# Hanbo-Cheng/DAWN-pytorch

Measured on NVIDIA H100. Metric: denoising-steps/sec (200-frame 256^2 clip), higher is better.
Workload: dtype f32

## Files before the change

### dawn_pytorch_b200/_lib.py

```python
import ctypes
import os

import torch
from torch import nn

_HERE = os.path.dirname(os.path.abspath(__file__))
LIB_PATH = os.path.join(_HERE, "libdawn_unet.so")


class DawnUnetCfg(ctypes.Structure):
    _fields_ = [("dim", ctypes.c_int), ("n_levels", ctypes.c_int), ("dim_mults", ctypes.c_int * 8),
                ("channels", ctypes.c_int), ("cond_aud", ctypes.c_int), ("cond_pose", ctypes.c_int),
                ("cond_eye", ctypes.c_int), ("out_grid_dim", ctypes.c_int), ("out_conf_dim", ctypes.c_int),
                ("attn_heads", ctypes.c_int), ("attn_dim_head", ctypes.c_int), ("resnet_groups", ctypes.c_int),
                ("init_kernel_size", ctypes.c_int), ("win_width", ctypes.c_int),
                ("upconv", ctypes.c_int), ("pad_mode", ctypes.c_int), ("no_sla", ctypes.c_int)]


class DawnLfgCfg(ctypes.Structure):
    _fields_ = [("num_channels", ctypes.c_int), ("block_expansion", ctypes.c_int), ("max_features", ctypes.c_int),
                ("num_down_blocks", ctypes.c_int), ("num_bottleneck_blocks", ctypes.c_int), ("skips", ctypes.c_int)]


PATH_MMA_SYNC, PATH_TC_GEMM, PATH_TC_GEMM_PRESPLIT, PATH_TC_CONV3, PATH_TC_CONV3_TMA = range(5)
EPI_PLAIN, EPI_QKV_TEMPORAL, EPI_QKV_SLA, EPI_QKV_MID, EPI_CA_GATE, EPI_GN_APPLY, EPI_GELU, EPI_LN_BIAS, EPI_LN_BIAS_GELU = range(9)


class DawnContractionCase(ctypes.Structure):
    _i, _p = ctypes.c_int, ctypes.c_void_p
    _fields_ = [("path", _i), ("epi", _i),
                ("F", _i), ("IH", _i), ("IW", _i), ("Cin", _i), ("lda", _i),
                ("ntaps", _i), ("dy", _i * 52), ("dx", _i * 52), ("in_stride", _i),
                ("OHs", _i), ("OWs", _i), ("OH", _i), ("OW", _i), ("out_stride", _i), ("oy0", _i), ("ox0", _i),
                ("up2", _i),
                ("perm_pb", _i), ("perm_F", _i), ("perm_in", _i), ("perm_out", _i), ("perm_f_lo", _i), ("perm_f_hi", _i),
                ("P", _i),
                ("N", _i), ("ldb", _i), ("ldo", _i), ("ldr", _i), ("drain", _i), ("ln_inline", _i),
                ("rows_per_batch", _i), ("b_batch_stride", ctypes.c_longlong), ("cpg", _i),
                ("q_post_scale", ctypes.c_float),
                ("A", _p), ("B", _p), ("bias", _p), ("Res", _p), ("Out", _p),
                ("stats", _p), ("rowstats", _p), ("wsum", _p), ("rot", _p),
                ("kq", _p), ("nkq", _p), ("gates", _p),
                ("Y", _p), ("ldy", _i), ("gn_stats", _p), ("gn_w", _p), ("gn_b", _p), ("film", _p), ("gn_count", ctypes.c_double)]


FUSED_TEMPORAL, FUSED_ATTN_TC, FUSED_ATTN_SIMT, FUSED_SLA_CTX, FUSED_SLA_OUT, FUSED_SLA_CTX_UNFUSED, FUSED_CA_WT, \
    FUSED_CA_RSTD, FUSED_GN_HCOND, FUSED_TEMPORAL_MMA_SYNC = range(10)


class DawnFusedCase(ctypes.Structure):
    _i, _p = ctypes.c_int, ctypes.c_void_p
    _fields_ = [("kernel", _i), ("F", _i), ("P", _i), ("C", _i), ("band", _i), ("q_lo", _i), ("q_hi", _i),
                ("nseq", _i), ("L", _i), ("pb", _i), ("seq_base_stride", ctypes.c_longlong), ("elem_stride", ctypes.c_longlong),
                ("ldx", _i), ("ldr", _i), ("ldo", _i), ("ld", _i), ("ldb", _i), ("ldy", _i), ("ldbT", _i),
                ("x", _p), ("res", _p), ("out", _p), ("gamma", _p), ("w_qkv", _p), ("w_out", _p), ("rot", _p), ("bias", _p),
                ("qkv", _p), ("Bf", _p), ("out_bias", _p), ("kq", _p), ("nkq", _p), ("G", _p), ("gates", _p), ("Wt", _p),
                ("T", _p), ("Y", _p), ("out16h", _p), ("out16l", _p),
                ("gn_stats", _p), ("gn_count", ctypes.c_double), ("cpg", _i), ("gn_w", _p), ("gn_b", _p), ("film", _p)]


KERNEL_ROWSTATS, KERNEL_GN_APPLY, KERNEL_COND_TABLES, KERNEL_TIME_MLP, KERNEL_FILM, KERNEL_ROTARY, KERNEL_SPLIT_ROWS, \
    KERNEL_NCF_TO_NHWC, KERNEL_FRAME_INVARIANCE, KERNEL_FEA_SHIFT, KERNEL_MAP_REDUCE, KERNEL_INIT_CONV_X3, KERNEL_HEADS_OUT, \
    KERNEL_DDIM_STEP, KERNEL_DDPM_STEP = range(15)
KERNEL_MAX_DESC = 16


class DawnKernelDesc(ctypes.Structure):
    _i, _p = ctypes.c_int, ctypes.c_void_p
    _fields_ = [("off", _i), ("K", _i), ("co", _i), ("ldbT", _i), ("ca", _i),
                ("mW", _p), ("mB", _p), ("Wkv", _p), ("nkv", _p), ("qs", _p), ("ks", _p), ("Wout", _p), ("gout", _p),
                ("ctx", _p), ("kv", _p), ("kq", _p), ("nkq", _p), ("T", _p), ("G", _p),
                ("W", _p), ("b", _p), ("out", _p), ("n", _i)]


class DawnKernelCase(ctypes.Structure):
    _i, _p, _ll = ctypes.c_int, ctypes.c_void_p, ctypes.c_longlong
    _fields_ = [("kernel", _i), ("M", _i), ("C", _i), ("ld", _i), ("ldy", _i), ("ldr", _i), ("ldo", _i),
                ("F", _i), ("H", _i), ("W", _i), ("P", _i), ("clips", _i),
                ("Cpad", _i), ("c0", _i), ("k", _i), ("skip_if", _i), ("cpg", _i), ("t_stride", _i), ("pos0", _i), ("dim", _i),
                ("ng", _i), ("nc", _i), ("cond_ld", _i), ("ndesc", _i),
                ("n", _ll), ("cstride", _ll), ("clip_stride", _ll), ("count", ctypes.c_double), ("eps", ctypes.c_float),
                ("x", _p), ("y", _p), ("res", _p), ("w", _p), ("b", _p), ("w2", _p), ("b2", _p),
                ("map", _p), ("freqs", _p), ("stats", _p), ("t", _p), ("skip_flag", _p),
                ("out", _p), ("out_hi", _p), ("out_lo", _p), ("flag", _p),
                ("desc", DawnKernelDesc * KERNEL_MAX_DESC),
                ("xs", _p), ("e", _p), ("noise", _p), ("scratch", _p), ("tab", _p), ("t_slot", _p), ("num_t", _i),
                ("replicas", _i), ("coef", ctypes.c_float * 5), ("q", ctypes.c_float)]


LFG_MOTION_PACK, LFG_WARP_BLEND, LFG_AFFINE_RELU, LFG_RESIDUAL_BN_RELU, LFG_RELU_AVGPOOL2, LFG_CHW_TO_HWC, LFG_HWC_TO_CHW, \
    LFG_FINAL_CONV = range(8)


class DawnLfgKernelCase(ctypes.Structure):
    _i, _p = ctypes.c_int, ctypes.c_void_p
    _fields_ = [("kernel", _i), ("F", _i), ("H", _i), ("W", _i), ("h", _i), ("w", _i), ("C", _i), ("Cpad", _i),
                ("layout", _i), ("blend", _i), ("ldx", _i), ("ldp", _i), ("ldo", _i), ("M", ctypes.c_longlong),
                ("x", _p), ("y", _p), ("flow", _p), ("occ", _p), ("motion", _p), ("prev", _p), ("scale", _p), ("shift", _p),
                ("weight", _p), ("bias", _p), ("source", _p), ("out", _p), ("out2", _p)]


class DawnLfgMotionCfg(ctypes.Structure):
    _i, _f = ctypes.c_int, ctypes.c_float
    _fields_ = [("num_regions", _i), ("num_channels", _i), ("estimate_affine", _i), ("pca_based", _i), ("fast_svd", _i),
                ("rp_block_expansion", _i), ("rp_max_features", _i), ("rp_num_blocks", _i), ("rp_temperature", _f),
                ("rp_scale_factor", _f), ("bg_block_expansion", _i), ("bg_max_features", _i), ("bg_num_blocks", _i),
                ("bg_type", _i), ("pw_block_expansion", _i), ("pw_max_features", _i), ("pw_num_blocks", _i),
                ("pw_scale_factor", _f), ("use_covar_heatmap", _i), ("use_deformed_source", _i),
                ("estimate_occlusion_map", _i), ("revert_axis_swap", _i)]


LFG_BG_ZERO, LFG_BG_AFFINE = 0, 1
LFGM_AA_DOWN, LFGM_REGION_MOMENTS, LFGM_FLOW_INPUT, LFGM_FLOW_COMBINE, LFGM_BG_HEAD = range(5)


class DawnLfgMotionKernelCase(ctypes.Structure):
    _i, _p = ctypes.c_int, ctypes.c_void_p
    _fields_ = [("kernel", _i), ("N", _i), ("H", _i), ("W", _i), ("h", _i), ("w", _i), ("R", _i), ("ld", _i), ("off", _i),
                ("cw", _i), ("ldl", _i), ("revert", _i), ("temperature", ctypes.c_float),
                ("x", _p), ("weight", _p), ("logits", _p), ("motion", _p), ("source", _p), ("bg", _p), ("fc_w", _p), ("fc_b", _p),
                ("src_shift", _p), ("src_covar", _p), ("src_affine", _p), ("drv_shift", _p), ("drv_covar", _p), ("drv_affine", _p),
                ("out", _p), ("out2", _p), ("out3", _p)]


class DawnPbnetCfg(ctypes.Structure):
    _fields_ = [(n, ctypes.c_int) for n in ("band", "pose_dim", "audio_dim", "latent_dim", "audio_latent_dim", "pose_latent_dim",
                                            "ff_size", "num_layers", "num_heads")]


class DawnPbnetAttentionCase(ctypes.Structure):
    _i, _p = ctypes.c_int, ctypes.c_void_p
    _fields_ = [("bs", _i), ("F", _i), ("D", _i), ("H", _i), ("band", _i), ("npairs", _i), ("qscale", ctypes.c_float),
                ("x_q", _p), ("x_kv", _p), ("wq", _p), ("wk", _p), ("wv", _p), ("freqs", _p), ("bias", _p), ("out", _p)]


class DawnHubertCfg(ctypes.Structure):
    _i = ctypes.c_int
    _fields_ = [("hidden_size", _i), ("num_layers", _i), ("num_heads", _i), ("intermediate_size", _i), ("num_conv", _i),
                ("conv_dim", _i * 8), ("conv_kernel", _i * 8), ("conv_stride", _i * 8), ("conv_bias", _i), ("pos_kernel", _i),
                ("pos_groups", _i), ("layer_norm_eps", ctypes.c_float)]


HUBERT_ATTENTION, HUBERT_CONV0, HUBERT_POS_CONV, HUBERT_ROW_LN, HUBERT_FE_CONV, HUBERT_LN_LINEAR = range(6)


class DawnHubertKernelCase(ctypes.Structure):
    _i, _p = ctypes.c_int, ctypes.c_void_p
    _fields_ = [("kernel", _i), ("B", _i), ("T", _i), ("L", _i), ("H", _i), ("ld", _i), ("C", _i), ("k", _i), ("s", _i), ("G", _i),
                ("eps", ctypes.c_float), ("q", _p), ("kk", _p), ("v", _p), ("x", _p), ("w", _p), ("bias", _p), ("gamma", _p),
                ("beta", _p), ("g", _p), ("out", _p),
                ("M", _i), ("N", _i), ("ldo", _i), ("gelu", _i), ("parts", _i), ("qscale", ctypes.c_float)]


class DawnError(RuntimeError):
    pass


def _load():
    if not os.path.exists(LIB_PATH):
        raise ImportError(
            f"{LIB_PATH} is missing: build it with `python dawn_pytorch_b200/build.py` "
            "(nvcc, sm_90a). There is no CPU or PyTorch fallback for the DAWN denoising UNet.")
    lib = ctypes.CDLL(LIB_PATH)
    vp, i64p, fp, cp = ctypes.c_void_p, ctypes.POINTER(ctypes.c_int64), ctypes.c_void_p, ctypes.c_char_p
    lib.dawn_unet_create.argtypes = [ctypes.POINTER(DawnUnetCfg), ctypes.POINTER(vp)]
    lib.dawn_unet_destroy.argtypes = [vp]
    lib.dawn_unet_destroy.restype = None
    lib.dawn_unet_set_param.argtypes = [vp, cp, fp, i64p, ctypes.c_int]
    lib.dawn_unet_commit_params.argtypes = [vp]
    lib.dawn_unet_set_num_frames.argtypes = [vp, ctypes.c_int, ctypes.c_int, ctypes.c_int]
    lib.dawn_unet_set_geometry.argtypes = [vp, ctypes.c_int, ctypes.c_int, ctypes.c_int, ctypes.c_int]
    lib.dawn_unet_set_clip_invariants.argtypes = [vp, fp, fp, vp]
    lib.dawn_unet_forward.argtypes = [vp, fp, vp, fp, fp, vp]
    lib.dawn_unet_forward_x3.argtypes = [vp, fp, vp, fp, vp]
    lib.dawn_unet_forward_host.argtypes = [vp, fp, fp, fp, ctypes.c_int64, fp]
    lib.dawn_unet_set_tap.argtypes = [vp, cp, fp]
    lib.dawn_unet_tap_shape.argtypes = [vp, cp, ctypes.POINTER(ctypes.c_int), ctypes.POINTER(ctypes.c_int),
                                        ctypes.POINTER(ctypes.c_int)]
    dp = ctypes.POINTER(ctypes.c_double)
    lib.dawn_unet_profile_enable.argtypes = [vp, ctypes.c_int]
    lib.dawn_unet_profile_read.argtypes = [vp, dp, dp, dp, i64p]
    lib.dawn_unet_last_launch_count.argtypes = [vp]
    lib.dawn_unet_last_launch_count.restype = ctypes.c_int64
    lib.dawn_unet_workspace_bytes.argtypes = [vp]
    lib.dawn_unet_workspace_bytes.restype = ctypes.c_int64
    lib.dawn_test_contraction.argtypes = [ctypes.POINTER(DawnContractionCase), vp]
    lib.dawn_test_fused.argtypes = [ctypes.POINTER(DawnFusedCase), vp]
    lib.dawn_test_kernel.argtypes = [ctypes.POINTER(DawnKernelCase), vp]
    lib.dawn_nccl_unique_id.argtypes = [ctypes.c_char_p]
    lib.dawn_unet_init_shard.argtypes = [vp, ctypes.c_char_p, ctypes.c_int, ctypes.c_int, ctypes.c_int]
    lib.dawn_unet_shard_ipc_export.argtypes = [vp, ctypes.c_char_p]
    lib.dawn_unet_shard_ipc_import.argtypes = [vp, ctypes.c_char_p]
    lib.dawn_ddim_step.argtypes = [fp, fp, fp, ctypes.c_int64] + [ctypes.c_float] * 6 + [vp, vp]
    lib.dawn_unet_ddim_step.argtypes = [vp, fp, fp, fp, ctypes.c_int64] + [ctypes.c_float] * 6 + [vp, vp]
    lib.dawn_unet_sampler_capture.argtypes = [vp, fp, fp, fp, vp, ctypes.POINTER(ctypes.c_float), ctypes.c_int, ctypes.c_float, vp]
    lib.dawn_unet_sampler_launch.argtypes = [vp, vp]
    lib.dawn_unet_ddim_step_guided.argtypes = [vp, fp, fp, fp, ctypes.c_int64, fp] + [ctypes.c_float] * 6 + [vp, vp]
    lib.dawn_unet_sampler_capture_guided.argtypes = [vp, fp, fp, fp, vp, fp, ctypes.POINTER(ctypes.c_float), ctypes.c_int,
                                                     ctypes.c_float, vp]
    lib.dawn_unet_sampler_launch_guided.argtypes = [vp, vp]
    lib.dawn_ddpm_step.argtypes = [fp, fp, fp, ctypes.c_int64] + [ctypes.c_float] * 6 + [vp, vp]
    lib.dawn_unet_ddpm_step.argtypes = [vp, fp, fp, fp, ctypes.c_int64] + [ctypes.c_float] * 6 + [vp, vp]
    lib.dawn_unet_ddpm_capture.argtypes = [vp, fp, fp, fp, vp, fp, ctypes.c_int, ctypes.c_float, vp]
    lib.dawn_unet_ddpm_launch.argtypes = [vp, vp]
    ip = ctypes.POINTER(ctypes.c_int)
    lib.dawn_lfg_create.argtypes = [ctypes.POINTER(DawnLfgCfg), ctypes.POINTER(vp)]
    lib.dawn_lfg_destroy.argtypes = [vp]
    lib.dawn_lfg_destroy.restype = None
    lib.dawn_lfg_set_param.argtypes = [vp, cp, fp, i64p, ctypes.c_int]
    lib.dawn_lfg_commit_params.argtypes = [vp]
    lib.dawn_lfg_set_geometry.argtypes = [vp] + [ctypes.c_int] * 5
    lib.dawn_lfg_set_source.argtypes = [vp, fp, vp]
    lib.dawn_lfg_get_fea.argtypes = [vp, fp, vp]
    lib.dawn_lfg_decode.argtypes = [vp, fp, fp, fp, fp, vp]
    lib.dawn_lfg_decode_sample.argtypes = [vp, fp, fp, fp, vp]
    lib.dawn_lfg_read_tap.argtypes = [vp, cp, fp, ip, ip, ip, vp]
    lib.dawn_conv3x3_s2_relu.argtypes = [fp, ctypes.c_int, ctypes.c_int, ctypes.c_int, fp, fp, ctypes.c_int, fp, vp]
    lib.dawn_lfg_last_launch_count.argtypes = [vp]
    lib.dawn_lfg_last_launch_count.restype = ctypes.c_int64
    lib.dawn_lfg_workspace_bytes.argtypes = [vp]
    lib.dawn_lfg_workspace_bytes.restype = ctypes.c_int64
    lib.dawn_lfg_test_kernel.argtypes = [ctypes.POINTER(DawnLfgKernelCase), vp]
    lib.dawn_lfg_motion_create.argtypes = [ctypes.POINTER(DawnLfgMotionCfg), ctypes.POINTER(vp)]
    lib.dawn_lfg_motion_destroy.argtypes = [vp]
    lib.dawn_lfg_motion_destroy.restype = None
    lib.dawn_lfg_motion_set_param.argtypes = [vp, cp, fp, i64p, ctypes.c_int]
    lib.dawn_lfg_motion_commit_params.argtypes = [vp]
    lib.dawn_lfg_motion_set_geometry.argtypes = [vp] + [ctypes.c_int] * 3
    lib.dawn_lfg_motion_regions.argtypes = [vp, fp, ctypes.c_int, fp, fp, fp, vp]
    lib.dawn_lfg_motion_bg.argtypes = [vp, fp, ctypes.c_int, fp, ctypes.c_int, fp, vp]
    lib.dawn_lfg_motion_flow.argtypes = [vp, fp, ctypes.c_int] + [fp] * 9 + [vp]
    lib.dawn_lfg_motion_read_tap.argtypes = [vp, cp, fp, ip, ip, ip, ip, vp]
    lib.dawn_lfg_motion_last_launch_count.argtypes = [vp]
    lib.dawn_lfg_motion_last_launch_count.restype = ctypes.c_int64
    lib.dawn_lfg_motion_workspace_bytes.argtypes = [vp]
    lib.dawn_lfg_motion_workspace_bytes.restype = ctypes.c_int64
    lib.dawn_lfg_motion_test_kernel.argtypes = [ctypes.POINTER(DawnLfgMotionKernelCase), vp]
    lib.dawn_pbnet_create.argtypes = [ctypes.POINTER(DawnPbnetCfg), ctypes.POINTER(vp)]
    lib.dawn_pbnet_destroy.argtypes = [vp]
    lib.dawn_pbnet_destroy.restype = None
    lib.dawn_pbnet_set_param.argtypes = [vp, cp, fp, i64p, ctypes.c_int]
    lib.dawn_pbnet_commit_params.argtypes = [vp]
    lib.dawn_pbnet_generate.argtypes = [vp, fp, fp, fp, fp, ctypes.c_int, ctypes.c_int, fp, vp]
    lib.dawn_pbnet_last_launch_count.argtypes = [vp]
    lib.dawn_pbnet_last_launch_count.restype = ctypes.c_int64
    lib.dawn_pbnet_workspace_bytes.argtypes = [vp]
    lib.dawn_pbnet_workspace_bytes.restype = ctypes.c_int64
    lib.dawn_pbnet_test_attention.argtypes = [ctypes.POINTER(DawnPbnetAttentionCase), vp]
    lib.dawn_hubert_create.argtypes = [ctypes.POINTER(DawnHubertCfg), ctypes.POINTER(vp)]
    lib.dawn_hubert_destroy.argtypes = [vp]
    lib.dawn_hubert_destroy.restype = None
    lib.dawn_hubert_set_param.argtypes = [vp, cp, fp, i64p, ctypes.c_int]
    lib.dawn_hubert_commit_params.argtypes = [vp]
    lib.dawn_hubert_forward.argtypes = [vp, fp, ctypes.c_int, ctypes.c_int, fp, vp]
    lib.dawn_hubert_output_length.argtypes = [vp, ctypes.c_int]
    lib.dawn_hubert_hidden.argtypes = [vp, fp, ctypes.c_int, ctypes.c_int, ctypes.c_int, fp, vp]
    lib.dawn_hubert_last_launch_count.argtypes = [vp]
    lib.dawn_hubert_last_launch_count.restype = ctypes.c_int64
    lib.dawn_hubert_workspace_bytes.argtypes = [vp]
    lib.dawn_hubert_workspace_bytes.restype = ctypes.c_int64
    lib.dawn_hubert_test_kernel.argtypes = [ctypes.POINTER(DawnHubertKernelCase), vp]
    lib.dawn_last_error.restype = cp
    lib.dawn_live_bytes.argtypes = []
    lib.dawn_live_bytes.restype = ctypes.c_int64
    lib.dawn_build_info.restype = cp
    return lib


lib = _load()

EXPORTS = ["dawn_unet_create", "dawn_unet_destroy", "dawn_unet_set_param", "dawn_unet_commit_params",
           "dawn_unet_set_num_frames", "dawn_unet_set_geometry", "dawn_nccl_unique_id", "dawn_unet_init_shard", "dawn_unet_shard_ipc_export", "dawn_unet_shard_ipc_import", "dawn_unet_set_clip_invariants", "dawn_unet_forward",
           "dawn_unet_forward_x3", "dawn_unet_forward_host", "dawn_unet_set_tap", "dawn_unet_tap_shape",
           "dawn_unet_profile_enable", "dawn_unet_profile_read", "dawn_unet_last_launch_count", "dawn_unet_workspace_bytes", "dawn_ddim_step", "dawn_unet_ddim_step", "dawn_unet_sampler_capture", "dawn_unet_sampler_launch",
           "dawn_unet_ddim_step_guided", "dawn_unet_sampler_capture_guided", "dawn_unet_sampler_launch_guided",
           "dawn_ddpm_step", "dawn_unet_ddpm_step", "dawn_unet_ddpm_capture", "dawn_unet_ddpm_launch",
           "dawn_test_contraction", "dawn_test_fused", "dawn_test_kernel", "dawn_last_error", "dawn_live_bytes", "dawn_build_info"]


LFG_EXPORTS = ["dawn_lfg_create", "dawn_lfg_destroy", "dawn_lfg_set_param", "dawn_lfg_commit_params", "dawn_lfg_set_geometry",
               "dawn_lfg_set_source", "dawn_lfg_get_fea", "dawn_lfg_decode", "dawn_lfg_decode_sample", "dawn_lfg_read_tap",
               "dawn_lfg_last_launch_count", "dawn_lfg_workspace_bytes", "dawn_lfg_test_kernel"]
LFG_MOTION_EXPORTS = ["dawn_lfg_motion_create", "dawn_lfg_motion_destroy", "dawn_lfg_motion_set_param",
                      "dawn_lfg_motion_commit_params", "dawn_lfg_motion_set_geometry", "dawn_lfg_motion_regions", "dawn_lfg_motion_bg",
                      "dawn_lfg_motion_flow", "dawn_lfg_motion_read_tap", "dawn_lfg_motion_last_launch_count",
                      "dawn_lfg_motion_workspace_bytes", "dawn_lfg_motion_test_kernel"]
LFG_EXPORTS += LFG_MOTION_EXPORTS
MISC_EXPORTS = ["dawn_conv3x3_s2_relu"]
PBNET_EXPORTS = ["dawn_pbnet_create", "dawn_pbnet_destroy", "dawn_pbnet_set_param", "dawn_pbnet_commit_params",
                 "dawn_pbnet_generate", "dawn_pbnet_last_launch_count", "dawn_pbnet_workspace_bytes", "dawn_pbnet_test_attention"]
HUBERT_EXPORTS = ["dawn_hubert_create", "dawn_hubert_destroy", "dawn_hubert_set_param", "dawn_hubert_commit_params",
                  "dawn_hubert_forward", "dawn_hubert_output_length", "dawn_hubert_hidden", "dawn_hubert_last_launch_count", "dawn_hubert_workspace_bytes",
                  "dawn_hubert_test_kernel"]

PROF_CATS = ["conv3x3", "conv_other", "qkv_proj", "out_proj", "ca_gate", "gn_hcond", "attn_core", "sla_context",
             "gn_apply", "rowstats", "ca_rstd", "misc", "prep", "temporal_fused_l0", "conv3x3_l0", "comm_allreduce", "comm_halo"]
PROF_NCAT = 20


def check(rc, what):
    if rc != 0:
        raise DawnError(f"{what} failed (rc={rc}): {lib.dawn_last_error().decode()}")


def stream():
    return ctypes.c_void_p(torch.cuda.current_stream().cuda_stream)


def ptr(t):
    return ctypes.c_void_p(t.data_ptr()) if t is not None else None


def put_param(set_param, handle, name, t):
    t = t.detach().to(device="cpu", dtype=torch.float32).contiguous()
    shape = (ctypes.c_int64 * max(t.dim(), 1))(*t.shape)
    check(set_param(handle, name.encode(), ctypes.c_void_p(t.data_ptr()), shape, t.dim()), f"{set_param.__name__}({name})")


class _Holder(nn.Module):

    def forward(self, *a, **k):
        raise RuntimeError("parameter holder: the computation runs in the CUDA library")


class _Handle:

    def __init__(self, api, cfg, what, param_name=lambda key: key, extra=lambda module: {}, keeps_geom=False):
        self.api, self.cfg, self.what, self.param_name, self.extra, self.keeps_geom = api, cfg, what, param_name, extra, keeps_geom
        self.handle, self.device_index, self.dirty, self.geom, self.commits = None, None, True, None, 0

    def _entry(self, name):
        return getattr(lib, f"{self.api}_{name}")

    def _create(self):
        hd = ctypes.c_void_p()
        check(self._entry("create")(ctypes.byref(self.cfg), ctypes.byref(hd)), f"{self.api}_create")
        return hd

    def validate(self):
        self._entry("destroy")(self._create())

    def destroy(self):
        if self.handle is not None:
            self._entry("destroy")(self.handle)
        self.handle, self.geom = None, None

    def ensure(self, module, device):
        if device.type != "cuda":
            raise DawnError(f"{self.what} runs on CUDA (sm_90a) only; there is no CPU path")
        idx = device.index if device.index is not None else torch.cuda.current_device()
        if self.handle is not None and self.device_index != idx:
            self.destroy()
            self.dirty = True
        with torch.cuda.device(idx):
            if self.handle is None:
                self.handle, self.device_index = self._create(), idx
            if self.dirty:
                for key, t in module.state_dict().items():
                    name = None if key.endswith("num_batches_tracked") else self.param_name(key)
                    if name is not None:
                        put_param(self._entry("set_param"), self.handle, name, t)
                for name, t in self.extra(module).items():
                    put_param(self._entry("set_param"), self.handle, name, t)
                check(self._entry("commit_params")(self.handle), f"{self.api}_commit_params")
                self.dirty, self.commits = False, self.commits + 1
                if not self.keeps_geom:
                    self.geom = None
        return idx

    def last_launch_count(self):
        return int(self._entry("last_launch_count")(self.handle)) if self.handle is not None else 0

    def workspace_bytes(self):
        return int(self._entry("workspace_bytes")(self.handle)) if self.handle is not None else 0


class _NativeModule(nn.Module):
    TRAIN_REFUSAL = None

    def _hold(self, *handles):
        self._handles = list(handles)
        self.register_load_state_dict_post_hook(lambda module, incompatible: module.mark_dirty())
        if self.TRAIN_REFUSAL:
            self.eval()

    def mark_dirty(self):
        for h in self._handles:
            h.dirty = True

    def _apply(self, fn, *a, **k):
        for h in self.__dict__.get("_handles", ()):
            h.dirty = True
        return super()._apply(fn, *a, **k)

    def train(self, mode=True):
        if mode and self.TRAIN_REFUSAL:
            raise NotImplementedError(self.TRAIN_REFUSAL)
        return super().train(mode)

    def __del__(self):
        for h in self.__dict__.get("_handles", ()):
            try:
                h.destroy()
            except Exception:
                pass

    def last_launch_count(self):
        return self._handles[0].last_launch_count()

    def workspace_bytes(self):
        return self._handles[0].workspace_bytes()
```

### dawn_pytorch_b200/csrc/contraction.cu

```cuda
#include <algorithm>
#include <atomic>
#include <cmath>
#include <cstring>

#include "common.cuh"
#include "contraction.cuh"
#include "kernels.cuh"
#include "tc_gemm.cuh"

namespace dawn {

void HostParams::set(const std::string& name, const float* data, const int64_t* shape, int ndim) {
  HostParam p;
  p.shape.assign(shape, shape + ndim);
  int64_t numel = 1;
  for (int64_t s : p.shape) numel *= s;
  p.data.assign(data, data + numel);
  map[name] = std::move(p);
}

int HostParams::need(const std::string& name, const std::vector<int64_t>& shape, const HostParam** out) const {
  auto it = map.find(name);
  if (it == map.end()) { set_last_error(prefix + "missing parameter: " + name); return -1; }
  const HostParam& p = it->second;
  if (p.shape != shape) {
    std::string s = prefix + "parameter " + name + " has shape (";
    for (auto d : p.shape) s += std::to_string(d) + ",";
    s += ") expected (";
    for (auto d : shape) s += std::to_string(d) + ",";
    set_last_error(s + ")");
    return -1;
  }
  *out = &p;
  return 0;
}

namespace {
std::atomic<int64_t> g_arena_bytes{0};
}

int DeviceArena::alloc_bytes(size_t bytes, void** out) {
  *out = nullptr;
  bytes = std::max<size_t>(bytes, 16);
  DAWN_CUDA_OK(cudaMalloc(out, bytes));
  blocks_.emplace_back(*out);
  bytes_ += (int64_t)bytes;
  g_arena_bytes += (int64_t)bytes;
  return 0;
}
int DeviceArena::copy_in(void* dst, const void* src, size_t bytes) {
  DAWN_CUDA_OK(cudaMemcpy(dst, src, bytes, cudaMemcpyHostToDevice));
  return 0;
}
void DeviceArena::release() {
  blocks_.clear();
  g_arena_bytes -= bytes_;
  bytes_ = 0;
}
int64_t DeviceArena::live_bytes() { return g_arena_bytes.load(); }

int upload_weight(DeviceArena& arena, const std::vector<float>& m, int K, int N, int ldb, const std::vector<float>& bias,
                  PackedWeight* out) {
  *out = PackedWeight{};
  DAWN_TRY(arena.upload(m, &out->w));
  if (N % 64 == 0 && K % 64 == 0) {
    std::vector<float> img;
    tc_pack_weights(m.data(), K, N, ldb, img, &out->img_scale);
    DAWN_TRY(arena.upload(img, &out->img));
  }
  if (!bias.empty()) {
    std::vector<float> b(ldb, 0.f);
    std::copy(bias.begin(), bias.end(), b.begin());
    DAWN_TRY(arena.upload(b, &out->b));
  }
  out->K = K; out->N = N; out->ldb = ldb;
  return 0;
}

std::vector<float> fold_linear(const float* w, int N, int K, const float* gain, float qscale, int nscale) {
  std::vector<float> m((size_t)N * K);
  for (int n = 0; n < N; ++n) {
    const float sc = (n < nscale) ? qscale : 1.0f;
    for (int k = 0; k < K; ++k) {
      float v = w[(size_t)n * K + k];
      if (gain) v *= gain[k];
      m[(size_t)n * K + k] = v * sc;
    }
  }
  return m;
}

std::vector<float> row_sums(const std::vector<float>& w, int N, int K) {
  std::vector<float> s(N);
  for (int n = 0; n < N; ++n) {
    double acc = 0.0;
    for (int k = 0; k < K; ++k) acc += w[(size_t)n * K + k];
    s[n] = (float)acc;
  }
  return s;
}

void fold_ca_q(const float* const to_q[3], const float* const gain[3], int ci, std::vector<float>& wq, std::vector<float>& wsum) {
  wq.assign((size_t)ci * 192, 0.f);
  wsum.assign(192, 0.f);
  for (int a = 0; a < 3; ++a) {
    const std::vector<float> m = fold_linear(to_q[a], 64, ci, gain[a], 1.f, 0);
    const std::vector<float> s = row_sums(m, 64, ci);
    for (int j = 0; j < 64; ++j) {
      for (int k = 0; k < ci; ++k) wq[(size_t)k * 192 + a * 64 + j] = m[(size_t)j * ci + k];
      wsum[a * 64 + j] = s[j];
    }
  }
}

int bn_affine(const HostParams& raw, const std::string& prefix, int c, std::vector<double>& s, std::vector<double>& t) {
  const HostParam *g, *b, *rm, *rv;
  DAWN_TRY(raw.need(prefix + ".weight", {c}, &g));
  DAWN_TRY(raw.need(prefix + ".bias", {c}, &b));
  DAWN_TRY(raw.need(prefix + ".running_mean", {c}, &rm));
  DAWN_TRY(raw.need(prefix + ".running_var", {c}, &rv));
  s.resize(c); t.resize(c);
  for (int i = 0; i < c; ++i) {
    s[i] = (double)g->data[i] / std::sqrt((double)rv->data[i] + 1e-5);
    t[i] = (double)b->data[i] - (double)rm->data[i] * s[i];
  }
  return 0;
}

void pack_conv_taps(const float* w, int co, int ci, int taps, int ci_pad, int ldb, int n0, const double* scale, std::vector<float>& m) {
  for (int n = 0; n < co; ++n) {
    const double sn = scale ? scale[n] : 1.0;
    for (int c = 0; c < ci; ++c)
      for (int tp = 0; tp < taps; ++tp)
        m[((size_t)tp * ci_pad + c) * ldb + n0 + n] = (float)((double)w[((size_t)n * ci + c) * taps + tp] * sn);
  }
}

int pack_lfg_conv(const HostParams& raw, DeviceArena& arena, const std::vector<std::pair<std::string, int>>& convs,
                  const std::string& bn_after, int ci, int k, int ci_pad, PackedWeight* out) {
  int N = 0;
  for (auto& c : convs) N += c.second;
  const int ldb = round_up(N, 64), K = k * k * ci_pad;
  std::vector<float> m((size_t)K * ldb, 0.f), bias(N);
  int n0 = 0;
  for (auto& cv : convs) {
    const int co = cv.second;
    const HostParam *w, *b;
    DAWN_TRY(raw.need(cv.first + ".weight", {co, ci, k, k}, &w));
    DAWN_TRY(raw.need(cv.first + ".bias", {co}, &b));
    std::vector<double> s(co, 1.0), t(co, 0.0);
    if (!bn_after.empty()) DAWN_TRY(bn_affine(raw, bn_after, co, s, t));
    for (int n = 0; n < co; ++n) bias[n0 + n] = (float)((double)b->data[n] * s[n] + t[n]);
    pack_conv_taps(w->data.data(), co, ci, k * k, ci_pad, ldb, n0, s.data(), m);
    n0 += co;
  }
  return upload_weight(arena, m, K, N, ldb, bias, out);
}

void base_params(GemmParams& p, const float* A, int lda, int Cin, int frames, int H, int W) {
  memset(&p, 0, sizeof(p));
  p.A = A; p.lda = lda; p.Cin = Cin;
  p.IH = H; p.IW = W; p.OHs = H; p.OWs = W; p.in_stride = 1;
  p.ntaps = 1;
  p.M = frames * H * W; p.rows_per_batch = p.M;
  p.OH = H; p.OW = W; p.out_stride = 1;
  p.P = H * W;
  p.q_post_scale = 1.f;
  p.clips = 1;
}
void set_weights(GemmParams& p, const PackedWeight& w) {
  p.B = w.w; p.Bimg = w.img; p.tc_scale = 1.0f / w.img_scale; p.ldb = w.ldb; p.N = w.N; p.K = w.K; p.bias = w.b;
}
void set_square_taps(GemmParams& p, int k, int pad) {
  p.ntaps = k * k;
  for (int ky = 0; ky < k; ++ky)
    for (int kx = 0; kx < k; ++kx) { p.dy[ky * k + kx] = (signed char)(ky - pad); p.dx[ky * k + kx] = (signed char)(kx - pad); }
}

namespace {
long long split_rows(const GemmParams& p) { return (long long)(p.M / (p.OHs * p.OWs)) * p.IH * p.IW; }
}

bool path_ok(const GemmParams& p, int epi, int path, size_t scratch_bytes) {
  const bool planes = p.A16h != nullptr || (p.Cin % 64 == 0 && (size_t)split_rows(p) * p.Cin * 4 <= scratch_bytes);
  switch (path) {
    case DAWN_PATH_MMA_SYNC: return true;
    case DAWN_PATH_TC_GEMM: return p.Bimg && tc_gemm_supported(p, epi);
    case DAWN_PATH_TC_GEMM_PRESPLIT: return p.Bimg && tc_gemm_supported(p, epi) && planes;
    case DAWN_PATH_TC_CONV3: return p.Bimg && tc_conv3_supported(p, epi);
    case DAWN_PATH_TC_CONV3_TMA: return p.Bimg && tc_conv3_supported(p, epi) && p.lda == p.Cin && planes;
  }
  return false;
}

int choose_path(const GemmParams& p, int epi, size_t scratch_bytes) {
  if (path_ok(p, epi, DAWN_PATH_TC_CONV3, 0)) return p.A16h ? DAWN_PATH_TC_CONV3_TMA : DAWN_PATH_TC_CONV3;
  if (!path_ok(p, epi, DAWN_PATH_TC_GEMM, 0)) return DAWN_PATH_MMA_SYNC;
  const bool split = (p.ntaps == 9 && p.N >= 256 && !p.perm_in) || p.want_split;
  return split && path_ok(p, epi, DAWN_PATH_TC_GEMM_PRESPLIT, scratch_bytes) ? DAWN_PATH_TC_GEMM_PRESPLIT : DAWN_PATH_TC_GEMM;
}

int launch_path(const GemmParams& p, int epi, int path, void* scratch, cudaStream_t st, int* kernels) {
  if (kernels) *kernels = 1;
  if (path == DAWN_PATH_MMA_SYNC) return launch_gemm(p, epi, st);
  GemmParams q = p;
  if ((path == DAWN_PATH_TC_GEMM_PRESPLIT || path == DAWN_PATH_TC_CONV3_TMA) && p.A16h == nullptr) {
    const long long rows = split_rows(p);
    unsigned short* hi = static_cast<unsigned short*>(scratch);
    q.A16h = hi; q.A16l = hi + (size_t)rows * p.Cin;
    DAWN_TRY(launch_split_rows(p.A, p.lda, p.Cin, rows, (void*)q.A16h, (void*)q.A16l, st));
    if (kernels) *kernels = 2;
  }
  if (path == DAWN_PATH_TC_CONV3 || path == DAWN_PATH_TC_CONV3_TMA) return launch_tc_conv3(q, q.Bimg, st);
  return launch_tc_gemm(q, q.Bimg, epi, st);
}

int pack_up(DeviceArena& arena, int ci, int co, const int (&off)[2][2], const std::vector<float>& bias, const UpWeight& weight,
            UpConv* u) {
  memcpy(u->off, off, sizeof(u->off));
  const int ldb = round_up(co, 64);
  for (int py = 0; py < 2; ++py)
    for (int px = 0; px < 2; ++px) {
      std::vector<float> m((size_t)4 * ci * ldb, 0.f);
      for (int ty = 0; ty < 2; ++ty)
        for (int tx = 0; tx < 2; ++tx)
          for (int c = 0; c < ci; ++c)
            for (int n = 0; n < co; ++n) m[((size_t)(ty * 2 + tx) * ci + c) * ldb + n] = weight(py, px, ty, tx, c, n);
      DAWN_TRY(upload_weight(arena, m, 4 * ci, co, ldb, bias, &u->cls[py * 2 + px]));
    }
  if (co == 64 && ci % 64 == 0) {
    const int N4 = 4 * co;
    std::vector<float> m((size_t)9 * ci * N4, 0.f), b4(N4, 0.f);
    for (int py = 0; py < 2; ++py)
      for (int px = 0; px < 2; ++px) {
        const int cls = py * 2 + px;
        for (int n = 0; n < co; ++n) b4[cls * co + n] = bias[n];
        for (int ty = 0; ty < 2; ++ty)
          for (int tx = 0; tx < 2; ++tx) {
            const int tap = (off[py][ty] + 1) * 3 + (off[px][tx] + 1);
            for (int c = 0; c < ci; ++c)
              for (int n = 0; n < co; ++n) m[((size_t)tap * ci + c) * N4 + cls * co + n] = weight(py, px, ty, tx, c, n);
          }
      }
    DAWN_TRY(upload_weight(arena, m, 9 * ci, N4, N4, b4, &u->all));
  }
  return 0;
}

int pack_up_nearest(DeviceArena& arena, const float* w, int ci, int co, const double* scale, const std::vector<float>& bias,
                    UpConv* u) {
  return pack_up(arena, ci, co, kUpOff, bias, [&](int py, int px, int ty, int tx, int c, int n) {
    double acc = 0.0;
    for (int ky = 0; ky < 3; ++ky)
      for (int kx = 0; kx < 3; ++kx)
        if (up_in_set(py, ty, ky) && up_in_set(px, tx, kx)) acc += (double)w[(((size_t)n * ci + c) * 3 + ky) * 3 + kx];
    return (float)(scale ? acc * scale[n] : acc);
  }, u);
}

int pack_lfg_up(const HostParams& raw, DeviceArena& arena, const std::string& name, int co, int ci, UpConv* u) {
  const HostParam *w, *b;
  DAWN_TRY(raw.need(name + ".conv.weight", {co, ci, 3, 3}, &w));
  DAWN_TRY(raw.need(name + ".conv.bias", {co}, &b));
  std::vector<double> s, t;
  DAWN_TRY(bn_affine(raw, name + ".norm", co, s, t));
  std::vector<float> bias(co);
  for (int n = 0; n < co; ++n) bias[n] = (float)((double)b->data[n] * s[n] + t[n]);
  return pack_up_nearest(arena, w->data.data(), ci, co, s.data(), bias, u);
}

int run_up(const GemmParams& in, const UpConv& u, float* out, int ldo, const std::function<int(const GemmParams&)>& run, int border) {
  if (!border) {
    GemmParams p = in;
    set_weights(p, u.all); set_square_taps(p, 3, 1);
    p.up2 = 1; p.Out = out; p.ldo = ldo;
    if (path_ok(p, EPI_PLAIN, DAWN_PATH_TC_CONV3, 0)) return run(p);
  }
  for (int py = 0; py < 2; ++py)
    for (int px = 0; px < 2; ++px) {
      GemmParams q = in;
      set_weights(q, u.cls[py * 2 + px]);
      q.ntaps = 4;
      for (int ty = 0; ty < 2; ++ty)
        for (int tx = 0; tx < 2; ++tx) {
          q.dy[ty * 2 + tx] = (signed char)(u.off[py][ty] + border); q.dx[ty * 2 + tx] = (signed char)(u.off[px][tx] + border);
        }
      q.OH = 2 * in.OHs; q.OW = 2 * in.OWs; q.out_stride = 2; q.oy0 = py; q.ox0 = px;
      q.Out = out; q.ldo = ldo;
      DAWN_TRY(run(q));
    }
  return 0;
}

namespace {

int refuse(const char* why) {
  set_last_error(std::string("dawn_test_contraction: ") + why);
  return -1;
}

int test_contraction(const dawn_contraction_case& c, cudaStream_t st) {
  if (c.path < DAWN_PATH_MMA_SYNC || c.path > DAWN_PATH_TC_CONV3_TMA) return refuse("unknown path");
  if (c.epi < EPI_PLAIN || c.epi > EPI_LN_BIAS_GELU) return refuse("unknown epilogue");
  if (c.ntaps < 1 || c.ntaps > 52 || c.F < 1 || c.N < 1 || c.ldb < c.N || c.lda < 1 || (c.ntaps > 1 && c.lda < c.Cin))
    return refuse("bad geometry");
  if (!c.A || !c.B) return refuse("A and B are required");
  if (c.epi == EPI_CA_GATE ? !c.gates : !c.Out) return refuse("no output buffer");

  GemmParams p;
  memset(&p, 0, sizeof(p));
  p.A = c.A; p.lda = c.lda; p.Cin = c.Cin;
  p.up2 = c.up2;
  p.IH = c.IH; p.IW = c.IW; p.OHs = c.OHs; p.OWs = c.OWs; p.in_stride = c.in_stride;
  p.ntaps = c.ntaps;
  for (int t = 0; t < c.ntaps; ++t) { p.dy[t] = (signed char)c.dy[t]; p.dx[t] = (signed char)c.dx[t]; }
  p.M = c.F * c.OHs * c.OWs; p.N = c.N; p.K = c.ntaps * c.Cin;
  p.rows_per_batch = c.rows_per_batch > 0 ? c.rows_per_batch : p.M;
  p.perm_pb = c.perm_pb; p.perm_F = c.perm_F; p.perm_in = c.perm_in; p.perm_out = c.perm_out;
  p.perm_f_lo = c.perm_f_lo; p.perm_f_hi = c.perm_f_hi;
  p.B = c.B; p.ldb = c.ldb; p.b_batch_stride = c.b_batch_stride;
  p.Out = c.Out; p.ldo = c.ldo; p.OH = c.OH; p.OW = c.OW; p.out_stride = c.out_stride; p.oy0 = c.oy0; p.ox0 = c.ox0;
  p.bias = c.bias; p.Res = c.Res; p.ldr = c.ldr;
  p.stats = c.stats; p.cpg = c.cpg; p.clips = 1;
  p.rowstats = c.rowstats; p.ln_inline = c.ln_inline; p.wsum = c.wsum; p.rot = c.rot; p.P = c.P;
  p.q_post_scale = c.q_post_scale;
  p.kq = c.kq; p.nkq = c.nkq; p.gates = c.gates;
  p.Y = c.Y; p.ldy = c.ldy; p.gn_stats = c.gn_stats; p.gn_w = c.gn_w; p.gn_b = c.gn_b; p.film = c.film; p.gn_count = c.gn_count;
  p.drain = c.drain;

  const bool ln_bias = c.epi == EPI_LN_BIAS || c.epi == EPI_LN_BIAS_GELU;
  const bool ln = (c.epi >= EPI_QKV_TEMPORAL && c.epi <= EPI_CA_GATE) || ln_bias;
  if (p.ln_inline && (c.path != DAWN_PATH_TC_GEMM || p.ntaps != 1)) return refuse("inline LayerNorm statistics need the gather-producer wgmma GEMM and one tap");
  if (ln && !p.ln_inline && !p.rowstats) return refuse("LayerNorm epilogue without row statistics");
  if (ln && !p.wsum) return refuse("LayerNorm epilogue without wsum");
  if (ln_bias && !p.bias) return refuse("LayerNorm + bias epilogue without a bias");
  if (p.stats && c.epi != EPI_PLAIN) return refuse("GroupNorm statistics with an epilogue other than the plain one");
  if (c.epi == EPI_PLAIN && p.stats && (p.cpg <= 0 || p.N / p.cpg > 8)) return refuse("GroupNorm statistics need 8 groups");

  DeviceArena arena;
  if (c.path != DAWN_PATH_MMA_SYNC) {
    std::vector<float> hB((size_t)p.K * p.ldb);
    DAWN_CUDA_OK(cudaMemcpy(hB.data(), p.B, hB.size() * sizeof(float), cudaMemcpyDeviceToHost));
    PackedWeight w;
    DAWN_TRY(upload_weight(arena, hB, p.K, p.N, p.ldb, {}, &w));
    set_weights(p, w);
    p.bias = c.bias;
  }
  const bool split = c.path == DAWN_PATH_TC_GEMM_PRESPLIT || c.path == DAWN_PATH_TC_CONV3_TMA;
  const size_t scratch_bytes = split ? (size_t)split_rows(p) * p.Cin * 4 : 0;
  if (!path_ok(p, c.epi, c.path, scratch_bytes)) return refuse("the path does not accept this geometry");
  unsigned short* scratch = nullptr;
  if (split) DAWN_TRY(arena.alloc(scratch_bytes / sizeof(unsigned short), &scratch));
  DAWN_TRY(launch_path(p, c.epi, c.path, scratch, st));
  DAWN_CUDA_OK(cudaStreamSynchronize(st));
  return 0;
}

}
}

extern "C" int dawn_test_contraction(const dawn_contraction_case* c, void* stream) {
  if (!c) return dawn::refuse("null case");
  return dawn::test_contraction(*c, static_cast<cudaStream_t>(stream));
}
```

### dawn_pytorch_b200/csrc/gemm.cuh

```cuda
#pragma once
#include <cuda_runtime.h>

namespace dawn {

enum Epi : int {
  EPI_PLAIN = 0,
  EPI_QKV_TEMPORAL = 1,
  EPI_QKV_SLA = 2,
  EPI_QKV_MID = 3,
  EPI_CA_GATE = 4,
  EPI_GN_APPLY = 5,
  EPI_GELU = 6,
  EPI_LN_BIAS = 7,
  EPI_LN_BIAS_GELU = 8,
};

__device__ __forceinline__ float gelu_erf(float x) { return 0.5f * x * (1.0f + erff(x * 0.70710678118654752440f)); }

struct GemmParams {
  const float* A; int lda; int Cin;
  const unsigned short* A16h = nullptr; const unsigned short* A16l = nullptr;
  int want_split = 0;
  int up2 = 0;
  int IH, IW;
  int OHs, OWs;
  int in_stride;
  int ntaps; signed char dy[52]; signed char dx[52];
  int M, N, K;
  int rows_per_batch;
  int perm_pb, perm_F, perm_in, perm_out;
  int perm_f_lo, perm_f_hi;
  const float* B; int ldb; long long b_batch_stride;
  const float* Bimg;
  float tc_scale;
  float* Out; int ldo; int OH, OW, out_stride, oy0, ox0;
  const float* bias;
  const float* Res; int ldr;
  double* stats; int cpg;
  int clips;
  const float* rowstats;
  int ln_inline;
  const float* wsum;
  const float* rot;
  int P;
  float q_post_scale;
  const float* kq;
  const float* nkq;
  float* gates;
  const float* Y; int ldy; const double* gn_stats; const float* gn_w; const float* gn_b;
  const float* film;
  double gn_count;
  const int* skip_flag; int skip_if;
  int drain;
};

__host__ __device__ inline int seq_blocked_pixel(int m, int pb, int F, int P) {
  const int blk = m / (F * pb), rem = m - blk * F * pb;
  const int f = rem / pb, pi = rem - f * pb;
  return f * P + blk * pb + pi;
}
__host__ __device__ inline int seq_blocked_out_pixel(int m, int pb, int F, int P, int f_lo, int f_hi) {
  const int blk = m / (F * pb), rem = m - blk * F * pb;
  const int f = rem / pb, pi = rem - f * pb;
  if (f < f_lo || f >= f_hi) return -1;
  return (f - f_lo) * P + blk * pb + pi;
}

int launch_gemm(const GemmParams& p, int epi, cudaStream_t st);

}
```

### dawn_pytorch_b200/csrc/tc_conv3.cu

```cuda
#include <cuda.h>
#include <cuda_fp16.h>
#include <cstdlib>
#include <cstring>
#include <string>
#include <map>
#include <tuple>
#include "common.cuh"
#include "f16x3.cuh"
#include "gemm.cuh"
#include "tc_common.cuh"
#include "tc_gemm.cuh"

namespace dawn {
namespace {

using namespace tc;

constexpr int TH = 16, TW = 8;
constexpr int HH = TH + 2, HW = TW + 2;
constexpr int NPROD = 256;
constexpr int PAIR_HH = 8 + 2;
constexpr int PAIR_ROW_B = 104;

template <int BN, bool PAIR = false>
struct CCfg {
  static_assert(!PAIR || BN == 64, "the pair-mode halos fit next to 64-column weight stages only");
  static constexpr int NWG = BN / 64;
  static constexpr bool SPLIT_EPI = (BN == 64);
  static constexpr int B_PANEL = BN * 128;
  static constexpr int FRAME_ROWS = PAIR ? PAIR_HH * HW : HH * HW;
  static constexpr int HALO_ROWS = PAIR ? PAIR_ROW_B + FRAME_ROWS : FRAME_ROWS;
  static constexpr int A_HALO = (HALO_ROWS * 128 + 1023) / 1024 * 1024;
  static constexpr int A_STAGES = 2;
  static constexpr int B_STAGES = PAIR ? 3 : (BN == 64) ? 4 : 2;
  static constexpr int A_BYTES = A_STAGES * 2 * A_HALO;
  static constexpr int B_BYTES = B_STAGES * 2 * B_PANEL;
  static constexpr int ACC_STAGE = 2 * 128 * kStageLd * 4;
  static constexpr int SMEM_DYN = A_BYTES + B_BYTES + ACC_STAGE + 1024;
  static_assert(SMEM_DYN + 1024 <= 232448, "shared memory");
  static constexpr int EPI_WARP = NPROD / 32 + 4 * NWG;
  static constexpr int LOAD_WARP = EPI_WARP + (SPLIT_EPI ? 4 : 0);
  static constexpr int NTHREADS = 32 * LOAD_WARP + 128;
  static constexpr uint32_t REG_LAUNCH = (65536 / NTHREADS) & ~7u;
  static constexpr uint32_t REG_LOAD = 24, REG_MMA = SPLIT_EPI ? 136 : 128, REG_EPI = 128;
  static_assert(REG_LOAD < REG_LAUNCH && REG_MMA > REG_LAUNCH && REG_EPI > REG_LAUNCH, "register budgets");
  static_assert(2 * REG_LAUNCH + REG_LOAD + NWG * REG_MMA + (SPLIT_EPI ? REG_EPI : 0) <= NTHREADS / 128 * REG_LAUNCH, "CTA register pool");
};

template <int BN, bool TMA, bool PAIR>
__device__ __forceinline__ void tc_conv3_body(const GemmParams& p, const float* __restrict__ Bimg, int tiles_y, int tiles_x, int tiles_n,
                                              int img_bn, const CUtensorMap& tm_hi, const CUtensorMap& tm_lo) {
  using C = CCfg<BN, PAIR>;
  constexpr int B_PANEL = C::B_PANEL, A_STAGES = C::A_STAGES, B_STAGES = C::B_STAGES, NWG = C::NWG;
  constexpr int A_HALO = C::A_HALO, FRAME_ROWS = C::FRAME_ROWS;
  constexpr bool SPLIT = C::SPLIT_EPI;
  extern __shared__ uint8_t smem_raw[];
  __shared__ uint64_t a_full[A_STAGES], a_free[A_STAGES], b_full[B_STAGES], b_free[B_STAGES];
  __shared__ uint64_t st_full[2], st_free[2];
  __shared__ float s_stat[NWG][16];
  __shared__ __align__(16) float s_bias[NWG][64];

  const int tid = threadIdx.x, lane = tid & 31;
  const int warp = __shfl_sync(0xffffffffu, tid >> 5, 0);
  uint8_t* smem = smem_align1024(smem_raw);
  uint8_t* smemA = smem;
  uint8_t* smemB = smem + C::A_BYTES;
  float* stage_base = reinterpret_cast<float*>(smemB + C::B_BYTES);

  if (tid == 0) {
    for (int s = 0; s < A_STAGES; ++s) { mbar_init(&a_full[s], TMA ? 1 : NPROD); mbar_init(&a_free[s], 4 * NWG); }
    for (int s = 0; s < B_STAGES; ++s) { mbar_init(&b_full[s], 1); mbar_init(&b_free[s], 4 * NWG); }
    for (int s = 0; s < 2; ++s) { mbar_init(&st_full[s], 128); mbar_init(&st_free[s], 128); }
    asm volatile("fence.mbarrier_init.release.cluster;" ::: "memory");
  }
  __syncthreads();

  const int H = p.IH, W = p.IW;
  const int F = p.M / (H * W);
  const int NCH = p.Cin / 64;
  const int tiles_sp = tiles_y * tiles_x;
  const int fpc = F / p.clips;
  const int ppc = (fpc + 1) / 2;
  const int total_tiles = (PAIR ? p.clips * ppc : F * tiles_sp) * tiles_n;
  auto decode = [&](int tile, int& f, int& y0, int& x0, int& nt, int& nf) {
    nt = tile % tiles_n;
    const int sp = tile / tiles_n;
    if constexpr (PAIR) {
      const int clip = sp / ppc, fa = 2 * (sp - clip * ppc);
      f = fa * p.clips + clip;
      nf = fa + 1 < fpc ? 2 : 1;
      y0 = 0; x0 = 0;
    } else {
      const int seq = sp / tiles_sp;
      const int r = sp - seq * tiles_sp;
      f = p.clips == 1 ? seq : (seq % fpc) * p.clips + seq / fpc;
      nf = 1;
      y0 = (r / tiles_x) * TH; x0 = (r % tiles_x) * TW;
    }
  };

  if (warp < 8) {
    if (TMA) {
      if (tid == 0) {
        const uint64_t mh = reinterpret_cast<uint64_t>(&tm_hi), ml = reinterpret_cast<uint64_t>(&tm_lo);
        uint32_t ait = 0;
        for (int tile = blockIdx.x; tile < total_tiles; tile += gridDim.x) {
          int f, y0, x0, nt, nf;
          decode(tile, f, y0, x0, nt, nf);
          for (int cc = 0; cc < NCH; ++cc, ++ait) {
            const int s = ait % A_STAGES;
            mbar_wait(&a_free[s], ((ait / A_STAGES) & 1) ^ 1);
            mbar_arrive_expect_tx(&a_full[s], nf * 2 * FRAME_ROWS * 128);
            const uint32_t bar = smem_u32(&a_full[s]);
            const int c0 = cc * 64, c1 = x0 - 1, c2 = y0 - 1;
            for (int fr = 0; fr < nf; ++fr) {
              const uint32_t dst = smem_u32(smemA + s * 2 * A_HALO) + fr * PAIR_ROW_B * 128;
              const int c3 = f + fr * p.clips;
              asm volatile("cp.async.bulk.tensor.4d.shared::cluster.global.tile.mbarrier::complete_tx::bytes [%0], [%1, {%3, %4, %5, %6}], [%2];"
                           ::"r"(dst), "l"(mh), "r"(bar), "r"(c0), "r"(c1), "r"(c2), "r"(c3) : "memory");
              asm volatile("cp.async.bulk.tensor.4d.shared::cluster.global.tile.mbarrier::complete_tx::bytes [%0], [%1, {%3, %4, %5, %6}], [%2];"
                           ::"r"(dst + A_HALO), "l"(ml), "r"(bar), "r"(c0), "r"(c1), "r"(c2), "r"(c3) : "memory");
            }
          }
        }
      }
    } else {
      constexpr int NQ = (C::FRAME_ROWS * (PAIR ? 2 : 1) + 31) / 32;
      const int c16 = tid & 7;
      const int r0 = (tid >> 3) & 31;
      uint32_t ait = 0;
      for (int tile = blockIdx.x; tile < total_tiles; tile += gridDim.x) {
        int f, y0, x0, nt, nf;
        decode(tile, f, y0, x0, nt, nf);
        const float* img = p.A + (size_t)f * H * W * p.lda;
        const float* img_b = PAIR ? img + (size_t)p.clips * H * W * p.lda : img;
        for (int cc = 0; cc < NCH; ++cc, ++ait) {
          const int s = ait % A_STAGES;
          const uint32_t round = ait / A_STAGES;
          auto load = [&](int q, float4& a, float4& b) {
            const int l = r0 + 32 * q;
            const int fr = (!PAIR || 32 * q + 31 < FRAME_ROWS) ? 0 : (32 * q >= FRAME_ROWS) ? 1 : (l >= FRAME_ROWS ? 1 : 0);
            const int r = l - fr * FRAME_ROWS;
            const int hy = r / HW, hx = r - hy * HW;
            const int iy = y0 + hy - 1, ix = x0 + hx - 1;
            const bool ok = (r < FRAME_ROWS) && fr < nf && (iy >= 0) && (iy < H) && (ix >= 0) && (ix < W);
            if (ok) {
              const float* fimg = fr ? img_b : img;
              const float4* src = reinterpret_cast<const float4*>(fimg + (size_t)(iy * W + ix) * p.lda + cc * 64) + 2 * c16;
              a = __ldg(src);
              b = __ldg(src + 1);
            } else {
              a = make_float4(0.f, 0.f, 0.f, 0.f);
              b = make_float4(0.f, 0.f, 0.f, 0.f);
            }
          };
          uint8_t* a_hi = smemA + s * 2 * A_HALO;
          uint8_t* a_lo = a_hi + A_HALO;
          auto store = [&](int q, const float4& a, const float4& b) {
            const int lr = r0 + 32 * q;
            const int fr = (!PAIR || 32 * q + 31 < FRAME_ROWS) ? 0 : (32 * q >= FRAME_ROWS) ? 1 : (lr >= FRAME_ROWS ? 1 : 0);
            const int r = lr + fr * (PAIR_ROW_B - FRAME_ROWS);
            if (lr < FRAME_ROWS * (PAIR ? 2 : 1)) {
              uint32_t h[4], l[4];
              split_f16x2_rn(a.x, a.y, h[0], l[0]);
              split_f16x2_rn(a.z, a.w, h[1], l[1]);
              split_f16x2_rn(b.x, b.y, h[2], l[2]);
              split_f16x2_rn(b.z, b.w, h[3], l[3]);
              const uint32_t off = swz(r, c16);
              *reinterpret_cast<uint4*>(a_hi + off) = make_uint4(h[0], h[1], h[2], h[3]);
              *reinterpret_cast<uint4*>(a_lo + off) = make_uint4(l[0], l[1], l[2], l[3]);
            }
          };
          constexpr int NPRE = NQ < 6 ? NQ : 6;
          float4 v[2 * NPRE];
#pragma unroll
          for (int q = 0; q < NPRE; ++q) load(q, v[2 * q], v[2 * q + 1]);
          mbar_wait(&a_free[s], (round & 1) ^ 1);
#pragma unroll
          for (int q = 0; q < NPRE; ++q) store(q, v[2 * q], v[2 * q + 1]);
#pragma unroll
          for (int q = NPRE; q < NQ; ++q) {
            float4 a, b;
            load(q, a, b);
            store(q, a, b);
          }
          mbar_arrive_relaxed(&a_full[s]);
        }
      }
    }
    return;
  }
  if (warp >= C::LOAD_WARP) {
    setmaxnreg_dec<C::REG_LOAD>();
    if (warp == C::LOAD_WARP && lane == 0) {
      uint32_t bit = 0;
      const int KC = 9 * NCH;
      const int sub = PAIR ? img_bn / BN : 1;
      const size_t ipanel = (size_t)sub * B_PANEL;
      for (int tile = blockIdx.x; tile < total_tiles; tile += gridDim.x) {
        int f, y0, x0, nt, nf;
        decode(tile, f, y0, x0, nt, nf);
        const uint8_t* src = reinterpret_cast<const uint8_t*>(Bimg) + (size_t)(nt / sub) * KC * (2 * ipanel) + (size_t)(nt % sub) * B_PANEL;
        for (int cc = 0; cc < NCH; ++cc)
          for (int tap = 0; tap < 9; ++tap, ++bit) {
            const int s = bit % B_STAGES;
            const uint32_t round = bit / B_STAGES;
            mbar_wait(&b_free[s], (round & 1) ^ 1);
            mbar_arrive_expect_tx(&b_full[s], 2 * B_PANEL);
            const uint8_t* panel = src + (size_t)(tap * NCH + cc) * (2 * ipanel);
            if (PAIR) {
              bulk_copy_g2s(smemB + s * 2 * B_PANEL, panel, B_PANEL, &b_full[s]);
              bulk_copy_g2s(smemB + s * 2 * B_PANEL + B_PANEL, panel + ipanel, B_PANEL, &b_full[s]);
            } else {
              bulk_copy_g2s(smemB + s * 2 * B_PANEL, panel, 2 * B_PANEL, &b_full[s]);
            }
          }
      }
    }
    return;
  }

  const int wg = SPLIT ? 0 : (warp - 8) >> 2;
  const int ew = (warp - 8) & 3;
  const int etid = ew * 32 + lane;
  const int bar_id = 2 + wg;
  constexpr uint32_t SBO_HALO = HW * 128;
  constexpr uint32_t H2 = PAIR ? PAIR_ROW_B * 128 : 8 * HW * 128;
  const int dt = (p.drain == 1 || p.drain == 3) ? p.drain : 9;

  auto mma_tile = [&](auto DTc, float* stage, uint32_t& ait, uint32_t& bit, auto&& claim) {
    constexpr int DT = decltype(DTc)::value;
    float d0[32], d1[32];
    bool first_drain = true;
    for (int cc = 0; cc < NCH; ++cc, ++ait) {
      const int sa = ait % A_STAGES;
      mbar_wait(&a_full[sa], (ait / A_STAGES) & 1);
      fence_proxy_async();
      const uint32_t a_hi = smem_u32(smemA + sa * 2 * A_HALO), a_lo = a_hi + A_HALO;
      static_for<0, 9>([&](auto TAPc) {
        constexpr int tap = decltype(TAPc)::value;
        constexpr bool group_first = tap % DT == 0, group_last = tap % DT == DT - 1;
        constexpr uint32_t woff = (uint32_t)(((tap / 3) * HW + tap % 3) * 128);
        const int sb = bit % B_STAGES;
        const int sprev = (bit + B_STAGES - 1) % B_STAGES;
        mbar_wait(&b_full[sb], (bit / B_STAGES) & 1);
        const uint64_t ahi = make_desc(a_hi + woff, SBO_HALO), alo = make_desc(a_lo + woff, SBO_HALO);
        const uint64_t ahi2 = make_desc(a_hi + woff + H2, SBO_HALO), alo2 = make_desc(a_lo + woff + H2, SBO_HALO);
        const uint32_t sbaddr = smem_u32(smemB + sb * 2 * B_PANEL) + wg * 64 * 128;
        const uint64_t bhi = make_desc(sbaddr), blo = make_desc(sbaddr + B_PANEL);
        wgmma_fence();
#pragma unroll
        for (int j = 0; j < 4; ++j) {
          const uint64_t o = (uint64_t)(j * 2);
          const uint32_t acc = (group_first && j == 0) ? 0u : 1u;
          wgmma_m64n64k16(d0, alo + o, bhi + o, acc);
          wgmma_m64n64k16(d1, alo2 + o, bhi + o, acc);
          wgmma_m64n64k16(d0, ahi + o, blo + o, 1u);
          wgmma_m64n64k16(d1, ahi2 + o, blo + o, 1u);
          wgmma_m64n64k16(d0, ahi + o, bhi + o, 1u);
          wgmma_m64n64k16(d1, ahi2 + o, bhi + o, 1u);
        }
        wgmma_commit();
        if constexpr (group_last) {
          wgmma_wait<0>();
          wgmma_fence_acc(d0); wgmma_fence_acc(d1);
          if (lane == 0) { if (!group_first) mbar_arrive(&b_free[sprev]); mbar_arrive(&b_free[sb]); }
          if (first_drain) claim();
          stage_fragment(stage, 0, d0, first_drain, etid);
          stage_fragment(stage, 64, d1, first_drain, etid);
          first_drain = false;
        } else {
          wgmma_wait<1>();
          wgmma_fence_acc(d0); wgmma_fence_acc(d1);
          if (lane == 0 && !group_first) mbar_arrive(&b_free[sprev]);
        }
        ++bit;
      });
      if (lane == 0) mbar_arrive(&a_free[sa]);
    }
  };

  const bool defer_stats = (p.stats != nullptr) && tiles_n == 1;
  const bool bias_smem = (p.bias != nullptr) && tiles_n == 1;
  auto load_bias = [&]() {
    if (bias_smem) {
      if (etid < 64) s_bias[wg][etid] = __ldg(p.bias + wg * 64 + etid);
      asm volatile("bar.sync %0, 128;" ::"r"(bar_id) : "memory");
    }
  };
  auto flush_stats = [&](float (&gs)[8], float (&gss)[8], int clip) {
    const int n0f = wg * 64;
    double* cs = p.stats + 16 * clip;
#pragma unroll
    for (int b8 = 0; b8 < 8; ++b8) {
      double s = (double)gs[b8], ss = (double)gss[b8];
#pragma unroll
      for (int o = 16; o > 0; o >>= 1) { s += __shfl_xor_sync(0xffffffffu, s, o); ss += __shfl_xor_sync(0xffffffffu, ss, o); }
      if (lane == 0) {
        const int grp = (n0f + b8 * 8) / p.cpg;
        atomicAdd(&cs[2 * grp], s);
        atomicAdd(&cs[2 * grp + 1], ss);
      }
      gs[b8] = 0.f; gss[b8] = 0.f;
    }
  };
  auto epilogue_tile = [&](int tile, float* stage, float (&gs)[8], float (&gss)[8], int& pending, int& pclip) {
    int f, y0, x0, nt, nf;
    decode(tile, f, y0, x0, nt, nf);
    const int clip = p.clips > 1 ? f % p.clips : 0;
    const int n0 = nt * BN + wg * 64;
    const int row_in_tile = etid;
    float* s_st = s_stat[wg];
    float* wbuf = stage + ew * 32 * kStageLd;
    float acc[64];
    {
      const float4* src = reinterpret_cast<const float4*>(stage + row_in_tile * kStageLd);
#pragma unroll
      for (int i = 0; i < 16; ++i) {
        const float4 v = src[i];
        acc[4 * i] = v.x; acc[4 * i + 1] = v.y; acc[4 * i + 2] = v.z; acc[4 * i + 3] = v.w;
      }
    }
    __syncwarp();
#pragma unroll
    for (int i = 0; i < 64; ++i) acc[i] *= p.tc_scale;
    const int fr = PAIR ? row_in_tile >> 6 : 0;
    const int img = f + fr * p.clips;
    const int oy = y0 + ((row_in_tile >> 3) & (PAIR ? 7 : 15)), ox = x0 + (row_in_tile & 7);
    const bool rv = (oy < H) && (ox < W) && fr < nf;
    size_t opix = (size_t)img * H * W + (size_t)(rv ? oy * W + ox : 0);
    int ocol = n0;
    if (p.up2) {
      const int cls = n0 >> 6, py = cls >> 1, px = cls & 1;
      opix = (size_t)img * 4 * H * W + (size_t)(rv ? (2 * oy + py) * 2 * W + 2 * ox + px : 0);
      ocol = n0 & 63;
    }
    if (bias_smem) {
      const float4* bp = reinterpret_cast<const float4*>(s_bias[wg]);
#pragma unroll
      for (int i = 0; i < 16; ++i) {
        const float4 b = bp[i];
        acc[4 * i] += b.x; acc[4 * i + 1] += b.y; acc[4 * i + 2] += b.z; acc[4 * i + 3] += b.w;
      }
    } else if (p.bias) {
      const float4* bp = reinterpret_cast<const float4*>(p.bias + n0);
#pragma unroll
      for (int i = 0; i < 16; ++i) {
        const float4 b = __ldg(bp + i);
        acc[4 * i] += b.x; acc[4 * i + 1] += b.y; acc[4 * i + 2] += b.z; acc[4 * i + 3] += b.w;
      }
    }
    store_rows_coalesced(wbuf, acc, p.Out, opix, p.ldo, ocol, rv, lane);
    if (defer_stats) {
      if (pending > 0 && clip != pclip) { flush_stats(gs, gss, pclip); pending = 0; }
      pclip = clip;
      if (rv) {
#pragma unroll
        for (int b8 = 0; b8 < 8; ++b8) {
          float s = 0.f, ss = 0.f;
#pragma unroll
          for (int i = 0; i < 8; ++i) { const float x = acc[b8 * 8 + i]; s += x; ss += x * x; }
          gs[b8] += s; gss[b8] += ss;
        }
      }
      if (++pending == 8) { flush_stats(gs, gss, clip); pending = 0; }
    } else if (p.stats != nullptr) {
      if (etid < 16) s_st[etid] = 0.f;
      asm volatile("bar.sync %0, 128;" ::"r"(bar_id) : "memory");
#pragma unroll
      for (int b8 = 0; b8 < 8; ++b8) {
        float s = 0.f, ss = 0.f;
        if (rv) {
#pragma unroll
          for (int i = 0; i < 8; ++i) { const float x = acc[b8 * 8 + i]; s += x; ss += x * x; }
        }
        s = warp_sum(s); ss = warp_sum(ss);
        if (lane == 0) {
          const int grp = (n0 + b8 * 8) / p.cpg;
          atomicAdd(&s_st[2 * grp], s);
          atomicAdd(&s_st[2 * grp + 1], ss);
        }
      }
      asm volatile("bar.sync %0, 128;" ::"r"(bar_id) : "memory");
      if (etid < 16) {
        const int grp = etid >> 1;
        const int glo = n0 / p.cpg, ghi = (n0 + 63) / p.cpg;
        if (grp >= glo && grp <= ghi) atomicAdd(&p.stats[16 * clip + etid], (double)s_st[etid]);
      }
    }
  };
  auto with_drain = [&](auto&& run) {
    if (dt == 1) run(std::integral_constant<int, 1>{});
    else if (dt == 3) run(std::integral_constant<int, 3>{});
    else run(std::integral_constant<int, 9>{});
  };

  if (SPLIT && warp >= C::EPI_WARP) {
    setmaxnreg_inc<C::REG_EPI>();
    float gs[8], gss[8];
    int pending = 0, pclip = 0;
#pragma unroll
    for (int i = 0; i < 8; ++i) { gs[i] = 0.f; gss[i] = 0.f; }
    load_bias();
    uint32_t lt = 0;
    for (int tile = blockIdx.x; tile < total_tiles; tile += gridDim.x, ++lt) {
      const int b = lt & 1;
      mbar_wait(&st_full[b], (lt >> 1) & 1);
      epilogue_tile(tile, stage_base + b * 128 * kStageLd, gs, gss, pending, pclip);
      mbar_arrive(&st_free[b]);
    }
    if (defer_stats && pending > 0) flush_stats(gs, gss, pclip);
  } else if (SPLIT) {
    setmaxnreg_inc<C::REG_MMA>();
    with_drain([&](auto DTc) {
      uint32_t ait = 0, bit = 0, lt = 0;
      for (int tile = blockIdx.x; tile < total_tiles; tile += gridDim.x, ++lt) {
        const int b = lt & 1;
        mma_tile(DTc, stage_base + b * 128 * kStageLd, ait, bit, [&]() { mbar_wait(&st_free[b], ((lt >> 1) & 1) ^ 1); });
        mbar_arrive(&st_full[b]);
      }
    });
  } else {
    setmaxnreg_inc<C::REG_MMA>();
    float gs[8], gss[8];
    int pending = 0, pclip = 0;
#pragma unroll
    for (int i = 0; i < 8; ++i) { gs[i] = 0.f; gss[i] = 0.f; }
    load_bias();
    float* stage = stage_base + wg * 128 * kStageLd;
    uint32_t ait = 0, bit = 0;
    for (int tile = blockIdx.x; tile < total_tiles; tile += gridDim.x) {
      with_drain([&](auto DTc) { mma_tile(DTc, stage, ait, bit, []() {}); });
      asm volatile("bar.sync %0, 128;" ::"r"(bar_id) : "memory");
      epilogue_tile(tile, stage, gs, gss, pending, pclip);
      asm volatile("bar.sync %0, 128;" ::"r"(bar_id) : "memory");
    }
    if (defer_stats && pending > 0) flush_stats(gs, gss, pclip);
  }
}

template <int BN, bool TMA>
__global__ void __launch_bounds__(CCfg<BN>::NTHREADS, 1) tc_conv3_kernel(const GemmParams p, const float* __restrict__ Bimg,
                                                                          int tiles_y, int tiles_x, int tiles_n, int img_bn,
                                                                          const __grid_constant__ CUtensorMap tm_hi,
                                                                          const __grid_constant__ CUtensorMap tm_lo) {
  tc_conv3_body<BN, TMA, false>(p, Bimg, tiles_y, tiles_x, tiles_n, img_bn, tm_hi, tm_lo);
}

template <bool TMA>
__global__ void __launch_bounds__(CCfg<64, true>::NTHREADS, 1) tc_conv3_pair_kernel(const GemmParams p, const float* __restrict__ Bimg,
                                                                                     int tiles_y, int tiles_x, int tiles_n, int img_bn,
                                                                                     const __grid_constant__ CUtensorMap tm_hi,
                                                                                     const __grid_constant__ CUtensorMap tm_lo) {
  tc_conv3_body<64, TMA, true>(p, Bimg, tiles_y, tiles_x, tiles_n, img_bn, tm_hi, tm_lo);
}

template <int BN, bool TMA, bool PAIR>
constexpr auto c3_kernel() {
  if constexpr (PAIR) return tc_conv3_pair_kernel<TMA>;
  else return tc_conv3_kernel<BN, TMA>;
}

typedef CUresult (*EncodeTiledFn)(CUtensorMap*, CUtensorMapDataType, cuuint32_t, void*, const cuuint64_t*, const cuuint64_t*, const cuuint32_t*,
                                  const cuuint32_t*, CUtensorMapInterleave, CUtensorMapSwizzle, CUtensorMapL2promotion, CUtensorMapFloatOOBfill);
int halo_tensor_map(const void* plane, int Cin, int W, int H, int F, int box_h, CUtensorMap* out) {
  static EncodeTiledFn fn = nullptr;
  if (!fn) {
    void* ptr = nullptr;
    cudaDriverEntryPointQueryResult q;
    DAWN_CUDA_OK(cudaGetDriverEntryPoint("cuTensorMapEncodeTiled", &ptr, cudaEnableDefault, &q));
    if (q != cudaDriverEntryPointSuccess || !ptr) { set_last_error("cuTensorMapEncodeTiled is not available in this driver"); return -2; }
    fn = reinterpret_cast<EncodeTiledFn>(ptr);
  }
  static std::map<std::tuple<const void*, int, int, int, int, int>, CUtensorMap> cache;
  const auto key = std::make_tuple(plane, Cin, W, H, F, box_h);
  auto it = cache.find(key);
  if (it != cache.end()) { *out = it->second; return 0; }
  const cuuint64_t dims[4] = {(cuuint64_t)Cin, (cuuint64_t)W, (cuuint64_t)H, (cuuint64_t)F};
  const cuuint64_t strides[3] = {(cuuint64_t)Cin * 2, (cuuint64_t)W * Cin * 2, (cuuint64_t)H * W * Cin * 2};
  const cuuint32_t box[4] = {64, (cuuint32_t)HW, (cuuint32_t)box_h, 1};
  const cuuint32_t estr[4] = {1, 1, 1, 1};
  CUtensorMap m;
  const CUresult r = fn(&m, CU_TENSOR_MAP_DATA_TYPE_UINT16, 4, const_cast<void*>(plane), dims, strides, box, estr, CU_TENSOR_MAP_INTERLEAVE_NONE,
                        CU_TENSOR_MAP_SWIZZLE_128B, CU_TENSOR_MAP_L2_PROMOTION_L2_128B, CU_TENSOR_MAP_FLOAT_OOB_FILL_NONE);
  if (r != CUDA_SUCCESS) { set_last_error("cuTensorMapEncodeTiled failed with CUresult " + std::to_string((int)r)); return -2; }
  if (cache.size() > 4096) cache.clear();
  cache[key] = m;
  *out = m;
  return 0;
}

template <int BN, bool PAIR>
int launch_c3(const GemmParams& p, const float* Bimg, cudaStream_t st) {
  using C = CCfg<BN, PAIR>;
  static bool attr_set = false;
  static int num_sms = 0;
  if (!attr_set) {
    DAWN_CUDA_OK(cudaFuncSetAttribute(c3_kernel<BN, false, PAIR>(), cudaFuncAttributeMaxDynamicSharedMemorySize, C::SMEM_DYN));
    DAWN_CUDA_OK(cudaFuncSetAttribute(c3_kernel<BN, true, PAIR>(), cudaFuncAttributeMaxDynamicSharedMemorySize, C::SMEM_DYN));
    int dev = 0;
    DAWN_CUDA_OK(cudaGetDevice(&dev));
    DAWN_CUDA_OK(cudaDeviceGetAttribute(&num_sms, cudaDevAttrMultiProcessorCount, dev));
    attr_set = true;
  }
  const int tiles_y = PAIR ? 1 : p.IH / TH, tiles_x = PAIR ? 1 : p.IW / TW, tiles_n = p.N / BN;
  const int F = p.M / (p.IH * p.IW);
  const int seqs = PAIR ? p.clips * ((F / p.clips + 1) / 2) : F;
  const int grid = std::min(seqs * tiles_y * tiles_x * tiles_n, num_sms);
  const int img_bn = tc_tile_n(p.N);
  if (p.A16h != nullptr && p.A16l != nullptr) {
    CUtensorMap mh, ml;
    const int box_h = PAIR ? PAIR_HH : HH;
    if (halo_tensor_map(p.A16h, p.Cin, p.IW, p.IH, F, box_h, &mh) != 0 || halo_tensor_map(p.A16l, p.Cin, p.IW, p.IH, F, box_h, &ml) != 0)
      return -2;
    c3_kernel<BN, true, PAIR>()<<<grid, C::NTHREADS, C::SMEM_DYN, st>>>(p, Bimg, tiles_y, tiles_x, tiles_n, img_bn, mh, ml);
  } else {
    CUtensorMap dummy;
    memset(&dummy, 0, sizeof(dummy));
    c3_kernel<BN, false, PAIR>()<<<grid, C::NTHREADS, C::SMEM_DYN, st>>>(p, Bimg, tiles_y, tiles_x, tiles_n, img_bn, dummy, dummy);
  }
  DAWN_LAUNCH_OK();
  return 0;
}

bool pair_mode(const GemmParams& p) { return p.IH == 8 && p.IW == 8; }

}

bool tc_conv3_supported(const GemmParams& p, int epi) {
  if (epi != EPI_PLAIN || p.Res != nullptr || p.perm_in || p.perm_out) return false;
  if (p.ntaps != 9 || p.in_stride != 1 || p.out_stride != 1 || p.oy0 != 0 || p.ox0 != 0) return false;
  for (int t = 0; t < 9; ++t)
    if (p.dy[t] != t / 3 - 1 || p.dx[t] != t % 3 - 1) return false;
  if (p.IH != p.OH || p.IW != p.OW || p.OHs != p.OH || p.OWs != p.OW) return false;
  if ((p.IH % TH != 0 || p.IW % TW != 0) && !pair_mode(p)) return false;
  if (p.Cin % 64 != 0 || p.N % 64 != 0 || p.K != 9 * p.Cin) return false;
  if (p.b_batch_stride != 0 || p.rows_per_batch != p.M) return false;
  if ((p.lda & 3) || (p.ldo & 3)) return false;
  if (p.stats && (p.cpg % 8 != 0)) return false;
  if (p.up2 && (p.stats != nullptr || p.N != 256)) return false;
  return true;
}

int launch_tc_conv3(const GemmParams& p, const float* Bimg, cudaStream_t st) {
  if (!tc_conv3_supported(p, EPI_PLAIN)) { set_last_error("launch_tc_conv3: unsupported geometry"); return -1; }
  if (pair_mode(p)) return launch_c3<64, true>(p, Bimg, st);
  if (tc_tile_n(p.N) == 128) return launch_c3<128, false>(p, Bimg, st);
  return launch_c3<64, false>(p, Bimg, st);
}

}
```

### dawn_pytorch_b200/csrc/tc_gemm.cuh

```cuda
#pragma once
#include <cuda_runtime.h>
#include <vector>
#include "gemm.cuh"

namespace dawn {

int tc_tile_n(int N);
bool tc_gemm_supported(const GemmParams& p, int epi);
size_t tc_pack_weights(const float* Bkn, int K, int N, int ldb, std::vector<float>& out, float* scale);
int launch_tc_gemm(const GemmParams& p, const float* Bimg, int epi, cudaStream_t st);
bool tc_conv3_supported(const GemmParams& p, int epi);
int launch_tc_conv3(const GemmParams& p, const float* Bimg, cudaStream_t st);

}
```

### dawn_pytorch_b200/csrc/unet.cu

```cuda
#include <dlfcn.h>
#include <algorithm>
#include <cmath>
#include <cstring>
#include <map>
#include <string>
#include <vector>

#include "../../include/dawn_unet.h"
#include "common.cuh"
#include "contraction.cuh"
#include "gemm.cuh"
#include "kernels.cuh"
#include "temporal_fused.cuh"
#include "sla_fused.cuh"
#include "ca_fused.cuh"
#include "sampler.cuh"

namespace dawn {

static thread_local std::string g_last_error;
void set_last_error(const std::string& s) { g_last_error = s; }

typedef struct ncclComm* ncclComm_t;
struct NcclUniqueId { char internal[128]; };
struct NcclApi {
  int (*GetUniqueId)(NcclUniqueId*) = nullptr;
  int (*CommInitRank)(ncclComm_t*, int, NcclUniqueId, int) = nullptr;
  int (*CommDestroy)(ncclComm_t) = nullptr;
  int (*AllReduce)(const void*, void*, size_t, int, int, ncclComm_t, cudaStream_t) = nullptr;
  int (*Send)(const void*, size_t, int, int, ncclComm_t, cudaStream_t) = nullptr;
  int (*Recv)(void*, size_t, int, int, ncclComm_t, cudaStream_t) = nullptr;
  int (*GroupStart)() = nullptr;
  int (*GroupEnd)() = nullptr;
  const char* (*GetErrorString)(int) = nullptr;
  bool ok = false;
};
constexpr int kNcclUint32 = 3, kNcclUint64 = 5, kNcclFloat32 = 7, kNcclFloat64 = 8, kNcclSum = 0, kNcclMin = 3;
static NcclApi g_nccl;
static int load_nccl() {
  if (g_nccl.ok) return 0;
  void* lib = dlopen("libnccl.so.2", RTLD_NOW | RTLD_GLOBAL);
  if (!lib) lib = dlopen("libnccl.so", RTLD_NOW | RTLD_GLOBAL);
  if (!lib) { set_last_error(std::string("cannot load libnccl.so.2: ") + dlerror()); return -1; }
#define DAWN_NCCL_SYM(field, name)                                                        \
  g_nccl.field = reinterpret_cast<decltype(g_nccl.field)>(dlsym(lib, name));              \
  if (!g_nccl.field) { set_last_error(std::string("libnccl lacks ") + name); return -1; }
  DAWN_NCCL_SYM(GetUniqueId, "ncclGetUniqueId")
  DAWN_NCCL_SYM(CommInitRank, "ncclCommInitRank")
  DAWN_NCCL_SYM(CommDestroy, "ncclCommDestroy")
  DAWN_NCCL_SYM(AllReduce, "ncclAllReduce")
  DAWN_NCCL_SYM(Send, "ncclSend")
  DAWN_NCCL_SYM(Recv, "ncclRecv")
  DAWN_NCCL_SYM(GroupStart, "ncclGroupStart")
  DAWN_NCCL_SYM(GroupEnd, "ncclGroupEnd")
  DAWN_NCCL_SYM(GetErrorString, "ncclGetErrorString")
#undef DAWN_NCCL_SYM
  g_nccl.ok = true;
  return 0;
}
#define DAWN_NCCL_OK(expr)                                                                                   \
  do {                                                                                                       \
    int _r = (expr);                                                                                         \
    if (_r != 0) { ::dawn::set_last_error(std::string(#expr) + ": " + g_nccl.GetErrorString(_r)); return -2; } \
  } while (0)

struct Act {
  float* p = nullptr; int ld = 0; int C = 0; int H = 0; int W = 0;
};

struct CrossAttnW { float *Wkv, *nkv, *qs, *ks, *Wout, *gout; };

struct ResBlockW {
  std::string name;
  int ci = 0, co = 0;
  bool cond = false, res = false;
  PackedWeight c1, c2, cres;
  float *gn1w = nullptr, *gn1b = nullptr, *gn2w = nullptr, *gn2b = nullptr;
  float *tW = nullptr, *tB = nullptr;
  float *mW[3] = {nullptr, nullptr, nullptr}, *mB[3] = {nullptr, nullptr, nullptr};
  PackedWeight wq; float* wsumq = nullptr;
  uint16_t* fWq = nullptr; float f_inv_wscale = 1.f;
  CrossAttnW ca[3];
  float *film = nullptr, *kq = nullptr, *nkq = nullptr, *T = nullptr, *G = nullptr;
  int ldbT = 0;
  int st1 = 0, st2 = 0;
};

struct AttnW {
  int C = 0; PackedWeight qkv, out; float* wsum = nullptr;
  uint16_t *fq = nullptr, *fo = nullptr; float f_inv_wscale = 1.f, f_inv_oscale = 1.f;
};
struct SlaW {
  int C = 0; PackedWeight qkv; float *wsum = nullptr, *WoutT = nullptr, *bout = nullptr;
  uint16_t* fkv = nullptr; float f_inv_wscale = 1.f;
  uint16_t* fq = nullptr; float fq_inv_wscale = 1.f;
};

}

using namespace dawn;

constexpr int kP2pMaxRanks = 8, kP2pSlots = 4;
struct P2pMail {
  double val[kP2pSlots][kP2pMaxRanks][16];
  unsigned int flag[kP2pSlots][kP2pMaxRanks];
};
struct P2pPeers { P2pMail* m[kP2pMaxRanks]; };

__global__ void gn_p2p_allreduce_kernel(double* __restrict__ stats, P2pPeers peers, int rank, int nranks, unsigned int* ctr) {
  const int lane = threadIdx.x;
  unsigned int seq = 0;
  if (lane == 0) seq = ++(*ctr);
  seq = __shfl_sync(0xffffffffu, seq, 0);
  const int slot = seq % kP2pSlots;
  if (lane < 16) {
    const double v = stats[lane];
    for (int r = 0; r < nranks; ++r) peers.m[r]->val[slot][rank][lane] = v;
  }
  __threadfence_system();
  __syncwarp();
  if (lane < nranks) {
    volatile unsigned int* f = &peers.m[lane]->flag[slot][rank];
    *f = seq;
  }
  P2pMail* mine = peers.m[rank];
  if (lane < nranks) {
    volatile unsigned int* f = &mine->flag[slot][lane];
    const long long t0 = clock64();
    while (*f != seq) {
      if (clock64() - t0 > 8000000000LL) break;
    }
  }
  __syncwarp();
  __threadfence_system();
  if (lane < 16) {
    double acc = 0.0;
    for (int r = 0; r < nranks; ++r) acc += *(volatile double*)&mine->val[slot][r][lane];
    stats[lane] = acc;
  }
}

struct SamplerGraph {
  cudaGraphExec_t exec = nullptr;
  int64_t launches = 0;
};

struct dawn_unet {
  dawn_unet_cfg cfg{};
  int nlev = 0;
  std::vector<int> dims;
  std::vector<std::pair<int, int>> in_out;
  int cond_dim = 0, tdim = 0;
  HostParams raw;
  bool committed = false;

  DeviceArena weights;
  DeviceArena workspace;
  PackedWeight init_full;
  float* init_w3 = nullptr;
  int cin_pad = 0;
  float *time_freqs = nullptr, *tW1 = nullptr, *tb1 = nullptr, *tW2 = nullptr, *tb2 = nullptr;
  float *rel_bias = nullptr, *rot_freqs = nullptr;
  std::vector<ResBlockW> rb;
  std::map<std::string, int> rb_index;
  AttnW init_ta, mid_sa, mid_ta;
  std::vector<AttnW> down_ta, up_ta;
  std::vector<SlaW> down_sla, up_sla;
  std::vector<PackedWeight> down_conv;
  std::vector<UpConv> up_conv;
  float *headW[2] = {nullptr, nullptr}, *headB[2] = {nullptr, nullptr};
  FilmDesc* film_descs = nullptr; int n_film = 0, film_max_n = 0;
  CondDesc* cond_descs = nullptr; int n_cond = 0, cond_max_n1 = 0, cond_max_k = 0, cond_max_co = 0;

  int B = 1, F = 0, H = 0, W = 0;
  std::vector<int> lH, lW;
  float* MAPPART = nullptr;
  int* VARY = nullptr;
  float *X288 = nullptr, *FEA288 = nullptr, *MAP = nullptr, *XR = nullptr, *S0 = nullptr;
  std::vector<float*> bufA, bufB, CAT, DS;
  float *Y = nullptr, *A1 = nullptr, *QKV = nullptr, *O = nullptr, *ROWSTATS = nullptr, *GATES = nullptr, *WT = nullptr;
  float *BF = nullptr, *HF = nullptr, *HO = nullptr, *ROT = nullptr, *TSILU = nullptr;
  float* UPPAD = nullptr;
  double* STATS = nullptr; int n_stats = 0;
  int64_t* T_HOSTSIDE = nullptr;
  float *H_XT = nullptr, *H_FEA = nullptr, *H_COND = nullptr, *H_OUT = nullptr;
  bool have_invariants = false;

  int sh_nranks = 1, sh_rank = 0, sh_Fglobal = 0, sh_halo_l = 0, sh_halo_r = 0;
  ncclComm_t sh_comm = nullptr;
  float* XE = nullptr;
  DeviceArena mailbox;
  P2pMail* p2p_own = nullptr;
  P2pMail* p2p_peer[kP2pMaxRanks] = {nullptr};
  unsigned int* p2p_ctr = nullptr;
  bool p2p_ready = false;

  std::map<std::string, float*> taps;
  int64_t launches = 0;

  SamplerGraph ddim_graph;
  SamplerGraph guided_graph;
  SamplerGraph ddpm_graph;
  cudaStream_t samp_stream = nullptr;

  bool prof_on = false;
  std::vector<cudaEvent_t> prof_ev;
  size_t prof_used = 0;
  struct ProfRec { int cat; double flops; double bytes; };
  std::vector<ProfRec> prof_recs;
  double prof_ms[DAWN_PROF_NCAT] = {0};
  double prof_flops[DAWN_PROF_NCAT] = {0};
  double prof_bytes[DAWN_PROF_NCAT] = {0};
  int64_t prof_cnt[DAWN_PROF_NCAT] = {0};
};

namespace {

int pack_conv(dawn_unet* h, const std::string& prefix, int co, int ci, int kh, int kw, int ci_pad, bool bias, PackedWeight* out) {
  const HostParam* w; const HostParam* b = nullptr;
  DAWN_TRY(h->raw.need(prefix + ".weight", {co, ci, 1, kh, kw}, &w));
  if (bias) DAWN_TRY(h->raw.need(prefix + ".bias", {co}, &b));
  const int ldb = round_up(co, 64);
  const int K = kh * kw * ci_pad;
  std::vector<float> m((size_t)K * ldb, 0.f);
  pack_conv_taps(w->data.data(), co, ci, kh * kw, ci_pad, ldb, 0, nullptr, m);
  return upload_weight(h->weights, m, K, co, ldb, b ? b->data : std::vector<float>{}, out);
}

int pack_linear(dawn_unet* h, const HostParam* w, int N, int K, const float* gain, float qscale, int nscale, PackedWeight* out,
                float** wsum) {
  const int ldb = round_up(N, 64);
  const std::vector<float> f = fold_linear(w->data.data(), N, K, gain, qscale, nscale);
  std::vector<float> m((size_t)K * ldb, 0.f), s = row_sums(f, N, K);
  for (int n = 0; n < N; ++n)
    for (int k = 0; k < K; ++k) m[(size_t)k * ldb + n] = f[(size_t)n * K + k];
  s.resize(ldb, 0.f);
  DAWN_TRY(upload_weight(h->weights, m, K, N, ldb, {}, out));
  if (wsum) DAWN_TRY(h->weights.upload(s, wsum));
  return 0;
}

int upload_raw(dawn_unet* h, const std::string& name, std::vector<int64_t> shape, float** out) {
  const HostParam* p;
  DAWN_TRY(h->raw.need(name, shape, &p));
  return h->weights.upload(p->data, out);
}

int pack_resblock(dawn_unet* h, const std::string& name, int ci, int co, bool cond, int* stat_counter) {
  ResBlockW r;
  r.name = name; r.ci = ci; r.co = co; r.cond = cond; r.res = (ci != co);
  DAWN_CHECK(ci % 32 == 0 && co % 64 == 0, "channel counts must be multiples of 64 (dim=64 family)");
  DAWN_TRY(pack_conv(h, name + ".block1.proj", co, ci, 3, 3, ci, true, &r.c1));
  DAWN_TRY(pack_conv(h, name + ".block2.proj", co, co, 3, 3, co, true, &r.c2));
  DAWN_TRY(upload_raw(h, name + ".block1.norm.weight", {co}, &r.gn1w));
  DAWN_TRY(upload_raw(h, name + ".block1.norm.bias", {co}, &r.gn1b));
  DAWN_TRY(upload_raw(h, name + ".block2.norm.weight", {co}, &r.gn2w));
  DAWN_TRY(upload_raw(h, name + ".block2.norm.bias", {co}, &r.gn2b));
  if (r.res) DAWN_TRY(pack_conv(h, name + ".res_conv", co, ci, 1, 1, ci, true, &r.cres));
  r.st1 = (*stat_counter)++;
  r.st2 = (*stat_counter)++;
  if (cond) {
    const int tdim = h->tdim;
    DAWN_TRY(upload_raw(h, name + ".time_mlp.1.weight", {2 * co, tdim}, &r.tW));
    DAWN_TRY(upload_raw(h, name + ".time_mlp.1.bias", {2 * co}, &r.tB));
    const char* mlp[3] = {"pose_mlp", "audio_mlp", "eye_mlp"};
    const int kdim[3] = {h->cfg.cond_pose, h->cfg.cond_aud, h->cfg.cond_eye};
    const char* can[3] = {"cross_attn_pose", "cross_attn_aud", "cross_attn_eye"};
    const float* to_q[3];
    const float* gain[3];
    for (int a = 0; a < 3; ++a) {
      DAWN_TRY(upload_raw(h, name + "." + mlp[a] + ".1.weight", {2 * co, kdim[a]}, &r.mW[a]));
      DAWN_TRY(upload_raw(h, name + "." + mlp[a] + ".1.bias", {2 * co}, &r.mB[a]));
      const std::string p = name + "." + can[a];
      const HostParam *g, *q;
      DAWN_TRY(h->raw.need(p + ".norm.g", {ci}, &g));
      DAWN_TRY(h->raw.need(p + ".to_q.weight", {64, ci}, &q));
      to_q[a] = q->data.data(); gain[a] = g->data.data();
      DAWN_TRY(upload_raw(h, p + ".to_kv.weight", {128, 2 * co}, &r.ca[a].Wkv));
      DAWN_TRY(upload_raw(h, p + ".null_kv", {2, 8}, &r.ca[a].nkv));
      DAWN_TRY(upload_raw(h, p + ".q_scale", {8}, &r.ca[a].qs));
      DAWN_TRY(upload_raw(h, p + ".k_scale", {8}, &r.ca[a].ks));
      DAWN_TRY(upload_raw(h, p + ".to_out.0.weight", {co, 64}, &r.ca[a].Wout));
      DAWN_TRY(upload_raw(h, p + ".to_out.1.g", {co}, &r.ca[a].gout));
    }
    std::vector<float> wq, wsum;
    fold_ca_q(to_q, gain, ci, wq, wsum);
    DAWN_TRY(upload_weight(h->weights, wq, ci, 192, 192, {}, &r.wq));
    DAWN_TRY(h->weights.upload(wsum, &r.wsumq));
    if (ci == 64 || ci == 128) {
      std::vector<uint16_t> W;
      ca_fused_pack(wq.data(), ci, W, &r.f_inv_wscale);
      DAWN_TRY(h->weights.upload(W, &r.fWq));
    }
  }
  h->rb_index[name] = (int)h->rb.size();
  h->rb.push_back(r);
  return 0;
}

int pack_attn(dawn_unet* h, const std::string& norm_name, const std::string& fn, int C, AttnW* a) {
  const HostParam *g, *qkv, *o;
  DAWN_TRY(h->raw.need(norm_name + ".gamma", {1, C, 1, 1, 1}, &g));
  DAWN_TRY(h->raw.need(fn + ".to_qkv.weight", {768, C}, &qkv));
  DAWN_TRY(h->raw.need(fn + ".to_out.weight", {C, 256}, &o));
  a->C = C;
  const float scale = 1.0f / sqrtf(32.0f);
  DAWN_TRY(pack_linear(h, qkv, 768, C, g->data.data(), scale, 256, &a->qkv, &a->wsum));
  DAWN_TRY(pack_linear(h, o, C, 256, nullptr, 1.f, 0, &a->out, nullptr));
  if (C == 64) {
    const std::vector<float> wq = fold_linear(qkv->data.data(), 768, C, g->data.data(), scale, 256);
    std::vector<uint16_t> Wq, Wo;
    temporal_fused_pack(wq.data(), o->data.data(), Wq, Wo, &a->f_inv_wscale, &a->f_inv_oscale);
    DAWN_TRY(h->weights.upload(Wq, &a->fq));
    DAWN_TRY(h->weights.upload(Wo, &a->fo));
  }
  return 0;
}

int pack_sla(dawn_unet* h, const std::string& p, int C, SlaW* s) {
  const HostParam *g, *qkv, *o, *b;
  DAWN_TRY(h->raw.need(p + ".norm.gamma", {1, C, 1, 1, 1}, &g));
  DAWN_TRY(h->raw.need(p + ".fn.to_qkv.weight", {768, C, 1, 1}, &qkv));
  DAWN_TRY(h->raw.need(p + ".fn.to_out.weight", {C, 256, 1, 1}, &o));
  DAWN_TRY(h->raw.need(p + ".fn.to_out.bias", {C}, &b));
  s->C = C;
  DAWN_TRY(pack_linear(h, qkv, 768, C, g->data.data(), 1.f, 0, &s->qkv, &s->wsum));
  if (C == 64) {
    const std::vector<float> wf = fold_linear(qkv->data.data(), 768, C, g->data.data(), 1.f, 0);
    std::vector<uint16_t> W;
    sla_fused_pack(wf.data(), W, &s->f_inv_wscale);
    DAWN_TRY(h->weights.upload(W, &s->fkv));
    sla_out_pack(wf.data(), W, &s->fq_inv_wscale);
    DAWN_TRY(h->weights.upload(W, &s->fq));
  }
  std::vector<float> wt((size_t)256 * C);
  for (int c = 0; c < C; ++c)
    for (int k = 0; k < 256; ++k) wt[(size_t)k * C + c] = o->data[(size_t)c * 256 + k];
  DAWN_TRY(h->weights.upload(wt, &s->WoutT));
  std::vector<float> bb(round_up(C, 64), 0.f);
  std::copy(b->data.begin(), b->data.end(), bb.begin());
  DAWN_TRY(h->weights.upload(bb, &s->bout));
  return 0;
}

static const int kUpK[2][2] = {{1, 3}, {0, 2}};
static const int kUpD[2][2] = {{0, -1}, {1, 0}};
int pack_up(dawn_unet* h, const std::string& name, int C, UpConv* u) {
  const HostParam *w, *b;
  DAWN_TRY(h->raw.need(name + ".weight", {C, C, 1, 4, 4}, &w));
  DAWN_TRY(h->raw.need(name + ".bias", {C}, &b));
  return dawn::pack_up(h->weights, C, C, kUpD, b->data, [&](int py, int px, int ty, int tx, int c, int n) {
    return w->data[(((size_t)c * C + n) * 4 + kUpK[py][ty]) * 4 + kUpK[px][tx]];
  }, u);
}

int pack_upconv(dawn_unet* h, const std::string& name, int C, UpConv* u) {
  const HostParam *w, *b;
  DAWN_TRY(h->raw.need(name + ".1.weight", {C, C, 1, 3, 3}, &w));
  DAWN_TRY(h->raw.need(name + ".1.bias", {C}, &b));
  return pack_up_nearest(h->weights, w->data.data(), C, C, nullptr, b->data, u);
}

void base_params(GemmParams& p, const Act& in, int F) { dawn::base_params(p, in.p, in.ld, in.C, F, in.H, in.W); }


enum ProfCat : int {
  PC_CONV3 = 0,
  PC_CONV_OTHER,
  PC_QKV,
  PC_OUTPROJ,
  PC_CA_GATE,
  PC_GN_HCOND,
  PC_ATTN_CORE,
  PC_SLA_CTX,
  PC_GN_APPLY,
  PC_ROWSTATS,
  PC_CA_RSTD,
  PC_MISC,
  PC_PREP,
  PC_TEMPORAL_L0,
  PC_CONV3_L0,
  PC_COMM_AR,
  PC_COMM_HALO,
  PC_COUNT
};
static_assert(PC_COUNT <= DAWN_PROF_NCAT, "increase DAWN_PROF_NCAT");

struct Ctx {
  dawn_unet* h; cudaStream_t st;
  int gemm(const GemmParams& p, int epi, int cat);
};

struct ProfScope {
  dawn_unet* h; cudaStream_t st; bool on;
  ProfScope(Ctx& c, int cat, double flops, double bytes) : h(c.h), st(c.st), on(c.h->prof_on) {
    h->launches++;
    if (!on) return;
    while (h->prof_ev.size() < h->prof_used + 2) {
      cudaEvent_t e; cudaEventCreate(&e); h->prof_ev.push_back(e);
    }
    h->prof_recs.push_back({cat, flops, bytes});
    cudaEventRecord(h->prof_ev[h->prof_used], st);
  }
  ~ProfScope() {
    if (!on) return;
    cudaEventRecord(h->prof_ev[h->prof_used + 1], st);
    h->prof_used += 2;
  }
};

int Ctx::gemm(const GemmParams& p, int epi, int cat) {
  const double flops = 2.0 * p.M * (double)p.N * (p.up2 ? p.K / 9 * 4 : p.K);
  double bytes = 4.0 * p.M * ((double)p.Cin * (p.in_stride == 1 ? 1 : 4) + p.N);
  if (p.Res) bytes += 4.0 * p.M * p.N;
  if (p.Y) bytes += 4.0 * p.M * p.N;
  if (epi == EPI_CA_GATE) bytes = 4.0 * p.M * (p.Cin + 24.0);
  ProfScope ps(*this, cat, flops, bytes);
  const size_t scratch = (size_t)(h->F * h->B + 2 * h->cfg.win_width) * h->lH[0] * h->lW[0] * 256 * sizeof(float);
  int kernels = 0;
  const int rc = launch_path(p, epi, choose_path(p, epi, scratch), h->O, st, &kernels);
  h->launches += kernels - 1;
  return rc;
}

int tap(Ctx& c, const std::string& name, const Act& a);

int ln_gemm(Ctx& c, GemmParams& p, int epi, int cat, const float* x, int ldx, int C, int rows) {
  dawn_unet* h = c.h;
  p.ln_inline = 0; p.rowstats = h->ROWSTATS;
  const bool tc_ok = path_ok(p, epi, DAWN_PATH_TC_GEMM, 0) && p.ntaps == 1;
  if (tc_ok && (p.N >= 384 || (p.N == 192 && p.Cin >= 256)) && p.Cin % 64 == 0) {
    p.want_split = 1;
    ProfScope ps(c, PC_ROWSTATS, 0, 4.0 * rows * C);
    DAWN_TRY(launch_rowstats(x, ldx, C, rows, 1e-5f, h->ROWSTATS, c.st));
  } else if (tc_ok) {
    p.ln_inline = 1; p.rowstats = nullptr;
  } else {
    ProfScope ps(c, PC_ROWSTATS, 0, 4.0 * rows * C);
    DAWN_TRY(launch_rowstats(x, ldx, C, rows, 1e-5f, h->ROWSTATS, c.st));
  }
  return c.gemm(p, epi, cat);
}

double* stats_slot(dawn_unet* h, int slot) { return h->STATS + (size_t)16 * h->B * slot; }

GemmParams conv_same_params(Ctx& c, const Act& in, const PackedWeight& w, int k, const Act& out, int stat_slot) {
  GemmParams p; base_params(p, in, c.h->F * c.h->B);
  set_weights(p, w); set_square_taps(p, k, k / 2);
  p.Out = out.p; p.ldo = out.ld;
  if (stat_slot >= 0) { p.stats = stats_slot(c.h, stat_slot); p.cpg = w.N / 8; p.clips = c.h->B; }
  return p;
}
int conv_same(Ctx& c, const GemmParams& p) {
  const bool l0 = p.IH == c.h->lH[0] && p.Cin == c.h->cfg.dim && p.N == c.h->cfg.dim;
  return c.gemm(p, EPI_PLAIN, p.ntaps == 9 ? (l0 ? PC_CONV3_L0 : PC_CONV3) : PC_CONV_OTHER);
}

int gn_allreduce(Ctx& c, int slot) {
  dawn_unet* h = c.h;
  if (h->sh_nranks <= 1) return 0;
  double* st = stats_slot(h, slot);
  ProfScope ps(c, PC_COMM_AR, 0, 128.0 * h->sh_nranks);
  if (h->p2p_ready) {
    P2pPeers pp;
    for (int r = 0; r < kP2pMaxRanks; ++r) pp.m[r] = h->p2p_peer[r];
    gn_p2p_allreduce_kernel<<<1, 32, 0, c.st>>>(st, pp, h->sh_rank, h->sh_nranks, h->p2p_ctr);
    DAWN_LAUNCH_OK();
    return 0;
  }
  DAWN_NCCL_OK(g_nccl.AllReduce(st, st, 16, kNcclFloat64, kNcclSum, h->sh_comm, c.st));
  return 0;
}

int resblock(Ctx& c, const ResBlockW& r, const Act& x, const Act& out) {
  dawn_unet* h = c.h;
  const int F = h->F * h->B, M = F * x.H * x.W, P = x.H * x.W;
  DAWN_CHECK(x.C == r.ci && out.C == r.co, "resblock channel mismatch: " + r.name);
  Act y{h->Y, r.co, r.co, x.H, x.W}, a1{h->A1, r.co, r.co, x.H, x.W};
  const double count = (double)h->sh_Fglobal * P * (r.co / 8);
  if (r.cond && r.fWq && ca_fused_supported(r.ci, P)) {
    CaFusedArgs a{};
    a.x = x.p; a.ldx = x.ld; a.F = F; a.P = P; a.Wq = r.fWq; a.inv_wscale = r.f_inv_wscale;
    a.kq = r.kq; a.nkq = r.nkq; a.G = r.G; a.Wt = h->WT;
    ProfScope ps(c, PC_CA_GATE, 2.0 * M * r.ci * 192, 4.0 * M * (r.ci + 32));
    DAWN_TRY(launch_ca_fused(a, r.ci, c.st));
  } else if (r.cond) {
    GemmParams p; base_params(p, x, F);
    set_weights(p, r.wq);
    p.wsum = r.wsumq; p.kq = r.kq; p.nkq = r.nkq; p.gates = h->GATES;
    DAWN_TRY(ln_gemm(c, p, EPI_CA_GATE, PC_CA_GATE, x.p, x.ld, x.C, M));
    ProfScope ps(c, PC_CA_RSTD, 0, 4.0 * M * 56);
    DAWN_TRY(launch_ca_rstd(h->GATES, r.G, M, P, h->WT, c.st));
  }
  DAWN_TRY(conv_same(c, conv_same_params(c, x, r.c1, 3, y, r.st1)));
  DAWN_TRY(gn_allreduce(c, r.st1));
  GemmParams conv2 = conv_same_params(c, a1, r.c2, 3, y, r.st2);
  if (r.cond && gn_hcond_supported(r.co, P) && path_ok(conv2, EPI_PLAIN, DAWN_PATH_TC_CONV3, 0)) {
    conv2.A16h = reinterpret_cast<const unsigned short*>(h->A1);
    conv2.A16l = conv2.A16h + (size_t)M * r.co;
  }
  if (r.cond && gn_hcond_supported(r.co, P)) {
    GnHcondArgs a{};
    a.Wt = h->WT; a.T = r.T; a.ldbT = r.ldbT; a.Y = y.p; a.ldy = y.ld; a.Out = a1.p; a.ldo = a1.ld;
    a.Out16h = const_cast<unsigned short*>(conv2.A16h); a.Out16l = const_cast<unsigned short*>(conv2.A16l);
    a.F = F; a.P = P; a.co = r.co; a.clips = h->B;
    a.gn_stats = stats_slot(h, r.st1); a.gn_count = count; a.cpg = r.co / 8;
    a.gn_w = r.gn1w; a.gn_b = r.gn1b; a.film = r.film;
    ProfScope ps(c, PC_GN_HCOND, 2.0 * M * 32 * r.co, 4.0 * M * (2.0 * r.co + 32));
    DAWN_TRY(launch_gn_hcond(a, c.st));
  } else if (r.cond) {
    Act wt{h->WT, 32, 32, x.H, x.W};
    GemmParams p; base_params(p, wt, F);
    p.B = r.T; p.ldb = r.ldbT; p.b_batch_stride = (long long)32 * r.ldbT; p.N = r.co; p.K = 32;
    p.rows_per_batch = P;
    p.Out = a1.p; p.ldo = a1.ld;
    p.Y = y.p; p.ldy = y.ld; p.gn_stats = stats_slot(h, r.st1); p.gn_w = r.gn1w; p.gn_b = r.gn1b;
    p.film = r.film; p.gn_count = count; p.cpg = r.co / 8; p.clips = h->B;
    DAWN_TRY(c.gemm(p, EPI_GN_APPLY, PC_GN_HCOND));
  } else {
    ProfScope ps(c, PC_GN_APPLY, 0, 8.0 * M * r.co);
    DAWN_TRY(launch_gn_apply(y.p, y.ld, r.co, M, stats_slot(h, r.st1), count, r.co / 8, P, h->B, r.gn1w, r.gn1b, nullptr,
                             nullptr, 0, a1.p, a1.ld, c.st));
  }
  DAWN_TRY(conv_same(c, conv2));
  DAWN_TRY(gn_allreduce(c, r.st2));
  const float* res = x.p; int ldr = x.ld;
  if (r.res) {
    DAWN_TRY(conv_same(c, conv_same_params(c, x, r.cres, 1, out, -1)));
    res = out.p; ldr = out.ld;
  }
  {
  ProfScope ps(c, PC_GN_APPLY, 0, 12.0 * M * r.co);
  DAWN_TRY(launch_gn_apply(y.p, y.ld, r.co, M, stats_slot(h, r.st2), count, r.co / 8, P, h->B, r.gn2w, r.gn2b, nullptr,
                           res, ldr, out.p, out.ld, c.st));
  }
  return tap(c, r.name, out);
}

inline int seq_block(int P) { for (int b = 16; b > 1; --b) if (P % b == 0) return b; return 1; }

int temporal_attn(Ctx& c, const AttnW& w, const Act& x, const Act& dst, const std::string& name) {
  dawn_unet* h = c.h;
  const int F = h->F, P = h->B * x.H * x.W;
  const int pb = seq_block(P);
  const int hl = h->sh_halo_l, hr = h->sh_halo_r, Fe = hl + F + hr;
  const int Me = Fe * P;
  Act xe = x;
  if (h->sh_nranks > 1) {
    const size_t rowb = (size_t)x.C * sizeof(float);
    float* mid = h->XE + (size_t)hl * P * x.C;
    ProfScope ps(c, PC_COMM_HALO, 0, 4.0 * (2.0 * F + 2.0 * (hl + hr)) * P * x.C);
    DAWN_CUDA_OK(cudaMemcpy2DAsync(mid, rowb, x.p, (size_t)x.ld * sizeof(float), rowb, (size_t)F * P, cudaMemcpyDeviceToDevice, c.st));
    const size_t hcount = (size_t)h->cfg.win_width * P * x.C;
    DAWN_NCCL_OK(g_nccl.GroupStart());
    if (h->sh_rank > 0) {
      DAWN_NCCL_OK(g_nccl.Send(mid, hcount, kNcclFloat32, h->sh_rank - 1, h->sh_comm, c.st));
      DAWN_NCCL_OK(g_nccl.Recv(h->XE, hcount, kNcclFloat32, h->sh_rank - 1, h->sh_comm, c.st));
    }
    if (h->sh_rank < h->sh_nranks - 1) {
      DAWN_NCCL_OK(g_nccl.Send(mid + (size_t)(F - h->cfg.win_width) * P * x.C, hcount, kNcclFloat32, h->sh_rank + 1, h->sh_comm, c.st));
      DAWN_NCCL_OK(g_nccl.Recv(mid + (size_t)F * P * x.C, hcount, kNcclFloat32, h->sh_rank + 1, h->sh_comm, c.st));
    }
    DAWN_NCCL_OK(g_nccl.GroupEnd());
    xe = Act{h->XE, x.C, x.C, x.H, x.W};
  }
  const bool fused_ok = w.fq && temporal_fused_supported(x.C, Fe, h->cfg.win_width, hl, hl + F);
  if (fused_ok) {
    TemporalFusedArgs a{};
    a.x = xe.p; a.ldx = xe.ld; a.res = x.p; a.ldr = x.ld; a.out = dst.p; a.ldo = dst.ld;
    a.F = Fe; a.P = P; a.q_lo = hl; a.q_hi = hl + F;
    a.Wqkv = w.fq; a.Wout = w.fo; a.wsum = w.wsum; a.rot = h->ROT; a.bias = h->rel_bias; a.band = h->cfg.win_width;
    a.inv_wscale = w.f_inv_wscale; a.inv_oscale = w.f_inv_oscale;
    double pairs = 0;
    for (int i = hl; i < hl + F; ++i) pairs += std::min(Fe - 1, i + a.band) - std::max(0, i - a.band) + 1;
    ProfScope ps(c, x.H == h->lH[0] ? PC_TEMPORAL_L0 : PC_ATTN_CORE, 2.0 * Me * x.C * 768 + 4.0 * 32 * 8 * P * pairs + 2.0 * F * P * 256 * x.C,
                 4.0 * (Me + 2.0 * F * P) * x.C);
    DAWN_TRY(launch_temporal_fused(a, c.st));
    return tap(c, name, dst);
  }
  {
    GemmParams p; base_params(p, xe, Fe * h->B);
    set_weights(p, w.qkv);
    p.P = P;
    p.wsum = w.wsum; p.rot = h->ROT;
    p.Out = h->QKV; p.ldo = 768;
    p.perm_pb = pb; p.perm_F = Fe; p.perm_in = 1; p.perm_out = 0;
    p.OH = Me; p.OW = 1; p.OHs = Me; p.OWs = 1; p.IH = Me; p.IW = 1;
    DAWN_TRY(ln_gemm(c, p, EPI_QKV_TEMPORAL, PC_QKV, xe.p, xe.ld, xe.C, Me));
  }
  {
    AttnArgs a{};
    a.qkv = h->QKV; a.ld = 768; a.out = h->O; a.ldo = 256;
    a.nseq = P; a.L = Fe; a.seq_base_stride = 1; a.elem_stride = P; a.pb = pb;
    a.band = h->cfg.win_width; a.bias = h->rel_bias; a.q_lo = hl; a.q_hi = hl + F;
    double pairs = 0;
    for (int i = hl; i < hl + F; ++i) pairs += std::min(Fe - 1, i + a.band) - std::max(0, i - a.band) + 1;
    ProfScope ps(c, PC_ATTN_CORE, 4.0 * 32 * 8 * P * pairs, 4.0 * Me * 1024);
    if (attention_tc_supported(a)) DAWN_TRY(launch_attention_tc(a, c.st));
    else DAWN_TRY(launch_attention(a, c.st));
  }
  {
    Act o{h->O, 256, 256, Me, 1};
    GemmParams p; base_params(p, o, 1);
    set_weights(p, w.out);
    p.P = P;
    p.perm_pb = pb; p.perm_F = Fe; p.perm_in = 0; p.perm_out = 1; p.perm_f_lo = hl; p.perm_f_hi = hl + F;
    p.Res = x.p; p.ldr = x.ld; p.Out = dst.p; p.ldo = dst.ld;
    DAWN_TRY(c.gemm(p, EPI_PLAIN, PC_OUTPROJ));
  }
  return tap(c, name, dst);
}

int mid_spatial_attn(Ctx& c, const AttnW& w, const Act& x, const std::string& name) {
  dawn_unet* h = c.h;
  const int F = h->F * h->B, P = x.H * x.W, M = F * P;
  {
    GemmParams p; base_params(p, x, F);
    set_weights(p, w.qkv);
    p.wsum = w.wsum;
    p.Out = h->QKV; p.ldo = 768;
    DAWN_TRY(ln_gemm(c, p, EPI_QKV_MID, PC_QKV, x.p, x.ld, x.C, M));
  }
  {
    AttnArgs a{};
    a.qkv = h->QKV; a.ld = 768; a.out = h->O; a.ldo = 256;
    a.nseq = F; a.L = P; a.seq_base_stride = P; a.elem_stride = 1;
    a.band = 1 << 30; a.bias = nullptr; a.q_lo = 0; a.q_hi = P;
    ProfScope ps(c, PC_ATTN_CORE, 4.0 * 32 * 8 * (double)F * P * P, 4.0 * M * 1024);
    if (attention_tc_supported(a)) DAWN_TRY(launch_attention_tc(a, c.st));
    else DAWN_TRY(launch_attention(a, c.st));
  }
  {
    Act o{h->O, 256, 256, x.H, x.W};
    GemmParams p; base_params(p, o, F);
    set_weights(p, w.out);
    p.Res = x.p; p.ldr = x.ld; p.Out = x.p; p.ldo = x.ld;
    DAWN_TRY(c.gemm(p, EPI_PLAIN, PC_OUTPROJ));
  }
  return tap(c, name, x);
}

int sla(Ctx& c, const SlaW& w, const Act& x, const std::string& name) {
  dawn_unet* h = c.h;
  const int F = h->F * h->B, P = x.H * x.W, M = F * P;
  const int ldb = round_up(x.C, 64);
  const bool fused = w.fkv && sla_fused_supported(x.C, P) &&
                     sla_fused_part_floats(F, P) <= (size_t)(F + 2 * h->cfg.win_width) * h->lH[0] * h->lW[0] * 256;
  const int qld = fused ? 256 : 768;
  if (fused) {
    SlaCtxArgs a{};
    a.x = x.p; a.ldx = x.ld; a.F = F; a.P = P; a.Wkv = w.fkv; a.inv_wscale = w.f_inv_wscale; a.part = h->O;
    {
      ProfScope ps(c, PC_SLA_CTX, 2.0 * M * x.C * 512 + 2.0 * 8 * 32 * 32 * M + 2.0 * F * 256 * 32 * x.C, 4.0 * M * x.C);
      h->launches++;
      DAWN_TRY(launch_sla_ctx_fused(a, w.WoutT, h->BF, ldb, c.st));
    }
    SlaOutArgs o{};
    o.x = x.p; o.ldx = x.ld; o.out = x.p; o.ldo = x.ld; o.F = F; o.P = P; o.Wq = w.fq; o.inv_wscale = w.fq_inv_wscale;
    o.Bf = h->BF; o.ldb = ldb; o.bias = w.bout;
    ProfScope ps2(c, PC_OUTPROJ, 2.0 * M * x.C * 256 + 2.0 * M * 256 * x.C, 8.0 * M * x.C);
    DAWN_TRY(launch_sla_out_fused(o, c.st));
    return tap(c, name, x);
  } else {
    GemmParams p; base_params(p, x, F);
    set_weights(p, w.qkv);
    p.wsum = w.wsum; p.q_post_scale = 1.0f / sqrtf(32.0f);
    p.Out = h->QKV; p.ldo = 768;
    DAWN_TRY(ln_gemm(c, p, EPI_QKV_SLA, PC_QKV, x.p, x.ld, x.C, M));
  }
  if (!fused) {
    ProfScope ps(c, PC_SLA_CTX, 2.0 * 8 * 32 * 32 * M + 2.0 * F * 256 * 32 * x.C, 4.0 * M * 768);
    DAWN_TRY(launch_sla_context(h->QKV, 768, F, P, w.WoutT, x.C, h->BF, ldb, c.st));
  }
  {
    Act q{h->QKV, qld, 256, x.H, x.W};
    GemmParams p; base_params(p, q, F);
    p.B = h->BF; p.ldb = ldb; p.b_batch_stride = (long long)256 * ldb; p.N = x.C; p.K = 256;
    p.rows_per_batch = P; p.bias = w.bout;
    p.Res = x.p; p.ldr = x.ld; p.Out = x.p; p.ldo = x.ld;
    DAWN_TRY(c.gemm(p, EPI_PLAIN, PC_OUTPROJ));
  }
  return tap(c, name, x);
}

int downsample(Ctx& c, const PackedWeight& w, const Act& x, const Act& out, const std::string& name) {
  GemmParams p; base_params(p, x, c.h->F * c.h->B);
  set_weights(p, w);
  p.OHs = out.H; p.OWs = out.W; p.in_stride = 2;
  set_square_taps(p, 4, 1);
  p.M = c.h->F * c.h->B * out.H * out.W; p.rows_per_batch = p.M;
  p.OH = out.H; p.OW = out.W; p.P = out.H * out.W;
  p.Out = out.p; p.ldo = out.ld;
  DAWN_TRY(c.gemm(p, EPI_PLAIN, PC_CONV_OTHER));
  return tap(c, name, out);
}

int upsample(Ctx& c, const UpConv& u, const Act& x, const Act& out, const std::string& name) {
  dawn_unet* h = c.h;
  const int NF = h->F * h->B;
  auto run = [&](const GemmParams& q) { return c.gemm(q, EPI_PLAIN, PC_CONV_OTHER); };
  GemmParams p;
  if (h->cfg.pad_mode == 0) {
    base_params(p, x, NF);
    DAWN_TRY(run_up(p, u, out.p, out.ld, run));
    return tap(c, name, out);
  }
  {
    const double px = (double)NF * x.C;
    ProfScope ps(c, PC_CONV_OTHER, 0, 4.0 * px * ((double)x.H * x.W + (x.H + 2.0) * (x.W + 2)));
    DAWN_TRY(launch_pad_border(x.p, x.ld, x.C, NF, x.H, x.W, h->cfg.pad_mode == 3, h->UPPAD, c.st));
  }
  base_params(p, h->UPPAD, x.C, x.C, NF, x.H + 2, x.W + 2);
  p.OHs = x.H; p.OWs = x.W; p.OH = x.H; p.OW = x.W; p.P = x.H * x.W;
  p.M = NF * x.H * x.W; p.rows_per_batch = p.M;
  DAWN_TRY(run_up(p, u, out.p, out.ld, run, 1));
  return tap(c, name, out);
}

__global__ void nhwc_to_ncf_kernel(const float* __restrict__ x, int ld, int C, long long M, float* __restrict__ out) {
  const long long idx = (long long)blockIdx.x * blockDim.x + threadIdx.x;
  if (idx >= M * C) return;
  const long long m = idx / C; const int ch = (int)(idx - m * C);
  out[(size_t)ch * M + m] = x[(size_t)m * ld + ch];
}
int tap(Ctx& c, const std::string& name, const Act& a) {
  auto it = c.h->taps.find(name);
  if (it == c.h->taps.end() || it->second == nullptr) return 0;
  const long long M = (long long)c.h->F * a.H * a.W;
  nhwc_to_ncf_kernel<<<(int)((M * a.C + 255) / 256), 256, 0, c.st>>>(a.p, a.ld, a.C, M, it->second);
  DAWN_LAUNCH_OK();
  return 0;
}

int prep_cond(dawn_unet* h, const float* cond, cudaStream_t st) {
  if (h->n_cond == 0) return 0;
  Ctx c{h, st};
  ProfScope ps(c, PC_PREP, 0, 0);
  h->launches += 2;
  return launch_cond_batched(cond, h->cond_dim, h->cond_descs, h->n_cond, h->cond_max_n1, h->cond_max_k, h->cond_max_co, h->F * h->B,
                             h->B, st);
}

int init_map(dawn_unet* h, const float* fea, long long cstride, long long clip_stride, cudaStream_t st, const int* skip_flag,
             int skip_if) {
  Ctx c{h, st};
  const int H0 = h->lH[0], W0 = h->lW[0], dim = h->cfg.dim, k = h->cfg.init_kernel_size;
  {
    ProfScope ps(c, PC_PREP, 0, 0);
    DAWN_TRY(launch_fea_shift_nhwc(fea, cstride, clip_stride, h->B, h->cfg.channels - 3, H0, W0, h->cin_pad, 3, k, h->FEA288, st,
                                   skip_flag, skip_if));
  }
  {
    Act in{h->FEA288, h->cin_pad, h->cin_pad, H0, W0};
    GemmParams p; base_params(p, in, k * h->B);
    set_weights(p, h->init_full);
    p.ntaps = k;
    for (int kx = 0; kx < k; ++kx) { p.dy[kx] = 0; p.dx[kx] = (signed char)(kx - k / 2); }
    p.K = k * h->cin_pad; p.rows_per_batch = h->B * H0 * W0; p.b_batch_stride = (long long)k * h->cin_pad * h->init_full.ldb;
    p.bias = nullptr;
    p.Out = h->MAPPART; p.ldo = dim;
    p.skip_flag = skip_flag; p.skip_if = skip_if;
    ProfScope ps(c, PC_PREP, 0, 0);
    DAWN_TRY(launch_path(p, EPI_PLAIN, DAWN_PATH_MMA_SYNC, nullptr, st));
  }
  ProfScope ps(c, PC_PREP, 0, 0);
  return launch_map_reduce(h->MAPPART, k, (long long)h->B * H0 * W0 * dim, h->init_full.b, dim, h->MAP, st, skip_flag, skip_if);
}

int forward_core(dawn_unet* h, const int64_t* t_dev, int t_stride, float* out, cudaStream_t st) {
  Ctx c{h, st};
  const int F = h->F * h->B, nlev = h->nlev, dim = h->cfg.dim;
  DAWN_CUDA_OK(cudaMemsetAsync(h->STATS, 0, sizeof(double) * 16 * h->B * h->n_stats, st));
  {
    ProfScope ps(c, PC_MISC, 0, 0);
    h->launches += 1;
    DAWN_TRY(launch_time_mlp(t_dev, t_stride, h->B, h->time_freqs, dim, h->tW1, h->tb1, h->tW2, h->tb2, h->TSILU, st));
    DAWN_TRY(launch_film(h->film_descs, h->n_film, h->film_max_n, h->B, h->TSILU, h->tdim, st));
  }

  const int H0 = h->lH[0], W0 = h->lW[0];
  Act r{h->XR + dim, 2 * dim, dim, H0, W0};
  DAWN_TRY(tap(c, "init_conv", r));
  Act s0{h->S0, dim, dim, H0, W0};
  DAWN_TRY(temporal_attn(c, h->init_ta, r, s0, "init_temporal_attn"));

  Act x = s0;
  for (int L = 0; L < nlev; ++L) {
    const int co = h->in_out[L].second;
    Act a{h->bufA[L], co, co, h->lH[L], h->lW[L]}, b{h->bufB[L], co, co, h->lH[L], h->lW[L]};
    Act skip{h->CAT[L] + co, 2 * co, co, h->lH[L], h->lW[L]};
    const std::string pre = "downs." + std::to_string(L);
    DAWN_TRY(resblock(c, h->rb[h->rb_index[pre + ".0"]], x, a));
    DAWN_TRY(resblock(c, h->rb[h->rb_index[pre + ".1"]], a, b));
    if (!h->cfg.no_sla) DAWN_TRY(sla(c, h->down_sla[L], b, pre + ".2"));
    DAWN_TRY(temporal_attn(c, h->down_ta[L], b, skip, pre + ".3"));
    if (L < nlev - 1) {
      Act d{h->DS[L + 1], co, co, h->lH[L + 1], h->lW[L + 1]};
      DAWN_TRY(downsample(c, h->down_conv[L], skip, d, pre + ".4"));
      x = d;
    } else {
      x = skip;
    }
  }
  {
    const int L = nlev - 1, cm = h->in_out[L].second;
    Act a{h->bufA[L], cm, cm, h->lH[L], h->lW[L]};
    Act xfirst{h->CAT[L], 2 * cm, cm, h->lH[L], h->lW[L]};
    DAWN_TRY(resblock(c, h->rb[h->rb_index["mid_block1"]], x, a));
    DAWN_TRY(mid_spatial_attn(c, h->mid_sa, a, "mid_spatial_attn"));
    DAWN_TRY(temporal_attn(c, h->mid_ta, a, a, "mid_temporal_attn"));
    DAWN_TRY(resblock(c, h->rb[h->rb_index["mid_block2"]], a, xfirst));
  }
  for (int K = 0; K < nlev; ++K) {
    const int l = nlev - 1 - K;
    const int ci = h->in_out[l].first, co = h->in_out[l].second;
    Act cat{h->CAT[l], 2 * co, 2 * co, h->lH[l], h->lW[l]};
    Act a{h->bufA[l], ci, ci, h->lH[l], h->lW[l]}, b{h->bufB[l], ci, ci, h->lH[l], h->lW[l]};
    const std::string pre = "ups." + std::to_string(K);
    DAWN_TRY(resblock(c, h->rb[h->rb_index[pre + ".0"]], cat, a));
    DAWN_TRY(resblock(c, h->rb[h->rb_index[pre + ".1"]], a, b));
    if (!h->cfg.no_sla) DAWN_TRY(sla(c, h->up_sla[K], b, pre + ".2"));
    if (K < nlev - 1) {
      DAWN_TRY(temporal_attn(c, h->up_ta[K], b, b, pre + ".3"));
      const int cn = h->in_out[l - 1].second;
      Act up{h->CAT[l - 1], 2 * cn, cn, h->lH[l - 1], h->lW[l - 1]};
      DAWN_TRY(upsample(c, h->up_conv[K], b, up, pre + ".4"));
    } else {
      Act xf{h->XR, 2 * dim, dim, H0, W0};
      DAWN_TRY(temporal_attn(c, h->up_ta[K], b, xf, pre + ".3"));
    }
  }
  Act xr{h->XR, 2 * dim, 2 * dim, H0, W0};
  Act hf{h->HF, dim, dim, H0, W0}, ho{h->HO, dim, dim, H0, W0};
  DAWN_TRY(resblock(c, h->rb[h->rb_index["final_conv.0"]], xr, hf));
  DAWN_TRY(resblock(c, h->rb[h->rb_index["occlusion_map.0"]], xr, ho));
  ProfScope ps(c, PC_MISC, 0, 4.0 * F * H0 * W0 * (2 * dim + 3));
  DAWN_TRY(launch_heads_out(h->HF, h->HO, dim, F * H0 * W0, H0 * W0, h->B, h->headW[0], h->headB[0], h->cfg.out_grid_dim,
                            h->headW[1], h->headB[1], h->cfg.out_conf_dim, out, st));
  return 0;
}

}

extern "C" {

const char* dawn_last_error(void) { return g_last_error.c_str(); }
int64_t dawn_live_bytes(void) { return dawn::DeviceArena::live_bytes(); }
const char* dawn_build_info(void) { return "dawn_unet sm_90a; contractions: wgmma m64n64k16 FP16x3 (register accumulators, RN fp32 drains) + mma.sync m16n8k16 FP16x3 fused attention kernels; fallback mma.sync 3xTF32"; }

int dawn_check_single_device(void) {
  static int first_dev = -1;
  int dev = -1;
  if (cudaGetDevice(&dev) != cudaSuccess) { cudaGetLastError(); return 0; }
  if (first_dev < 0) first_dev = dev;
  if (dev != first_dev) {
    set_last_error("this process already uses CUDA device " + std::to_string(first_dev) + "; the library supports one GPU per process "
                   "(launch one rank per GPU), got device " + std::to_string(dev));
    return -1;
  }
  return 0;
}

int dawn_unet_create(const dawn_unet_cfg* cfg, dawn_unet** out) {
  DAWN_CHECK(cfg && out, "null argument");
  DAWN_TRY(dawn_check_single_device());
  DAWN_CHECK(cfg->attn_heads == 8 && cfg->attn_dim_head == 32, "only attn_heads=8, attn_dim_head=32 are supported");
  DAWN_CHECK(cfg->resnet_groups == 8, "only resnet_groups=8 is supported");
  DAWN_CHECK(cfg->dim == 64 || cfg->dim == 128, "dim must be 64 or 128");
  DAWN_CHECK(cfg->n_levels >= 2 && cfg->n_levels <= 6, "n_levels out of range");
  DAWN_CHECK(cfg->init_kernel_size == 7 || cfg->init_kernel_size == 5 || cfg->init_kernel_size == 3, "init kernel must be 3, 5 or 7");
  DAWN_CHECK(cfg->win_width >= 1 && cfg->win_width <= 120, "win_width out of range");
  DAWN_CHECK(cfg->upconv == 0 || cfg->upconv == 1, "upconv must be 0 (ConvTranspose3d) or 1 (nearest x2 + 3x3 conv)");
  DAWN_CHECK(cfg->pad_mode >= 0 && cfg->pad_mode <= 3, "pad_mode must be 0 (zeros), 1 (reflect), 2 (replicate) or 3 (circular)");
  DAWN_CHECK(cfg->pad_mode == 0 || cfg->upconv == 1, "pad_mode applies to the upconv variant only (upconv = 1)");
  DAWN_CHECK(cfg->no_sla == 0 || cfg->no_sla == 1, "no_sla must be 0 or 1");
  dawn_unet* h = new dawn_unet();
  h->cfg = *cfg;
  h->nlev = cfg->n_levels;
  h->dims.push_back(cfg->dim);
  for (int i = 0; i < cfg->n_levels; ++i) h->dims.push_back(cfg->dim * cfg->dim_mults[i]);
  for (int i = 0; i < cfg->n_levels; ++i) h->in_out.push_back({h->dims[i], h->dims[i + 1]});
  for (auto& io : h->in_out)
    if (io.second < 1 || io.second > 1024) { delete h; set_last_error("dim * dim_mults[i] must be in [1, 1024] for every level"); return -1; }
  h->cond_dim = cfg->cond_aud + cfg->cond_pose + cfg->cond_eye;
  h->tdim = 4 * cfg->dim;
  h->cin_pad = round_up(cfg->channels, 32);
  *out = h;
  return 0;
}

static void drop_graph(SamplerGraph& g) {
  if (g.exec) { cudaGraphExecDestroy(g.exec); g.exec = nullptr; }
}
static void drop_graphs(dawn_unet* h) {
  drop_graph(h->ddim_graph);
  drop_graph(h->ddpm_graph);
  drop_graph(h->guided_graph);
}

void dawn_unet_destroy(dawn_unet* h) {
  if (!h) return;
  for (cudaEvent_t e : h->prof_ev) cudaEventDestroy(e);
  drop_graphs(h);
  if (h->samp_stream) cudaStreamDestroy(h->samp_stream);
  if (h->sh_comm && g_nccl.ok) g_nccl.CommDestroy(h->sh_comm);
  for (int r = 0; r < kP2pMaxRanks; ++r)
    if (h->p2p_peer[r] && h->p2p_peer[r] != h->p2p_own) cudaIpcCloseMemHandle(h->p2p_peer[r]);
  delete h;
}

int dawn_unet_set_param(dawn_unet* h, const char* name, const float* host, const int64_t* shape, int ndim) {
  DAWN_CHECK(h && name && host && (shape || ndim == 0), "null argument");
  h->raw.set(name, host, shape, ndim);
  h->committed = false;
  return 0;
}

int dawn_unet_commit_params(dawn_unet* h) {
  DAWN_CHECK(h, "null handle");
  drop_graphs(h);
  h->weights.release();
  h->rb.clear(); h->rb_index.clear();
  h->down_ta.clear(); h->up_ta.clear(); h->down_sla.clear(); h->up_sla.clear(); h->down_conv.clear(); h->up_conv.clear();
  const auto& cfg = h->cfg;
  const int dim = cfg.dim, nlev = h->nlev, k = cfg.init_kernel_size;
  DAWN_TRY(pack_conv(h, "init_conv", dim, cfg.channels, k, k, h->cin_pad, true, &h->init_full));
  {
    const HostParam* w;
    DAWN_TRY(h->raw.need("init_conv.weight", {dim, cfg.channels, 1, k, k}, &w));
    std::vector<float> w3((size_t)k * k * 3 * dim);
    for (int t = 0; t < k * k; ++t)
      for (int c = 0; c < 3; ++c)
        for (int n = 0; n < dim; ++n) w3[((size_t)t * 3 + c) * dim + n] = w->data[((size_t)n * cfg.channels + c) * k * k + t];
    DAWN_TRY(h->weights.upload(w3, &h->init_w3));
  }
  DAWN_TRY(upload_raw(h, "aux.time_freqs", {dim / 2}, &h->time_freqs));
  DAWN_TRY(upload_raw(h, "aux.rel_bias", {8, 2 * cfg.win_width + 1}, &h->rel_bias));
  DAWN_TRY(upload_raw(h, "time_mlp.1.weight", {h->tdim, dim}, &h->tW1));
  DAWN_TRY(upload_raw(h, "time_mlp.1.bias", {h->tdim}, &h->tb1));
  DAWN_TRY(upload_raw(h, "time_mlp.3.weight", {h->tdim, h->tdim}, &h->tW2));
  DAWN_TRY(upload_raw(h, "time_mlp.3.bias", {h->tdim}, &h->tb2));
  DAWN_TRY(upload_raw(h, "init_temporal_attn.fn.fn.fn.rotary_emb.freqs", {16}, &h->rot_freqs));
  DAWN_TRY(pack_attn(h, "init_temporal_attn.fn.norm", "init_temporal_attn.fn.fn.fn", dim, &h->init_ta));
  int stat_counter = 0;
  for (int L = 0; L < nlev; ++L) {
    const int ci = h->in_out[L].first, co = h->in_out[L].second;
    const std::string pre = "downs." + std::to_string(L);
    DAWN_TRY(pack_resblock(h, pre + ".0", ci, co, true, &stat_counter));
    DAWN_TRY(pack_resblock(h, pre + ".1", co, co, true, &stat_counter));
    if (!cfg.no_sla) { SlaW s; DAWN_TRY(pack_sla(h, pre + ".2.fn", co, &s)); h->down_sla.push_back(s); }
    AttnW a; DAWN_TRY(pack_attn(h, pre + ".3.fn.norm", pre + ".3.fn.fn.fn", co, &a)); h->down_ta.push_back(a);
    if (L < nlev - 1) {
      PackedWeight d; DAWN_TRY(pack_conv(h, pre + ".4", co, co, 4, 4, co, true, &d)); h->down_conv.push_back(d);
    }
  }
  const int mid = h->dims.back();
  DAWN_TRY(pack_resblock(h, "mid_block1", mid, mid, true, &stat_counter));
  DAWN_TRY(pack_attn(h, "mid_spatial_attn.fn.norm", "mid_spatial_attn.fn.fn.fn", mid, &h->mid_sa));
  DAWN_TRY(pack_attn(h, "mid_temporal_attn.fn.norm", "mid_temporal_attn.fn.fn.fn", mid, &h->mid_ta));
  DAWN_TRY(pack_resblock(h, "mid_block2", mid, mid, true, &stat_counter));
  for (int K = 0; K < nlev; ++K) {
    const int l = nlev - 1 - K;
    const int ci = h->in_out[l].first, co = h->in_out[l].second;
    const std::string pre = "ups." + std::to_string(K);
    DAWN_TRY(pack_resblock(h, pre + ".0", 2 * co, ci, true, &stat_counter));
    DAWN_TRY(pack_resblock(h, pre + ".1", ci, ci, true, &stat_counter));
    if (!cfg.no_sla) { SlaW s; DAWN_TRY(pack_sla(h, pre + ".2.fn", ci, &s)); h->up_sla.push_back(s); }
    AttnW a; DAWN_TRY(pack_attn(h, pre + ".3.fn.norm", pre + ".3.fn.fn.fn", ci, &a)); h->up_ta.push_back(a);
    if (K < nlev - 1) {
      UpConv u; DAWN_TRY(cfg.upconv ? pack_upconv(h, pre + ".4", ci, &u) : pack_up(h, pre + ".4", ci, &u)); h->up_conv.push_back(u);
    }
  }
  DAWN_TRY(pack_resblock(h, "final_conv.0", 2 * dim, dim, false, &stat_counter));
  DAWN_TRY(pack_resblock(h, "occlusion_map.0", 2 * dim, dim, false, &stat_counter));
  DAWN_TRY(upload_raw(h, "final_conv.1.weight", {cfg.out_grid_dim, dim, 1, 1, 1}, &h->headW[0]));
  DAWN_TRY(upload_raw(h, "final_conv.1.bias", {cfg.out_grid_dim}, &h->headB[0]));
  DAWN_TRY(upload_raw(h, "occlusion_map.1.weight", {cfg.out_conf_dim, dim, 1, 1, 1}, &h->headW[1]));
  DAWN_TRY(upload_raw(h, "occlusion_map.1.bias", {cfg.out_conf_dim}, &h->headB[1]));
  h->n_stats = stat_counter;
  h->committed = true;
  h->have_invariants = false;
  if (h->F > 0) return dawn_unet_set_geometry(h, h->B, h->F, h->H, h->W);
  return 0;
}

int dawn_unet_set_num_frames(dawn_unet* h, int F, int height, int width) { return dawn_unet_set_geometry(h, 1, F, height, width); }

int dawn_unet_set_geometry(dawn_unet* h, int B, int F, int height, int width) {
  DAWN_CHECK(h, "null handle");
  drop_graphs(h);
  DAWN_CHECK(h->committed, "commit_params must precede set_geometry");
  DAWN_CHECK(F >= 1 && F <= 65535, "F out of range");
  DAWN_CHECK(B >= 1 && B <= kMaxClips, "the clip count B must be in [1, " + std::to_string(kMaxClips) + "]");
  DAWN_CHECK((int64_t)B * F <= 65535, "B * F out of range");
  DAWN_CHECK(B == 1 || h->sh_nranks <= 1, "a frame-sharded handle runs one clip at a time (B = 1)");
  DAWN_CHECK(B == 1 || h->taps.empty(), "debugging taps need B = 1: clear them before setting B > 1");
  const int nlev = h->nlev, dim = h->cfg.dim;
  const int div = 1 << (nlev - 1);
  DAWN_CHECK(height % div == 0 && width % div == 0 && height >= div && width >= div,
             "latent height/width must be divisible by 2^(levels-1)");
  h->workspace.release();
  h->have_invariants = false;
  h->B = B; h->F = F; h->H = height; h->W = width;
  h->lH.assign(nlev, 0); h->lW.assign(nlev, 0);
  for (int l = 0; l < nlev; ++l) { h->lH[l] = height >> l; h->lW[l] = width >> l; }
  auto& ws = h->workspace;
  const int NF = B * F;
  const size_t P0 = (size_t)height * width, M0 = (size_t)NF * P0;
  DAWN_TRY(ws.alloc(M0 * h->cin_pad, &h->X288));
  DAWN_TRY(ws.alloc(B * P0 * h->cin_pad * h->cfg.init_kernel_size, &h->FEA288));
  DAWN_TRY(ws.alloc(B * P0 * dim * h->cfg.init_kernel_size, &h->MAPPART));
  DAWN_TRY(ws.alloc(B + 4, &h->VARY));
  DAWN_TRY(ws.alloc(B * P0 * dim, &h->MAP));
  DAWN_TRY(ws.alloc(M0 * 2 * dim, &h->XR));
  DAWN_TRY(ws.alloc(M0 * dim, &h->S0));
  h->bufA.assign(nlev, nullptr); h->bufB.assign(nlev, nullptr); h->CAT.assign(nlev, nullptr); h->DS.assign(nlev, nullptr);
  size_t max_mc = 0, max_bf = 0, max_pc = P0 * dim;
  for (int l = 0; l < nlev; ++l) {
    const size_t Ml = (size_t)NF * h->lH[l] * h->lW[l];
    const int ci = h->in_out[l].first, co = h->in_out[l].second;
    const int cw = std::max(ci, co);
    DAWN_TRY(ws.alloc(Ml * cw, &h->bufA[l]));
    DAWN_TRY(ws.alloc(Ml * cw, &h->bufB[l]));
    DAWN_TRY(ws.alloc(Ml * 2 * co, &h->CAT[l]));
    if (l > 0) DAWN_TRY(ws.alloc(Ml * ci, &h->DS[l]));
    max_mc = std::max(max_mc, Ml * cw);
    max_bf = std::max(max_bf, (size_t)NF * 256 * round_up(cw, 64));
    max_pc = std::max(max_pc, (size_t)h->lH[l] * h->lW[l] * cw);
  }
  if (h->cfg.pad_mode != 0) {
    size_t n = 0;
    for (int l = 1; l < nlev; ++l) n = std::max(n, (size_t)NF * (h->lH[l] + 2) * (h->lW[l] + 2) * h->in_out[l].first);
    DAWN_TRY(ws.alloc(n, &h->UPPAD));
  }
  max_mc = std::max(max_mc, M0 * dim);
  DAWN_TRY(ws.alloc(max_mc, &h->Y));
  DAWN_TRY(ws.alloc(max_mc, &h->A1));
  const size_t Mext = (size_t)(NF + 2 * h->cfg.win_width) * P0;
  DAWN_TRY(ws.alloc(Mext * 768, &h->QKV));
  DAWN_TRY(ws.alloc(Mext * 256, &h->O));
  DAWN_TRY(ws.alloc(Mext * 2, &h->ROWSTATS));
  DAWN_TRY(ws.alloc((size_t)(NF + 2 * h->cfg.win_width) * max_pc, &h->XE));
  DAWN_TRY(ws.alloc(M0 * 24, &h->GATES));
  DAWN_TRY(ws.alloc(M0 * 32, &h->WT));
  DAWN_TRY(ws.alloc(max_bf, &h->BF));
  DAWN_TRY(ws.alloc(M0 * dim, &h->HF));
  DAWN_TRY(ws.alloc(M0 * dim, &h->HO));
  DAWN_TRY(ws.alloc((size_t)(F + 2 * h->cfg.win_width) * 32, &h->ROT));
  DAWN_TRY(ws.alloc((size_t)B * h->tdim, &h->TSILU));
  DAWN_TRY(ws.alloc((size_t)h->n_stats * 16 * B, &h->STATS));
  DAWN_TRY(ws.alloc(2, &h->T_HOSTSIDE));
  DAWN_TRY(ws.alloc(3 * M0, &h->H_XT));
  DAWN_TRY(ws.alloc((size_t)(h->cfg.channels - 3) * P0, &h->H_FEA));
  DAWN_TRY(ws.alloc((size_t)F * h->cond_dim, &h->H_COND));
  DAWN_TRY(ws.alloc((size_t)(h->cfg.out_grid_dim + h->cfg.out_conf_dim) * M0, &h->H_OUT));
  std::vector<FilmDesc> descs;
  for (auto& r : h->rb) {
    if (!r.cond) continue;
    r.ldbT = round_up(r.co, 64);
    DAWN_TRY(ws.alloc((size_t)B * 2 * r.co, &r.film));
    DAWN_TRY(ws.alloc((size_t)NF * 3 * 64, &r.kq));
    DAWN_TRY(ws.alloc(24, &r.nkq));
    DAWN_TRY(ws.alloc((size_t)NF * 32 * r.ldbT, &r.T));
    DAWN_CUDA_OK(cudaMemset(r.T, 0, (size_t)NF * 32 * r.ldbT * sizeof(float)));
    DAWN_TRY(ws.alloc((size_t)NF * 3 * 81, &r.G));
    descs.push_back(FilmDesc{r.tW, r.tB, r.film, 2 * r.co});
  }
  {
    DAWN_TRY(ws.upload(descs, &h->film_descs));
    h->n_film = (int)descs.size();
    h->film_max_n = 0;
    for (const auto& fd : descs) h->film_max_n = std::max(h->film_max_n, fd.n);
  }
  {
    const int off[3] = {h->cfg.cond_aud, 0, h->cfg.cond_aud + h->cfg.cond_pose};
    const int kd[3] = {h->cfg.cond_pose, h->cfg.cond_aud, h->cfg.cond_eye};
    std::vector<CondDesc> cd;
    h->cond_max_n1 = h->cond_max_k = h->cond_max_co = 0;
    for (auto& r : h->rb) {
      if (!r.cond) continue;
      for (int a = 0; a < 3; ++a) {
        CondDesc d{};
        d.mW = r.mW[a]; d.mB = r.mB[a]; d.off = off[a]; d.K = kd[a]; d.n1 = 2 * r.co; d.Wkv = r.ca[a].Wkv;
        DAWN_TRY(ws.alloc((size_t)NF * d.n1, &d.ctx));
        DAWN_TRY(ws.alloc((size_t)NF * 128, &d.kv));
        d.t.kv = d.kv; d.t.nkv = r.ca[a].nkv; d.t.qs = r.ca[a].qs; d.t.ks = r.ca[a].ks; d.t.Wout = r.ca[a].Wout; d.t.gout = r.ca[a].gout;
        d.t.co = r.co; d.t.ldbT = r.ldbT; d.t.ca = a; d.t.kq = r.kq; d.t.nkq = r.nkq; d.t.T = r.T; d.t.G = r.G;
        cd.push_back(d);
        h->cond_max_n1 = std::max(h->cond_max_n1, d.n1); h->cond_max_k = std::max(h->cond_max_k, d.K); h->cond_max_co = std::max(h->cond_max_co, r.co);
      }
    }
    DAWN_TRY(ws.upload(cd, &h->cond_descs));
    h->n_cond = (int)cd.size();
  }
  h->sh_nranks = 1; h->sh_rank = 0; h->sh_Fglobal = F; h->sh_halo_l = 0; h->sh_halo_r = 0;
  h->p2p_ready = false;
  DAWN_TRY(launch_rotary_table(h->rot_freqs, 16, F, 0, h->ROT, 0));
  DAWN_CUDA_OK(cudaDeviceSynchronize());
  return 0;
}

int dawn_unet_set_clip_invariants(dawn_unet* h, const float* fea, const float* cond, void* stream) {
  DAWN_CHECK(h && fea && cond, "null argument");
  DAWN_CHECK(h->F > 0, "set_num_frames must precede set_clip_invariants");
  cudaStream_t st = (cudaStream_t)stream;
  const long long P0 = (long long)h->lH[0] * h->lW[0];
  DAWN_TRY(init_map(h, fea, P0, (h->cfg.channels - 3) * P0, st, nullptr, 0));
  DAWN_TRY(prep_cond(h, cond, st));
  h->have_invariants = true;
  return 0;
}

int dawn_unet_forward(dawn_unet* h, const float* x, const int64_t* t, const float* cond, float* out, void* stream) {
  DAWN_CHECK(h && x && t && cond && out, "null argument");
  DAWN_CHECK(h->F > 0, "set_num_frames must precede forward");
  DAWN_CHECK(h->B == 1 || h->taps.empty(), "debugging taps need B = 1");
  cudaStream_t st = (cudaStream_t)stream;
  h->launches = 0;
  Ctx c{h, st};
  const int H0 = h->lH[0], W0 = h->lW[0], dim = h->cfg.dim, k = h->cfg.init_kernel_size, B = h->B, NF = h->B * h->F;
  DAWN_TRY(prep_cond(h, cond, st));
  h->have_invariants = false;
  const int* vary = h->VARY;
  const int* n_vary = h->VARY + B;
  {
    ProfScope ps(c, PC_MISC, 0, 4.0 * NF * H0 * W0 * h->cfg.channels);
    DAWN_TRY(launch_frame_invariance(x, 3, h->cfg.channels, h->F, H0 * W0, B, h->VARY, st));
  }
  {
    ProfScope ps(c, PC_MISC, 0, 8.0 * NF * H0 * W0 * h->cin_pad);
    DAWN_TRY(launch_ncf_to_nhwc(x, h->cfg.channels, h->F, H0 * W0, h->cin_pad, 0, h->X288, st, n_vary, 0, B));
  }
  {
    Act in{h->X288, h->cin_pad, h->cin_pad, H0, W0};
    GemmParams p; base_params(p, in, NF);
    set_weights(p, h->init_full); set_square_taps(p, k, k / 2);
    p.Out = h->XR + dim; p.ldo = 2 * dim;
    p.skip_flag = n_vary; p.skip_if = 0;
    ProfScope ps(c, PC_CONV_OTHER, 2.0 * p.M * (double)p.N * p.K, 4.0 * p.M * ((double)p.Cin + p.N));
    DAWN_TRY(launch_path(p, EPI_PLAIN, DAWN_PATH_MMA_SYNC, nullptr, st));
  }
  const long long clip_in = (long long)h->cfg.channels * h->F * H0 * W0;
  DAWN_TRY(init_map(h, x + (size_t)3 * h->F * H0 * W0, (long long)h->F * H0 * W0, clip_in, st, n_vary, B));
  {
    const double k2 = (double)k * k;
    ProfScope ps(c, PC_MISC, 2.0 * NF * H0 * W0 * dim * 3 * k2, 4.0 * NF * H0 * W0 * (dim + 3));
    DAWN_TRY(launch_init_conv_x3(x, clip_in, h->F, H0, W0, B, h->init_w3, h->MAP, dim, h->XR + dim, 2 * dim, k, st, vary, 1));
  }
  return forward_core(h, t, 1, out, st);
}

static int forward_x3_impl(dawn_unet* h, const float* x_t, const int64_t* t, int t_stride, float* out, cudaStream_t st) {
  DAWN_CHECK(h && x_t && t && out, "null argument");
  DAWN_CHECK(h->F > 0 && h->have_invariants, "set_clip_invariants must precede forward_x3");
  DAWN_CHECK(h->B == 1 || h->taps.empty(), "debugging taps need B = 1");
  h->launches = 0;
  const int H0 = h->lH[0], W0 = h->lW[0], dim = h->cfg.dim, NF = h->B * h->F;
  {
    Ctx c{h, st};
    const double k2 = (double)h->cfg.init_kernel_size * h->cfg.init_kernel_size;
    ProfScope ps(c, PC_MISC, 2.0 * NF * H0 * W0 * dim * 3 * k2, 4.0 * NF * H0 * W0 * (dim + 3));
    DAWN_TRY(launch_init_conv_x3(x_t, 3LL * h->F * H0 * W0, h->F, H0, W0, h->B, h->init_w3, h->MAP, dim, h->XR + dim, 2 * dim,
                                 h->cfg.init_kernel_size, st));
  }
  return forward_core(h, t, t_stride, out, st);
}

int dawn_unet_forward_x3(dawn_unet* h, const float* x_t, const int64_t* t, float* out, void* stream) {
  return forward_x3_impl(h, x_t, t, 1, out, (cudaStream_t)stream);
}

int dawn_unet_forward_host(dawn_unet* h, const float* x_t, const float* fea, const float* cond, int64_t t, float* out) {
  DAWN_CHECK(h && x_t && fea && cond && out, "null argument");
  DAWN_CHECK(h->F > 0, "set_num_frames must precede forward_host");
  DAWN_CHECK(h->B == 1, "forward_host runs one clip: set_geometry with B = 1 (use the device entries for a batch)");
  cudaStream_t st = 0;
  const size_t M0 = (size_t)h->F * h->H * h->W, P0 = (size_t)h->H * h->W;
  const size_t nout = (size_t)(h->cfg.out_grid_dim + h->cfg.out_conf_dim) * M0;
  DAWN_CUDA_OK(cudaMemcpyAsync(h->H_XT, x_t, 3 * M0 * sizeof(float), cudaMemcpyHostToDevice, st));
  DAWN_CUDA_OK(cudaMemcpyAsync(h->H_FEA, fea, (size_t)(h->cfg.channels - 3) * P0 * sizeof(float), cudaMemcpyHostToDevice, st));
  DAWN_CUDA_OK(cudaMemcpyAsync(h->H_COND, cond, (size_t)h->F * h->cond_dim * sizeof(float), cudaMemcpyHostToDevice, st));
  DAWN_CUDA_OK(cudaMemcpyAsync(h->T_HOSTSIDE, &t, sizeof(int64_t), cudaMemcpyHostToDevice, st));
  DAWN_TRY(dawn_unet_set_clip_invariants(h, h->H_FEA, h->H_COND, st));
  const int64_t prep_launches = h->launches;
  DAWN_TRY(forward_x3_impl(h, h->H_XT, h->T_HOSTSIDE, 1, h->H_OUT, st));
  h->launches += prep_launches;
  DAWN_CUDA_OK(cudaMemcpyAsync(out, h->H_OUT, nout * sizeof(float), cudaMemcpyDeviceToHost, st));
  DAWN_CUDA_OK(cudaStreamSynchronize(st));
  return 0;
}

int dawn_unet_tap_shape(dawn_unet* h, const char* name, int* C, int* hl, int* wl) {
  DAWN_CHECK(h && name && C && hl && wl && h->F > 0, "bad argument");
  const std::string n(name);
  const int nlev = h->nlev, dim = h->cfg.dim;
  auto set = [&](int c, int l) { *C = c; *hl = h->lH[l]; *wl = h->lW[l]; return 0; };
  if (n == "init_conv" || n == "init_temporal_attn" || n == "final_conv.0" || n == "occlusion_map.0") return set(dim, 0);
  if (n.rfind("mid_", 0) == 0) return set(h->dims.back(), nlev - 1);
  int L = -1, j = -1;
  if ((sscanf(name, "downs.%d.%d", &L, &j) == 2 || sscanf(name, "ups.%d.%d", &L, &j) == 2) && j == 2)
    DAWN_CHECK(!h->cfg.no_sla, "no such tap: the network has no spatial linear attention");
  if (sscanf(name, "downs.%d.%d", &L, &j) == 2 && L >= 0 && L < nlev) {
    if (j == 4) { DAWN_CHECK(L < nlev - 1, "no such tap"); return set(h->in_out[L].second, L + 1); }
    return set(h->in_out[L].second, L);
  }
  if (sscanf(name, "ups.%d.%d", &L, &j) == 2 && L >= 0 && L < nlev) {
    const int l = nlev - 1 - L;
    if (j == 4) { DAWN_CHECK(L < nlev - 1, "no such tap"); return set(h->in_out[l].first, l - 1); }
    return set(h->in_out[l].first, l);
  }
  set_last_error("unknown tap: " + n);
  return -1;
}

int dawn_unet_set_tap(dawn_unet* h, const char* name, float* dst) {
  DAWN_CHECK(h && name, "null argument");
  DAWN_CHECK(!dst || h->B == 1, "debugging taps need B = 1 (set_geometry with one clip)");
  if (dst) h->taps[name] = dst; else h->taps.erase(name);
  return 0;
}

int dawn_nccl_unique_id(char* out128) {
  DAWN_CHECK(out128, "null argument");
  DAWN_TRY(load_nccl());
  NcclUniqueId id;
  DAWN_NCCL_OK(g_nccl.GetUniqueId(&id));
  memcpy(out128, id.internal, 128);
  return 0;
}

int dawn_unet_init_shard(dawn_unet* h, const char* id128, int nranks, int rank, int F_global) {
  DAWN_CHECK(h && id128, "null argument");
  DAWN_CHECK(h->F > 0, "set_num_frames (with the LOCAL frame count) must precede init_shard");
  DAWN_CHECK(nranks >= 1 && rank >= 0 && rank < nranks, "bad rank");
  DAWN_CHECK(F_global == h->F * nranks, "F_global must equal nranks * local frames (equal contiguous frame ranges)");
  DAWN_CHECK(nranks == 1 || h->F >= h->cfg.win_width, "each rank must own at least win_width frames (only neighbours exchange halos)");
  DAWN_CHECK(nranks == 1 || h->B == 1, "frame sharding runs one clip at a time: set_geometry with B = 1 before init_shard");
  drop_graphs(h);
  if (nranks > 1) {
    DAWN_TRY(load_nccl());
    if (h->sh_comm) { g_nccl.CommDestroy(h->sh_comm); h->sh_comm = nullptr; }
    NcclUniqueId id;
    memcpy(id.internal, id128, 128);
    DAWN_NCCL_OK(g_nccl.CommInitRank(&h->sh_comm, nranks, id, rank));
  }
  h->sh_nranks = nranks; h->sh_rank = rank; h->sh_Fglobal = F_global;
  h->p2p_ready = false;
  h->sh_halo_l = (rank > 0) ? h->cfg.win_width : 0;
  h->sh_halo_r = (rank < nranks - 1) ? h->cfg.win_width : 0;
  const int pos0 = rank * h->F - h->sh_halo_l;
  DAWN_TRY(launch_rotary_table(h->rot_freqs, 16, h->sh_halo_l + h->F + h->sh_halo_r, pos0, h->ROT, 0));
  DAWN_CUDA_OK(cudaDeviceSynchronize());
  return 0;
}

int dawn_unet_shard_ipc_export(dawn_unet* h, char* out64) {
  DAWN_CHECK(h && out64, "null argument");
  DAWN_CHECK(h->sh_nranks > 1 && h->sh_nranks <= kP2pMaxRanks, "init_shard (2..8 ranks) must precede shard_ipc_export");
  if (!h->p2p_own) {
    DAWN_TRY(h->mailbox.alloc(1, &h->p2p_own));
    DAWN_TRY(h->mailbox.alloc(4, &h->p2p_ctr));
  }
  DAWN_CUDA_OK(cudaMemset(h->p2p_own, 0, sizeof(P2pMail)));
  DAWN_CUDA_OK(cudaMemset(h->p2p_ctr, 0, 16));
  DAWN_CUDA_OK(cudaDeviceSynchronize());
  cudaIpcMemHandle_t hd;
  DAWN_CUDA_OK(cudaIpcGetMemHandle(&hd, h->p2p_own));
  static_assert(sizeof(hd) == 64, "cudaIpcMemHandle_t is 64 bytes");
  memcpy(out64, &hd, 64);
  h->p2p_ready = false;
  return 0;
}
int dawn_unet_shard_ipc_import(dawn_unet* h, const char* handles) {
  DAWN_CHECK(h && handles, "null argument");
  DAWN_CHECK(h->p2p_own && h->sh_nranks > 1 && h->sh_nranks <= kP2pMaxRanks, "shard_ipc_export must precede shard_ipc_import");
  for (int r = 0; r < h->sh_nranks; ++r) {
    if (r == h->sh_rank) { h->p2p_peer[r] = h->p2p_own; continue; }
    if (h->p2p_peer[r]) { cudaIpcCloseMemHandle(h->p2p_peer[r]); h->p2p_peer[r] = nullptr; }
    cudaIpcMemHandle_t hd;
    memcpy(&hd, handles + 64 * r, 64);
    void* ptr = nullptr;
    DAWN_CUDA_OK(cudaIpcOpenMemHandle(&ptr, hd, cudaIpcMemLazyEnablePeerAccess));
    h->p2p_peer[r] = reinterpret_cast<P2pMail*>(ptr);
  }
  h->p2p_ready = true;
  drop_graphs(h);
  return 0;
}

static int red_sum_u32(void* ctx, unsigned int* b, size_t n, cudaStream_t st) {
  DAWN_NCCL_OK(g_nccl.AllReduce(b, b, n, kNcclUint32, kNcclSum, (ncclComm_t)ctx, st)); return 0;
}
static int red_sum_u64(void* ctx, unsigned long long* b, size_t n, cudaStream_t st) {
  DAWN_NCCL_OK(g_nccl.AllReduce(b, b, n, kNcclUint64, kNcclSum, (ncclComm_t)ctx, st)); return 0;
}
static int red_min_u32(void* ctx, unsigned int* b, size_t n, cudaStream_t st) {
  DAWN_NCCL_OK(g_nccl.AllReduce(b, b, n, kNcclUint32, kNcclMin, (ncclComm_t)ctx, st)); return 0;
}

}

template <class Step>
static int update_clips(dawn_unet* h, int64_t n_local, Step step) {
  if (h->sh_nranks <= 1 || !h->sh_comm) {
    DAWN_CHECK(n_local % h->B == 0, "n must be a multiple of the clip count");
    const int64_t nc = n_local / h->B;
    for (int b = 0; b < h->B; ++b) DAWN_TRY(step(b * nc, nc, nc, nullptr));
    return 0;
  }
  DdimReduce red{(void*)h->sh_comm, red_sum_u32, red_sum_u64, red_min_u32};
  return step(0, n_local, n_local * h->sh_nranks, &red);
}

static int64_t clip_values(const dawn_unet* h) {
  return (int64_t)(h->cfg.out_grid_dim + h->cfg.out_conf_dim) * h->F * h->H * h->W;
}

template <class Body>
static int capture_graph(dawn_unet* h, SamplerGraph& g, const char* entry, const char* graph, Body body) {
  DAWN_CHECK(h->F > 0 && h->have_invariants, std::string("set_clip_invariants must precede ") + entry);
  DAWN_CHECK(!h->prof_on, std::string("disable profiling before capturing ") + graph);
  drop_graph(g);
  if (!h->samp_stream) DAWN_CUDA_OK(cudaStreamCreateWithFlags(&h->samp_stream, cudaStreamNonBlocking));
  DAWN_CUDA_OK(cudaStreamBeginCapture(h->samp_stream, cudaStreamCaptureModeThreadLocal));
  const int64_t launches = body(h->samp_stream);
  cudaGraph_t captured = nullptr;
  const cudaError_t e = cudaStreamEndCapture(h->samp_stream, &captured);
  if (launches < 0) { if (captured) cudaGraphDestroy(captured); return (int)launches; }
  DAWN_CUDA_OK(e);
  const cudaError_t ei = cudaGraphInstantiate(&g.exec, captured, 0);
  cudaGraphDestroy(captured);
  DAWN_CUDA_OK(ei);
  g.launches = launches;
  return 0;
}

static int launch_graph(dawn_unet* h, SamplerGraph dawn_unet::*slot, const char* entry, const char* launch, void* stream) {
  DAWN_CHECK(h && (h->*slot).exec, std::string(entry) + " must precede " + launch + " (a geometry change drops the graph)");
  DAWN_CHECK(h->have_invariants, std::string("set_clip_invariants must precede ") + launch);
  const SamplerGraph& g = h->*slot;
  DAWN_CUDA_OK(cudaGraphLaunch(g.exec, (cudaStream_t)stream));
  h->launches = g.launches;
  return 0;
}

extern "C" {

int dawn_unet_ddim_step(dawn_unet* h, float* x, const float* eps, const float* noise, int64_t n_local, float ca, float cb,
                        float sqrt_an, float c, float sigma, float q, void* scratch, void* stream) {
  DAWN_CHECK(h, "null handle");
  return update_clips(h, n_local, [&](int64_t o, int64_t n, int64_t n_global, const DdimReduce* red) {
    return ddim_step_impl(x + o, eps + o, noise ? noise + o : nullptr, n, n_global, ca, cb, sqrt_an, c, sigma, q, scratch,
                          (cudaStream_t)stream, red);
  });
}

int dawn_unet_sampler_capture(dawn_unet* h, float* x, float* eps, const float* noise_all, const int64_t* t_all,
                              const float* coef, int nsteps, float q, void* scratch) {
  DAWN_CHECK(h && x && eps && t_all && coef && scratch && nsteps >= 1, "bad argument");
  DAWN_CHECK(noise_all || nsteps == 1, "noise_all is required for more than one step");
  return capture_graph(h, h->ddim_graph, "sampler_capture", "the sampler graph", [&](cudaStream_t st) -> int64_t {
    const int64_t n = clip_values(h) * h->B;
    int64_t launches = 0;
    for (int k = 0; k < nsteps; ++k) {
      DAWN_TRY(forward_x3_impl(h, x, t_all + k, 0, eps, st));
      launches += h->launches;
      const float* cf = coef + 5 * k;
      DAWN_TRY(dawn_unet_ddim_step(h, x, eps, (k < nsteps - 1) ? noise_all + (size_t)k * n : nullptr, n, cf[0], cf[1], cf[2], cf[3],
                                   cf[4], q, scratch, st));
    }
    return launches;
  });
}

int dawn_unet_sampler_launch(dawn_unet* h, void* stream) {
  return launch_graph(h, &dawn_unet::ddim_graph, "sampler_capture", "sampler_launch", stream);
}

int dawn_unet_ddim_step_guided(dawn_unet* h, float* x, const float* eps, const float* noise, int64_t n_clip, const float* cond_scale_dev,
                               float ca, float cb, float sqrt_an, float c, float sigma, float q, void* scratch, void* stream) {
  DAWN_CHECK(h, "null handle");
  DAWN_CHECK(h->sh_nranks <= 1, "guided DDIM steps run on an unsharded handle (a frame-sharded handle holds one clip, not a pair)");
  DAWN_CHECK(h->F > 0 && h->B % 2 == 0, "a guided DDIM step needs an even clip count B = 2b (b conditioned clips, then their null twins)");
  DAWN_CHECK(x && eps && cond_scale_dev && scratch, "bad argument");
  DAWN_CHECK(n_clip == clip_values(h), "n_clip must be the size of one clip (3 * F * height * width)");
  const int b = h->B / 2;
  for (int i = 0; i < b; ++i)
    DAWN_TRY(ddim_guided_step_impl(x + i * n_clip, x + (b + i) * n_clip, eps + i * n_clip, eps + (b + i) * n_clip,
                                   noise ? noise + i * n_clip : nullptr, n_clip, cond_scale_dev, ca, cb, sqrt_an, c, sigma, q, scratch,
                                   (cudaStream_t)stream));
  return 0;
}

int dawn_unet_sampler_capture_guided(dawn_unet* h, float* x, float* eps, const float* noise_all, const int64_t* t_all,
                                     const float* cond_scale_dev, const float* coef, int nsteps, float q, void* scratch) {
  DAWN_CHECK(h && x && eps && t_all && cond_scale_dev && coef && scratch && nsteps >= 1, "bad argument");
  DAWN_CHECK(noise_all || nsteps == 1, "noise_all is required for more than one step");
  return capture_graph(h, h->guided_graph, "sampler_capture_guided", "the sampler graph", [&](cudaStream_t st) -> int64_t {
    DAWN_CHECK(h->sh_nranks <= 1 && h->B % 2 == 0, "the guided sampler graph needs an unsharded handle with an even clip count");
    const int64_t nc = clip_values(h), n_noise = nc * (h->B / 2);
    int64_t launches = 0;
    for (int k = 0; k < nsteps; ++k) {
      DAWN_TRY(forward_x3_impl(h, x, t_all + k, 0, eps, st));
      launches += h->launches;
      const float* cf = coef + 5 * k;
      DAWN_TRY(dawn_unet_ddim_step_guided(h, x, eps, (k < nsteps - 1) ? noise_all + (size_t)k * n_noise : nullptr, nc, cond_scale_dev,
                                          cf[0], cf[1], cf[2], cf[3], cf[4], q, scratch, st));
    }
    return launches;
  });
}

int dawn_unet_sampler_launch_guided(dawn_unet* h, void* stream) {
  return launch_graph(h, &dawn_unet::guided_graph, "sampler_capture_guided", "sampler_launch_guided", stream);
}

static int ddpm_step_handle(dawn_unet* h, float* x, const float* eps, const float* noise, int64_t n_local, DdpmCoef c,
                            const DdpmCoef* tab, const int64_t* t_slot, int num_t, float q, void* scratch, cudaStream_t st) {
  return update_clips(h, n_local, [&](int64_t o, int64_t n, int64_t n_global, const DdimReduce* red) {
    return ddpm_step_impl(x + o, eps + o, noise ? noise + o : nullptr, n, n_global, c, tab, t_slot, num_t, q, scratch, st, red);
  });
}

int dawn_unet_ddpm_step(dawn_unet* h, float* x, const float* eps, const float* noise, int64_t n_local, float ca, float cb,
                        float c1, float c2, float sigma, float q, void* scratch, void* stream) {
  DAWN_CHECK(h, "null handle");
  return ddpm_step_handle(h, x, eps, noise, n_local, DdpmCoef{ca, cb, c1, c2, sigma}, nullptr, nullptr, 0, q, scratch,
                          (cudaStream_t)stream);
}

int dawn_unet_ddpm_capture(dawn_unet* h, float* x, float* eps, const float* noise, int64_t* t_slot, const float* coef,
                           int num_timesteps, float q, void* scratch) {
  static_assert(sizeof(DdpmCoef) == 5 * sizeof(float), "a coefficient table row is 5 floats");
  DAWN_CHECK(h && x && eps && noise && t_slot && coef && scratch && num_timesteps >= 1, "bad argument");
  return capture_graph(h, h->ddpm_graph, "ddpm_capture", "the ancestral step graph", [&](cudaStream_t st) -> int64_t {
    DAWN_TRY(forward_x3_impl(h, x, t_slot, 0, eps, st));
    const int64_t launches = h->launches;
    DAWN_TRY(ddpm_step_handle(h, x, eps, noise, clip_values(h) * h->B, DdpmCoef{}, reinterpret_cast<const DdpmCoef*>(coef), t_slot,
                              num_timesteps, q, scratch, st));
    DAWN_TRY(ddpm_advance_slot(t_slot, st));
    return launches;
  });
}

int dawn_unet_ddpm_launch(dawn_unet* h, void* stream) {
  return launch_graph(h, &dawn_unet::ddpm_graph, "ddpm_capture", "ddpm_launch", stream);
}

int64_t dawn_unet_last_launch_count(dawn_unet* h) { return h ? h->launches : 0; }

int dawn_unet_profile_enable(dawn_unet* h, int on) {
  DAWN_CHECK(h, "null handle");
  h->prof_on = on != 0;
  h->prof_used = 0;
  h->prof_recs.clear();
  for (int i = 0; i < DAWN_PROF_NCAT; ++i) { h->prof_ms[i] = 0; h->prof_flops[i] = 0; h->prof_bytes[i] = 0; h->prof_cnt[i] = 0; }
  return 0;
}

int dawn_unet_profile_read(dawn_unet* h, double* ms, double* flops, double* bytes, int64_t* count) {
  DAWN_CHECK(h && ms && flops && bytes && count, "null argument");
  if (h->prof_used > 0) {
    DAWN_CUDA_OK(cudaEventSynchronize(h->prof_ev[h->prof_used - 1]));
    for (size_t i = 0; i < h->prof_recs.size(); ++i) {
      float t = 0.f;
      DAWN_CUDA_OK(cudaEventElapsedTime(&t, h->prof_ev[2 * i], h->prof_ev[2 * i + 1]));
      const auto& r = h->prof_recs[i];
      h->prof_ms[r.cat] += t; h->prof_flops[r.cat] += r.flops; h->prof_bytes[r.cat] += r.bytes; h->prof_cnt[r.cat]++;
    }
    h->prof_used = 0;
    h->prof_recs.clear();
  }
  for (int i = 0; i < DAWN_PROF_NCAT; ++i) { ms[i] = h->prof_ms[i]; flops[i] = h->prof_flops[i]; bytes[i] = h->prof_bytes[i]; count[i] = h->prof_cnt[i]; }
  return 0;
}
int64_t dawn_unet_workspace_bytes(dawn_unet* h) { return h ? h->workspace.bytes() : 0; }

}
```

### include/dawn_unet.h

```cpp
#ifndef DAWN_UNET_H_
#define DAWN_UNET_H_

#include <stdint.h>

#ifdef __cplusplus
extern "C" {
#endif

typedef struct dawn_unet dawn_unet;

typedef struct {
  int dim;
  int n_levels;
  int dim_mults[8];
  int channels;
  int cond_aud;
  int cond_pose;
  int cond_eye;
  int out_grid_dim;
  int out_conf_dim;
  int attn_heads;
  int attn_dim_head;
  int resnet_groups;
  int init_kernel_size;
  int win_width;
  int upconv;
  int pad_mode;
  int no_sla;
} dawn_unet_cfg;

int dawn_unet_create(const dawn_unet_cfg* cfg, dawn_unet** out);
void dawn_unet_destroy(dawn_unet* h);

int dawn_unet_set_param(dawn_unet* h, const char* name, const float* host, const int64_t* shape, int ndim);
int dawn_unet_commit_params(dawn_unet* h);

int dawn_unet_set_num_frames(dawn_unet* h, int F, int height, int width);
int dawn_unet_set_geometry(dawn_unet* h, int B, int F, int height, int width);

int dawn_nccl_unique_id(char* out128);
int dawn_unet_init_shard(dawn_unet* h, const char* id128, int nranks, int rank, int F_global);
int dawn_unet_shard_ipc_export(dawn_unet* h, char* out64);
int dawn_unet_shard_ipc_import(dawn_unet* h, const char* handles);

int dawn_unet_set_clip_invariants(dawn_unet* h, const float* fea, const float* cond, void* stream);

int dawn_unet_forward(dawn_unet* h, const float* x, const int64_t* t, const float* cond, float* out, void* stream);

int dawn_unet_forward_x3(dawn_unet* h, const float* x_t, const int64_t* t, float* out, void* stream);

int dawn_unet_forward_host(dawn_unet* h, const float* x_t, const float* fea, const float* cond, int64_t t, float* out);

int dawn_unet_set_tap(dawn_unet* h, const char* name, float* dst);
int dawn_unet_tap_shape(dawn_unet* h, const char* name, int* C, int* hl, int* wl);

#define DAWN_PROF_NCAT 20
int dawn_unet_profile_enable(dawn_unet* h, int on);
int dawn_unet_profile_read(dawn_unet* h, double* ms, double* flops, double* bytes, int64_t* count);

int64_t dawn_unet_last_launch_count(dawn_unet* h);
int64_t dawn_unet_workspace_bytes(dawn_unet* h);

int dawn_ddim_step(float* x, const float* eps, const float* noise, int64_t n, float ca, float cb, float sqrt_an, float c,
                   float sigma, float q, void* scratch, void* stream);

int dawn_unet_ddim_step(dawn_unet* h, float* x, const float* eps, const float* noise, int64_t n_local, float ca, float cb,
                        float sqrt_an, float c, float sigma, float q, void* scratch, void* stream);

int dawn_unet_sampler_capture(dawn_unet* h, float* x, float* eps, const float* noise_all, const int64_t* t_all,
                              const float* coef, int nsteps, float q, void* scratch);
int dawn_unet_sampler_launch(dawn_unet* h, void* stream);

int dawn_unet_ddim_step_guided(dawn_unet* h, float* x, const float* eps, const float* noise, int64_t n_clip, const float* cond_scale_dev,
                               float ca, float cb, float sqrt_an, float c, float sigma, float q, void* scratch, void* stream);

int dawn_unet_sampler_capture_guided(dawn_unet* h, float* x, float* eps, const float* noise_all, const int64_t* t_all,
                                     const float* cond_scale_dev, const float* coef, int nsteps, float q, void* scratch);
int dawn_unet_sampler_launch_guided(dawn_unet* h, void* stream);

int dawn_ddpm_step(float* x, const float* eps, const float* noise, int64_t n, float ca, float cb, float c1, float c2,
                   float sigma, float q, void* scratch, void* stream);

int dawn_unet_ddpm_step(dawn_unet* h, float* x, const float* eps, const float* noise, int64_t n_local, float ca, float cb,
                        float c1, float c2, float sigma, float q, void* scratch, void* stream);

int dawn_unet_ddpm_capture(dawn_unet* h, float* x, float* eps, const float* noise, int64_t* t_slot, const float* coef,
                           int num_timesteps, float q, void* scratch);
int dawn_unet_ddpm_launch(dawn_unet* h, void* stream);

enum {
  DAWN_PATH_MMA_SYNC = 0,
  DAWN_PATH_TC_GEMM = 1,
  DAWN_PATH_TC_GEMM_PRESPLIT = 2,
  DAWN_PATH_TC_CONV3 = 3,
  DAWN_PATH_TC_CONV3_TMA = 4
};
typedef struct {
  int path, epi;
  int F, IH, IW, Cin, lda;
  int ntaps; int dy[52]; int dx[52]; int in_stride;
  int OHs, OWs, OH, OW, out_stride, oy0, ox0;
  int up2;
  int perm_pb, perm_F, perm_in, perm_out, perm_f_lo, perm_f_hi;
  int P;
  int N, ldb, ldo, ldr, drain, ln_inline;
  int rows_per_batch;
  long long b_batch_stride;
  int cpg;
  float q_post_scale;
  const float* A; const float* B; const float* bias; const float* Res; float* Out;
  double* stats;
  const float* rowstats;
  const float* wsum;
  const float* rot;
  const float* kq; const float* nkq; float* gates;
  const float* Y; int ldy; const double* gn_stats; const float* gn_w; const float* gn_b; const float* film; double gn_count;
} dawn_contraction_case;
int dawn_test_contraction(const dawn_contraction_case* c, void* stream);

enum {
  DAWN_FUSED_TEMPORAL = 0,
  DAWN_FUSED_ATTN_TC = 1,
  DAWN_FUSED_ATTN_SIMT = 2,
  DAWN_FUSED_SLA_CTX = 3,
  DAWN_FUSED_SLA_OUT = 4,
  DAWN_FUSED_SLA_CTX_UNFUSED = 5,
  DAWN_FUSED_CA_WT = 6,
  DAWN_FUSED_CA_RSTD = 7,
  DAWN_FUSED_GN_HCOND = 8,
  DAWN_FUSED_TEMPORAL_MMA_SYNC = 9
};
typedef struct {
  int kernel;
  int F, P, C;
  int band, q_lo, q_hi;
  int nseq, L, pb;
  long long seq_base_stride, elem_stride;
  int ldx, ldr, ldo, ld, ldb, ldy, ldbT;
  const float* x; const float* res; float* out;
  const float* gamma;
  const float* w_qkv;
  const float* w_out;
  const float* rot;
  const float* bias;
  const float* qkv;
  float* Bf;
  const float* out_bias;
  const float* kq; const float* nkq; const float* G; const float* gates; float* Wt;
  const float* T; const float* Y; unsigned short* out16h; unsigned short* out16l;
  const double* gn_stats; double gn_count; int cpg; const float* gn_w; const float* gn_b; const float* film;
} dawn_fused_case;
int dawn_test_fused(const dawn_fused_case* c, void* stream);

enum {
  DAWN_KERNEL_ROWSTATS = 0,
  DAWN_KERNEL_GN_APPLY = 1,
  DAWN_KERNEL_COND_TABLES = 2,
  DAWN_KERNEL_TIME_MLP = 3,
  DAWN_KERNEL_FILM = 4,
  DAWN_KERNEL_ROTARY = 5,
  DAWN_KERNEL_SPLIT_ROWS = 6,
  DAWN_KERNEL_NCF_TO_NHWC = 7,
  DAWN_KERNEL_FRAME_INVARIANCE = 8,
  DAWN_KERNEL_FEA_SHIFT = 9,
  DAWN_KERNEL_MAP_REDUCE = 10,
  DAWN_KERNEL_INIT_CONV_X3 = 11,
  DAWN_KERNEL_HEADS_OUT = 12,
  DAWN_KERNEL_DDIM_STEP = 13,
  DAWN_KERNEL_DDPM_STEP = 14
};
#define DAWN_KERNEL_MAX_DESC 16
typedef struct {
  int off, K, co, ldbT, ca;
  const float* mW; const float* mB;
  const float* Wkv;
  const float* nkv; const float* qs; const float* ks;
  const float* Wout; const float* gout;
  float* ctx; float* kv;
  float* kq; float* nkq; float* T; float* G;
  const float* W; const float* b; float* out; int n;
} dawn_kernel_desc;
typedef struct {
  int kernel;
  int M, C, ld, ldy, ldr, ldo;
  int F, H, W, P, clips;
  int Cpad, c0, k, skip_if, cpg, t_stride, pos0, dim, ng, nc, cond_ld, ndesc;
  long long n, cstride, clip_stride;
  double count; float eps;
  const float* x; const float* y; const float* res;
  const float* w; const float* b; const float* w2; const float* b2;
  const float* map; const float* freqs; const double* stats; const int64_t* t; const int* skip_flag;
  float* out; void* out_hi; void* out_lo; int* flag;
  dawn_kernel_desc desc[DAWN_KERNEL_MAX_DESC];
  float* xs; const float* e; const float* noise; void* scratch;
  const float* tab; const int64_t* t_slot; int num_t;
  int replicas;
  float coef[5]; float q;
} dawn_kernel_case;
int dawn_test_kernel(const dawn_kernel_case* c, void* stream);

const char* dawn_last_error(void);
int64_t dawn_live_bytes(void);
const char* dawn_build_info(void);

#ifdef __cplusplus
}
#endif
#endif
```

Measured before the change: 23.19.

## Split-K balance the tail wave of the persistent tensor-core 3x3 conv

Adds a stream-K style scheduler to the persistent tc_conv3 kernel. Whole output tiles are handed out round-robin as before, but the leftover tail tiles are split by input-channel chunk across all CTAs. Partial accumulators are published to a global workspace with acquire/release flags, and the owning CTA sums them before running the epilogue. This targets the idle SMs in a partial last wave, at the cost of extra global traffic, spin-waiting on flags and a new persistent workspace allocation.

```diff
diff --git a/dawn_pytorch_b200/_lib.py b/dawn_pytorch_b200/_lib.py
--- a/dawn_pytorch_b200/_lib.py
+++ b/dawn_pytorch_b200/_lib.py
@@ -41,7 +41,8 @@
                 ("A", _p), ("B", _p), ("bias", _p), ("Res", _p), ("Out", _p),
                 ("stats", _p), ("rowstats", _p), ("wsum", _p), ("rot", _p),
                 ("kq", _p), ("nkq", _p), ("gates", _p),
-                ("Y", _p), ("ldy", _i), ("gn_stats", _p), ("gn_w", _p), ("gn_b", _p), ("film", _p), ("gn_count", ctypes.c_double)]
+                ("Y", _p), ("ldy", _i), ("gn_stats", _p), ("gn_w", _p), ("gn_b", _p), ("film", _p), ("gn_count", ctypes.c_double),
+                ("c3_work", _p), ("c3_grid", _i), ("clips", _i)]
 
 
 FUSED_TEMPORAL, FUSED_ATTN_TC, FUSED_ATTN_SIMT, FUSED_SLA_CTX, FUSED_SLA_OUT, FUSED_SLA_CTX_UNFUSED, FUSED_CA_WT, \
@@ -185,6 +186,14 @@
     lib.dawn_unet_workspace_bytes.argtypes = [vp]
     lib.dawn_unet_workspace_bytes.restype = ctypes.c_int64
     lib.dawn_test_contraction.argtypes = [ctypes.POINTER(DawnContractionCase), vp]
+    ip, ci = ctypes.POINTER(ctypes.c_int), ctypes.c_int
+    lib.dawn_conv3_split_pays.argtypes = [ci, ci, ci]
+    lib.dawn_conv3_workspace_bytes.argtypes = [ci]
+    lib.dawn_conv3_workspace_bytes.restype = ctypes.c_int64
+    lib.dawn_conv3_flag_bytes.argtypes = [ci]
+    lib.dawn_conv3_flag_bytes.restype = ctypes.c_int64
+    lib.dawn_conv3_items.argtypes = [ci, ci, ci, ci, ci, ip, ci]
+    lib.dawn_conv3_producers.argtypes = [ci, ci, ci, ci, ci, ci, ip, ci]
     lib.dawn_test_fused.argtypes = [ctypes.POINTER(DawnFusedCase), vp]
     lib.dawn_test_kernel.argtypes = [ctypes.POINTER(DawnKernelCase), vp]
     lib.dawn_nccl_unique_id.argtypes = [ctypes.c_char_p]
@@ -275,7 +284,8 @@
            "dawn_unet_profile_enable", "dawn_unet_profile_read", "dawn_unet_last_launch_count", "dawn_unet_workspace_bytes", "dawn_ddim_step", "dawn_unet_ddim_step", "dawn_unet_sampler_capture", "dawn_unet_sampler_launch",
            "dawn_unet_ddim_step_guided", "dawn_unet_sampler_capture_guided", "dawn_unet_sampler_launch_guided",
            "dawn_ddpm_step", "dawn_unet_ddpm_step", "dawn_unet_ddpm_capture", "dawn_unet_ddpm_launch",
-           "dawn_test_contraction", "dawn_test_fused", "dawn_test_kernel", "dawn_last_error", "dawn_live_bytes", "dawn_build_info"]
+           "dawn_test_contraction", "dawn_conv3_split_pays", "dawn_conv3_workspace_bytes", "dawn_conv3_flag_bytes", "dawn_conv3_items",
+           "dawn_conv3_producers", "dawn_test_fused", "dawn_test_kernel", "dawn_last_error", "dawn_live_bytes", "dawn_build_info"]
 
 
 LFG_EXPORTS = ["dawn_lfg_create", "dawn_lfg_destroy", "dawn_lfg_set_param", "dawn_lfg_commit_params", "dawn_lfg_set_geometry",
diff --git a/dawn_pytorch_b200/csrc/contraction.cu b/dawn_pytorch_b200/csrc/contraction.cu
--- a/dawn_pytorch_b200/csrc/contraction.cu
+++ b/dawn_pytorch_b200/csrc/contraction.cu
@@ -321,7 +321,9 @@
   p.B = c.B; p.ldb = c.ldb; p.b_batch_stride = c.b_batch_stride;
   p.Out = c.Out; p.ldo = c.ldo; p.OH = c.OH; p.OW = c.OW; p.out_stride = c.out_stride; p.oy0 = c.oy0; p.ox0 = c.ox0;
   p.bias = c.bias; p.Res = c.Res; p.ldr = c.ldr;
-  p.stats = c.stats; p.cpg = c.cpg; p.clips = 1;
+  if (c.clips < 0 || c.clips > 1 && c.F % c.clips != 0) return refuse("the frame count must be a multiple of the clip count");
+  p.stats = c.stats; p.cpg = c.cpg; p.clips = c.clips > 1 ? c.clips : 1;
+  p.c3_work = c.c3_work; p.c3_grid = c.c3_grid;
   p.rowstats = c.rowstats; p.ln_inline = c.ln_inline; p.wsum = c.wsum; p.rot = c.rot; p.P = c.P;
   p.q_post_scale = c.q_post_scale;
   p.kq = c.kq; p.nkq = c.nkq; p.gates = c.gates;
diff --git a/dawn_pytorch_b200/csrc/conv3_sched.cuh b/dawn_pytorch_b200/csrc/conv3_sched.cuh
--- /dev/null
+++ b/dawn_pytorch_b200/csrc/conv3_sched.cuh
@@ -0,0 +1,65 @@
+#pragma once
+#include <cstddef>
+#include <cstdint>
+
+namespace dawn {
+
+struct C3Sched {
+  int tiles, nch, grid;
+  int dp_waves, dp_rem, dp_tiles;
+};
+
+struct C3Item {
+  int tile, c0, c1, unit0;
+};
+
+__host__ __device__ inline bool c3_split_pays(int tiles, int grid, int nch) {
+  if (nch < 2 || grid < 2) return false;
+  const int waves = tiles / grid, rem = tiles % grid;
+  const int tail_chunks = (int)(((long long)rem * nch + grid - 1) / grid);
+  return rem > 0 && waves < 16 && 2 * tail_chunks <= nch;
+}
+
+__host__ __device__ inline size_t c3_flag_bytes(int grid) { return ((size_t)grid * 2 * sizeof(int) + 255) / 256 * 256; }
+__host__ __device__ inline size_t c3_workspace_bytes(int grid) { return c3_flag_bytes(grid) + (size_t)grid * 128 * 128 * sizeof(float); }
+
+__host__ __device__ inline C3Sched c3_sched(int tiles, int grid, int nch, bool split) {
+  return split ? C3Sched{tiles, nch, grid, tiles / grid, 0, tiles / grid * grid} : C3Sched{tiles, nch, grid, tiles / grid, tiles % grid, tiles};
+}
+
+__host__ __device__ inline int c3_tail_units(const C3Sched& s) { return (s.tiles - s.dp_tiles) * s.nch; }
+__host__ __device__ inline int c3_run_begin(const C3Sched& s, int b) { return b * c3_tail_units(s) / s.grid; }
+__host__ __device__ inline int c3_unit_owner(const C3Sched& s, int u) { return ((u + 1) * s.grid - 1) / c3_tail_units(s); }
+template <typename Fn>
+__host__ __device__ inline void c3_producers(const C3Sched& s, const C3Item& it, Fn&& f) {
+  for (int u = it.unit0 + s.nch - 1 - it.c1; u >= it.unit0;) {
+    const int b = c3_unit_owner(s, u);
+    f(b);
+    u = c3_run_begin(s, b) - 1;
+  }
+}
+
+__host__ __device__ inline int c3_num_whole(const C3Sched& s, int b) { return s.dp_waves + (b < s.dp_rem); }
+
+__host__ __device__ inline int c3_num_items(const C3Sched& s, int b) {
+  const int ndp = c3_num_whole(s, b);
+  const int u0 = c3_run_begin(s, b), u1 = c3_run_begin(s, b + 1);
+  return ndp + (u1 > u0 ? (u1 - 1) / s.nch - u0 / s.nch + 1 : 0);
+}
+
+__host__ __device__ inline C3Item c3_item(const C3Sched& s, int b, int j) {
+  const int ndp = c3_num_whole(s, b);
+  if (j < ndp) return C3Item{b + j * s.grid, 0, s.nch, 0};
+  const int u0 = c3_run_begin(s, b), u1 = c3_run_begin(s, b + 1);
+  const int t0 = u0 / s.nch, t1 = (u1 - 1) / s.nch;
+  const bool ends_inside = u1 % s.nch != 0;
+  int k = j - ndp, t;
+  if (ends_inside) t = k == 0 ? t1 : t0 + k - 1;
+  else t = t0 + k;
+  const int base = t * s.nch;
+  const int k0 = u0 > base ? u0 - base : 0;
+  const int k1 = u1 - base < s.nch ? u1 - base : s.nch;
+  return C3Item{s.dp_tiles + t, s.nch - k1, s.nch - k0, base};
+}
+
+}
diff --git a/dawn_pytorch_b200/csrc/gemm.cuh b/dawn_pytorch_b200/csrc/gemm.cuh
--- a/dawn_pytorch_b200/csrc/gemm.cuh
+++ b/dawn_pytorch_b200/csrc/gemm.cuh
@@ -52,6 +52,8 @@
   double gn_count;
   const int* skip_flag; int skip_if;
   int drain;
+  void* c3_work = nullptr;
+  int c3_grid = 0;
 };
 
 __host__ __device__ inline int seq_blocked_pixel(int m, int pb, int F, int P) {
diff --git a/dawn_pytorch_b200/csrc/tc_conv3.cu b/dawn_pytorch_b200/csrc/tc_conv3.cu
--- a/dawn_pytorch_b200/csrc/tc_conv3.cu
+++ b/dawn_pytorch_b200/csrc/tc_conv3.cu
@@ -3,9 +3,11 @@
 #include <cstdlib>
 #include <cstring>
 #include <string>
+#include <algorithm>
 #include <map>
 #include <tuple>
 #include "common.cuh"
+#include "conv3_sched.cuh"
 #include "f16x3.cuh"
 #include "gemm.cuh"
 #include "tc_common.cuh"
@@ -47,9 +49,9 @@
   static_assert(2 * REG_LAUNCH + REG_LOAD + NWG * REG_MMA + (SPLIT_EPI ? REG_EPI : 0) <= NTHREADS / 128 * REG_LAUNCH, "CTA register pool");
 };
 
-template <int BN, bool TMA, bool PAIR>
+template <int BN, bool TMA, bool PAIR, bool BAL>
 __device__ __forceinline__ void tc_conv3_body(const GemmParams& p, const float* __restrict__ Bimg, int tiles_y, int tiles_x, int tiles_n,
-                                              int img_bn, const CUtensorMap& tm_hi, const CUtensorMap& tm_lo) {
+                                              int img_bn, const C3Sched& sched, const CUtensorMap& tm_hi, const CUtensorMap& tm_lo) {
   using C = CCfg<BN, PAIR>;
   constexpr int B_PANEL = C::B_PANEL, A_STAGES = C::A_STAGES, B_STAGES = C::B_STAGES, NWG = C::NWG;
   constexpr int A_HALO = C::A_HALO, FRAME_ROWS = C::FRAME_ROWS;
@@ -81,7 +83,11 @@
   const int tiles_sp = tiles_y * tiles_x;
   const int fpc = F / p.clips;
   const int ppc = (fpc + 1) / 2;
-  const int total_tiles = (PAIR ? p.clips * ppc : F * tiles_sp) * tiles_n;
+  const int nitems = BAL ? c3_num_items(sched, blockIdx.x) : c3_num_whole(sched, blockIdx.x);
+  auto item = [&](int j) {
+    if constexpr (BAL) return c3_item(sched, blockIdx.x, j);
+    else return C3Item{(int)blockIdx.x + j * (int)gridDim.x, 0, NCH, 0};
+  };
   auto decode = [&](int tile, int& f, int& y0, int& x0, int& nt, int& nf) {
     nt = tile % tiles_n;
     const int sp = tile / tiles_n;
@@ -104,10 +110,11 @@
       if (tid == 0) {
         const uint64_t mh = reinterpret_cast<uint64_t>(&tm_hi), ml = reinterpret_cast<uint64_t>(&tm_lo);
         uint32_t ait = 0;
-        for (int tile = blockIdx.x; tile < total_tiles; tile += gridDim.x) {
+        for (int j = 0; j < nitems; ++j) {
+          const C3Item it = item(j);
           int f, y0, x0, nt, nf;
-          decode(tile, f, y0, x0, nt, nf);
-          for (int cc = 0; cc < NCH; ++cc, ++ait) {
+          decode(it.tile, f, y0, x0, nt, nf);
+          for (int cc = it.c0; cc < it.c1; ++cc, ++ait) {
             const int s = ait % A_STAGES;
             mbar_wait(&a_free[s], ((ait / A_STAGES) & 1) ^ 1);
             mbar_arrive_expect_tx(&a_full[s], nf * 2 * FRAME_ROWS * 128);
@@ -129,12 +136,13 @@
       const int c16 = tid & 7;
       const int r0 = (tid >> 3) & 31;
       uint32_t ait = 0;
-      for (int tile = blockIdx.x; tile < total_tiles; tile += gridDim.x) {
+      for (int j = 0; j < nitems; ++j) {
+        const C3Item it = item(j);
         int f, y0, x0, nt, nf;
-        decode(tile, f, y0, x0, nt, nf);
+        decode(it.tile, f, y0, x0, nt, nf);
         const float* img = p.A + (size_t)f * H * W * p.lda;
         const float* img_b = PAIR ? img + (size_t)p.clips * H * W * p.lda : img;
-        for (int cc = 0; cc < NCH; ++cc, ++ait) {
+        for (int cc = it.c0; cc < it.c1; ++cc, ++ait) {
           const int s = ait % A_STAGES;
           const uint32_t round = ait / A_STAGES;
           auto load = [&](int q, float4& a, float4& b) {
@@ -197,11 +205,12 @@
       const int KC = 9 * NCH;
       const int sub = PAIR ? img_bn / BN : 1;
       const size_t ipanel = (size_t)sub * B_PANEL;
-      for (int tile = blockIdx.x; tile < total_tiles; tile += gridDim.x) {
+      for (int j = 0; j < nitems; ++j) {
+        const C3Item it = item(j);
         int f, y0, x0, nt, nf;
-        decode(tile, f, y0, x0, nt, nf);
+        decode(it.tile, f, y0, x0, nt, nf);
         const uint8_t* src = reinterpret_cast<const uint8_t*>(Bimg) + (size_t)(nt / sub) * KC * (2 * ipanel) + (size_t)(nt % sub) * B_PANEL;
-        for (int cc = 0; cc < NCH; ++cc)
+        for (int cc = it.c0; cc < it.c1; ++cc)
           for (int tap = 0; tap < 9; ++tap, ++bit) {
             const int s = bit % B_STAGES;
             const uint32_t round = bit / B_STAGES;
@@ -224,15 +233,16 @@
   const int ew = (warp - 8) & 3;
   const int etid = ew * 32 + lane;
   const int bar_id = 2 + wg;
+  const int part_bar = SPLIT ? 3 : bar_id;
   constexpr uint32_t SBO_HALO = HW * 128;
   constexpr uint32_t H2 = PAIR ? PAIR_ROW_B * 128 : 8 * HW * 128;
   const int dt = (p.drain == 1 || p.drain == 3) ? p.drain : 9;
 
-  auto mma_tile = [&](auto DTc, float* stage, uint32_t& ait, uint32_t& bit, auto&& claim) {
+  auto mma_tile = [&](auto DTc, int nchunks, float* stage, uint32_t& ait, uint32_t& bit, auto&& claim) {
     constexpr int DT = decltype(DTc)::value;
     float d0[32], d1[32];
     bool first_drain = true;
-    for (int cc = 0; cc < NCH; ++cc, ++ait) {
+    for (int cc = 0; cc < nchunks; ++cc, ++ait) {
       const int sa = ait % A_STAGES;
       mbar_wait(&a_full[sa], (ait / A_STAGES) & 1);
       fence_proxy_async();
@@ -304,6 +314,48 @@
       gs[b8] = 0.f; gss[b8] = 0.f;
     }
   };
+  int* const c3_flags = static_cast<int*>(p.c3_work);
+  float4* const c3_parts = reinterpret_cast<float4*>(static_cast<char*>(p.c3_work) + c3_flag_bytes(gridDim.x));
+  auto c3_slot = [&](int b) { return c3_parts + (size_t)(b * NWG + wg) * 16 * 128 + etid; };
+  auto publish_partial = [&](const float* stage) {
+    asm volatile("bar.sync %0, 128;" ::"r"(part_bar) : "memory");
+    const float4* src = reinterpret_cast<const float4*>(stage + etid * kStageLd);
+    float4* dst = c3_slot(blockIdx.x);
+#pragma unroll
+    for (int i = 0; i < 16; ++i) __stcg(dst + i * 128, src[i]);
+    asm volatile("bar.sync %0, 128;" ::"r"(part_bar) : "memory");
+    if (etid == 0) {
+      int* fl = c3_flags + blockIdx.x * NWG + wg;
+      asm volatile("fence.acq_rel.gpu;\n\tst.relaxed.gpu.global.s32 [%0], 1;" ::"l"(fl) : "memory");
+    }
+  };
+  auto add_partials = [&](const C3Item& it, float* stage) {
+    if (etid < 32) {
+      int q = 0;
+      c3_producers(sched, it, [&](int b) {
+        if ((q++ & 31) != lane) return;
+        int* fl = c3_flags + b * NWG + wg;
+        int v;
+        do {
+          asm volatile("ld.acquire.gpu.global.s32 %0, [%1];" : "=r"(v) : "l"(fl) : "memory");
+        } while (v == 0);
+        asm volatile("st.relaxed.gpu.global.s32 [%0], 0;" ::"l"(fl) : "memory");
+      });
+    }
+    asm volatile("bar.sync %0, 128;" ::"r"(part_bar) : "memory");
+    float4* row = reinterpret_cast<float4*>(stage + etid * kStageLd);
+    c3_producers(sched, it, [&](int b) {
+      const float4* src = c3_slot(b);
+      float4 v[16];
+#pragma unroll
+      for (int i = 0; i < 16; ++i) v[i] = __ldcg(src + i * 128);
+#pragma unroll
+      for (int i = 0; i < 16; ++i) {
+        const float4 o = row[i];
+        row[i] = make_float4(o.x + v[i].x, o.y + v[i].y, o.z + v[i].z, o.w + v[i].w);
+      }
+    });
+  };
   auto epilogue_tile = [&](int tile, float* stage, float (&gs)[8], float (&gss)[8], int& pending, int& pclip) {
     int f, y0, x0, nt, nf;
     decode(tile, f, y0, x0, nt, nf);
@@ -402,22 +454,46 @@
 #pragma unroll
     for (int i = 0; i < 8; ++i) { gs[i] = 0.f; gss[i] = 0.f; }
     load_bias();
-    uint32_t lt = 0;
-    for (int tile = blockIdx.x; tile < total_tiles; tile += gridDim.x, ++lt) {
-      const int b = lt & 1;
-      mbar_wait(&st_full[b], (lt >> 1) & 1);
-      epilogue_tile(tile, stage_base + b * 128 * kStageLd, gs, gss, pending, pclip);
-      mbar_arrive(&st_free[b]);
+    if constexpr (!BAL) {
+      uint32_t lt = 0;
+      for (int tile = blockIdx.x; tile < sched.tiles; tile += gridDim.x, ++lt) {
+        const int b = lt & 1;
+        mbar_wait(&st_full[b], (lt >> 1) & 1);
+        epilogue_tile(tile, stage_base + b * 128 * kStageLd, gs, gss, pending, pclip);
+        mbar_arrive(&st_free[b]);
+      }
+    } else {
+      const int nwhole = c3_num_whole(sched, blockIdx.x);
+      const int skip = nitems > nwhole && item(nwhole).c0 > 0 ? 1 : 0;
+      for (int k = 0; k < nitems - skip; ++k) {
+        const int b = k & 1;
+        mbar_wait(&st_full[b], (k >> 1) & 1);
+        epilogue_tile(item(k + (k >= nwhole ? skip : 0)).tile, stage_base + b * 128 * kStageLd, gs, gss, pending, pclip);
+        mbar_arrive(&st_free[b]);
+      }
     }
     if (defer_stats && pending > 0) flush_stats(gs, gss, pclip);
   } else if (SPLIT) {
     setmaxnreg_inc<C::REG_MMA>();
     with_drain([&](auto DTc) {
       uint32_t ait = 0, bit = 0, lt = 0;
-      for (int tile = blockIdx.x; tile < total_tiles; tile += gridDim.x, ++lt) {
+      bool held = false;
+      for (int j = 0; j < nitems; ++j) {
+        const C3Item it = item(j);
         const int b = lt & 1;
-        mma_tile(DTc, stage_base + b * 128 * kStageLd, ait, bit, [&]() { mbar_wait(&st_free[b], ((lt >> 1) & 1) ^ 1); });
+        float* stage = stage_base + b * 128 * kStageLd;
+        mma_tile(DTc, it.c1 - it.c0, stage, ait, bit, [&]() { if (!held) mbar_wait(&st_free[b], ((lt >> 1) & 1) ^ 1); });
+        if constexpr (BAL) {
+          if (it.c0 > 0) {
+            publish_partial(stage);
+            held = true;
+            continue;
+          }
+          if (it.c1 < NCH) add_partials(it, stage);
+        }
         mbar_arrive(&st_full[b]);
+        ++lt;
+        held = false;
       }
     });
   } else {
@@ -429,10 +505,20 @@
     load_bias();
     float* stage = stage_base + wg * 128 * kStageLd;
     uint32_t ait = 0, bit = 0;
-    for (int tile = blockIdx.x; tile < total_tiles; tile += gridDim.x) {
-      with_drain([&](auto DTc) { mma_tile(DTc, stage, ait, bit, []() {}); });
+    for (int j = 0; j < nitems; ++j) {
+      const C3Item it = item(j);
+      with_drain([&](auto DTc) { mma_tile(DTc, it.c1 - it.c0, stage, ait, bit, []() {}); });
       asm volatile("bar.sync %0, 128;" ::"r"(bar_id) : "memory");
-      epilogue_tile(tile, stage, gs, gss, pending, pclip);
+      if constexpr (BAL) {
+        if (it.c0 > 0) {
+          publish_partial(stage);
+        } else {
+          if (it.c1 < NCH) add_partials(it, stage);
+          epilogue_tile(it.tile, stage, gs, gss, pending, pclip);
+        }
+      } else {
+        epilogue_tile(it.tile, stage, gs, gss, pending, pclip);
+      }
       asm volatile("bar.sync %0, 128;" ::"r"(bar_id) : "memory");
     }
     if (defer_stats && pending > 0) flush_stats(gs, gss, pclip);
@@ -442,23 +528,41 @@
 template <int BN, bool TMA>
 __global__ void __launch_bounds__(CCfg<BN>::NTHREADS, 1) tc_conv3_kernel(const GemmParams p, const float* __restrict__ Bimg,
                                                                           int tiles_y, int tiles_x, int tiles_n, int img_bn,
+                                                                          const __grid_constant__ C3Sched sched,
                                                                           const __grid_constant__ CUtensorMap tm_hi,
                                                                           const __grid_constant__ CUtensorMap tm_lo) {
-  tc_conv3_body<BN, TMA, false>(p, Bimg, tiles_y, tiles_x, tiles_n, img_bn, tm_hi, tm_lo);
+  tc_conv3_body<BN, TMA, false, false>(p, Bimg, tiles_y, tiles_x, tiles_n, img_bn, sched, tm_hi, tm_lo);
+}
+
+template <int BN, bool TMA>
+__global__ void __launch_bounds__(CCfg<BN>::NTHREADS, 1) tc_conv3_balanced_kernel(const GemmParams p, const float* __restrict__ Bimg,
+                                                                                   int tiles_y, int tiles_x, int tiles_n, int img_bn,
+                                                                                   const __grid_constant__ C3Sched sched,
+                                                                                   const __grid_constant__ CUtensorMap tm_hi,
+                                                                                   const __grid_constant__ CUtensorMap tm_lo) {
+  tc_conv3_body<BN, TMA, false, true>(p, Bimg, tiles_y, tiles_x, tiles_n, img_bn, sched, tm_hi, tm_lo);
 }
 
 template <bool TMA>
 __global__ void __launch_bounds__(CCfg<64, true>::NTHREADS, 1) tc_conv3_pair_kernel(const GemmParams p, const float* __restrict__ Bimg,
                                                                                      int tiles_y, int tiles_x, int tiles_n, int img_bn,
+                                                                                     const __grid_constant__ C3Sched sched,
                                                                                      const __grid_constant__ CUtensorMap tm_hi,
                                                                                      const __grid_constant__ CUtensorMap tm_lo) {
-  tc_conv3_body<64, TMA, true>(p, Bimg, tiles_y, tiles_x, tiles_n, img_bn, tm_hi, tm_lo);
-}
-
-template <int BN, bool TMA, bool PAIR>
+  tc_conv3_body<64, TMA, true, false>(p, Bimg, tiles_y, tiles_x, tiles_n, img_bn, sched, tm_hi, tm_lo);
+}
+
+template <bool TMA>
+__global__ void __launch_bounds__(CCfg<64, true>::NTHREADS, 1) tc_conv3_pair_balanced_kernel(
+    const GemmParams p, const float* __restrict__ Bimg, int tiles_y, int tiles_x, int tiles_n, int img_bn,
+    const __grid_constant__ C3Sched sched, const __grid_constant__ CUtensorMap tm_hi, const __grid_constant__ CUtensorMap tm_lo) {
+  tc_conv3_body<64, TMA, true, true>(p, Bimg, tiles_y, tiles_x, tiles_n, img_bn, sched, tm_hi, tm_lo);
+}
+
+template <int BN, bool TMA, bool PAIR, bool BAL>
 constexpr auto c3_kernel() {
-  if constexpr (PAIR) return tc_conv3_pair_kernel<TMA>;
-  else return tc_conv3_kernel<BN, TMA>;
+  if constexpr (PAIR) return BAL ? tc_conv3_pair_balanced_kernel<TMA> : tc_conv3_pair_kernel<TMA>;
+  else return BAL ? tc_conv3_balanced_kernel<BN, TMA> : tc_conv3_kernel<BN, TMA>;
 }
 
 typedef CUresult (*EncodeTiledFn)(CUtensorMap*, CUtensorMapDataType, cuuint32_t, void*, const cuuint64_t*, const cuuint64_t*, const cuuint32_t*,
@@ -496,8 +600,10 @@
   static bool attr_set = false;
   static int num_sms = 0;
   if (!attr_set) {
-    DAWN_CUDA_OK(cudaFuncSetAttribute(c3_kernel<BN, false, PAIR>(), cudaFuncAttributeMaxDynamicSharedMemorySize, C::SMEM_DYN));
-    DAWN_CUDA_OK(cudaFuncSetAttribute(c3_kernel<BN, true, PAIR>(), cudaFuncAttributeMaxDynamicSharedMemorySize, C::SMEM_DYN));
+    DAWN_CUDA_OK(cudaFuncSetAttribute(c3_kernel<BN, false, PAIR, false>(), cudaFuncAttributeMaxDynamicSharedMemorySize, C::SMEM_DYN));
+    DAWN_CUDA_OK(cudaFuncSetAttribute(c3_kernel<BN, true, PAIR, false>(), cudaFuncAttributeMaxDynamicSharedMemorySize, C::SMEM_DYN));
+    DAWN_CUDA_OK(cudaFuncSetAttribute(c3_kernel<BN, false, PAIR, true>(), cudaFuncAttributeMaxDynamicSharedMemorySize, C::SMEM_DYN));
+    DAWN_CUDA_OK(cudaFuncSetAttribute(c3_kernel<BN, true, PAIR, true>(), cudaFuncAttributeMaxDynamicSharedMemorySize, C::SMEM_DYN));
     int dev = 0;
     DAWN_CUDA_OK(cudaGetDevice(&dev));
     DAWN_CUDA_OK(cudaDeviceGetAttribute(&num_sms, cudaDevAttrMultiProcessorCount, dev));
@@ -506,18 +612,24 @@
   const int tiles_y = PAIR ? 1 : p.IH / TH, tiles_x = PAIR ? 1 : p.IW / TW, tiles_n = p.N / BN;
   const int F = p.M / (p.IH * p.IW);
   const int seqs = PAIR ? p.clips * ((F / p.clips + 1) / 2) : F;
-  const int grid = std::min(seqs * tiles_y * tiles_x * tiles_n, num_sms);
+  const int tiles = seqs * tiles_y * tiles_x * tiles_n;
+  const int grid = std::min({tiles, num_sms, p.c3_grid > 0 ? p.c3_grid : num_sms});
+  const int nch = p.Cin / 64;
+  const bool split = p.c3_work != nullptr && c3_split_pays(tiles, grid, nch);
+  const C3Sched sched = c3_sched(tiles, grid, nch, split);
   const int img_bn = tc_tile_n(p.N);
   if (p.A16h != nullptr && p.A16l != nullptr) {
     CUtensorMap mh, ml;
     const int box_h = PAIR ? PAIR_HH : HH;
     if (halo_tensor_map(p.A16h, p.Cin, p.IW, p.IH, F, box_h, &mh) != 0 || halo_tensor_map(p.A16l, p.Cin, p.IW, p.IH, F, box_h, &ml) != 0)
       return -2;
-    c3_kernel<BN, true, PAIR>()<<<grid, C::NTHREADS, C::SMEM_DYN, st>>>(p, Bimg, tiles_y, tiles_x, tiles_n, img_bn, mh, ml);
+    (split ? c3_kernel<BN, true, PAIR, true>() : c3_kernel<BN, true, PAIR, false>())<<<grid, C::NTHREADS, C::SMEM_DYN, st>>>(
+        p, Bimg, tiles_y, tiles_x, tiles_n, img_bn, sched, mh, ml);
   } else {
     CUtensorMap dummy;
     memset(&dummy, 0, sizeof(dummy));
-    c3_kernel<BN, false, PAIR>()<<<grid, C::NTHREADS, C::SMEM_DYN, st>>>(p, Bimg, tiles_y, tiles_x, tiles_n, img_bn, dummy, dummy);
+    (split ? c3_kernel<BN, false, PAIR, true>() : c3_kernel<BN, false, PAIR, false>())<<<grid, C::NTHREADS, C::SMEM_DYN, st>>>(
+        p, Bimg, tiles_y, tiles_x, tiles_n, img_bn, sched, dummy, dummy);
   }
   DAWN_LAUNCH_OK();
   return 0;
@@ -542,6 +654,12 @@
   return true;
 }
 
+size_t tc_conv3_workspace_bytes() {
+  int dev = 0, sms = 0;
+  if (cudaGetDevice(&dev) != cudaSuccess || cudaDeviceGetAttribute(&sms, cudaDevAttrMultiProcessorCount, dev) != cudaSuccess) return 0;
+  return c3_workspace_bytes(sms);
+}
+
 int launch_tc_conv3(const GemmParams& p, const float* Bimg, cudaStream_t st) {
   if (!tc_conv3_supported(p, EPI_PLAIN)) { set_last_error("launch_tc_conv3: unsupported geometry"); return -1; }
   if (pair_mode(p)) return launch_c3<64, true>(p, Bimg, st);
@@ -550,3 +668,30 @@
 }
 
 }
+
+extern "C" int dawn_conv3_split_pays(int tiles, int grid, int nch) { return dawn::c3_split_pays(tiles, grid, nch) ? 1 : 0; }
+
+extern "C" int64_t dawn_conv3_workspace_bytes(int grid) { return (int64_t)dawn::c3_workspace_bytes(grid); }
+
+extern "C" int64_t dawn_conv3_flag_bytes(int grid) { return (int64_t)dawn::c3_flag_bytes(grid); }
+
+extern "C" int dawn_conv3_items(int tiles, int grid, int nch, int split, int cta, int* out, int cap) {
+  if (tiles < 1 || grid < 1 || grid > tiles || nch < 1 || cta < 0 || cta >= grid || cap < 0) return -1;
+  const dawn::C3Sched s = dawn::c3_sched(tiles, grid, nch, split != 0);
+  const int n = dawn::c3_num_items(s, cta);
+  for (int j = 0; j < n && j < cap; ++j) {
+    const dawn::C3Item it = dawn::c3_item(s, cta, j);
+    out[3 * j] = it.tile; out[3 * j + 1] = it.c0; out[3 * j + 2] = it.c1;
+  }
+  return n;
+}
+
+extern "C" int dawn_conv3_producers(int tiles, int grid, int nch, int split, int cta, int j, int* out, int cap) {
+  if (tiles < 1 || grid < 1 || grid > tiles || nch < 1 || cta < 0 || cta >= grid || cap < 0) return -1;
+  const dawn::C3Sched s = dawn::c3_sched(tiles, grid, nch, split != 0);
+  if (j < 0 || j >= dawn::c3_num_items(s, cta)) return -1;
+  const dawn::C3Item it = dawn::c3_item(s, cta, j);
+  int n = 0;
+  if (it.c0 == 0) dawn::c3_producers(s, it, [&](int b) { if (n < cap) out[n] = b; ++n; });
+  return n;
+}
diff --git a/dawn_pytorch_b200/csrc/tc_gemm.cuh b/dawn_pytorch_b200/csrc/tc_gemm.cuh
--- a/dawn_pytorch_b200/csrc/tc_gemm.cuh
+++ b/dawn_pytorch_b200/csrc/tc_gemm.cuh
@@ -11,5 +11,6 @@
 int launch_tc_gemm(const GemmParams& p, const float* Bimg, int epi, cudaStream_t st);
 bool tc_conv3_supported(const GemmParams& p, int epi);
 int launch_tc_conv3(const GemmParams& p, const float* Bimg, cudaStream_t st);
+size_t tc_conv3_workspace_bytes();
 
 }
diff --git a/dawn_pytorch_b200/csrc/unet.cu b/dawn_pytorch_b200/csrc/unet.cu
--- a/dawn_pytorch_b200/csrc/unet.cu
+++ b/dawn_pytorch_b200/csrc/unet.cu
@@ -11,6 +11,7 @@
 #include "contraction.cuh"
 #include "gemm.cuh"
 #include "kernels.cuh"
+#include "tc_gemm.cuh"
 #include "temporal_fused.cuh"
 #include "sla_fused.cuh"
 #include "ca_fused.cuh"
@@ -181,6 +182,7 @@
   float *Y = nullptr, *A1 = nullptr, *QKV = nullptr, *O = nullptr, *ROWSTATS = nullptr, *GATES = nullptr, *WT = nullptr;
   float *BF = nullptr, *HF = nullptr, *HO = nullptr, *ROT = nullptr, *TSILU = nullptr;
   float* UPPAD = nullptr;
+  uint8_t* C3WORK = nullptr;
   double* STATS = nullptr; int n_stats = 0;
   int64_t* T_HOSTSIDE = nullptr;
   float *H_XT = nullptr, *H_FEA = nullptr, *H_COND = nullptr, *H_OUT = nullptr;
@@ -418,7 +420,9 @@
   ProfScope ps(*this, cat, flops, bytes);
   const size_t scratch = (size_t)(h->F * h->B + 2 * h->cfg.win_width) * h->lH[0] * h->lW[0] * 256 * sizeof(float);
   int kernels = 0;
-  const int rc = launch_path(p, epi, choose_path(p, epi, scratch), h->O, st, &kernels);
+  GemmParams q = p;
+  q.c3_work = h->C3WORK;
+  const int rc = launch_path(q, epi, choose_path(q, epi, scratch), h->O, st, &kernels);
   h->launches += kernels - 1;
   return rc;
 }
@@ -1050,6 +1054,12 @@
   DAWN_TRY(ws.alloc((size_t)B * h->tdim, &h->TSILU));
   DAWN_TRY(ws.alloc((size_t)h->n_stats * 16 * B, &h->STATS));
   DAWN_TRY(ws.alloc(2, &h->T_HOSTSIDE));
+  {
+    const size_t n = tc_conv3_workspace_bytes();
+    DAWN_CHECK(n > 0, "cannot query the device's SM count");
+    DAWN_TRY(ws.alloc(n, &h->C3WORK));
+    DAWN_CUDA_OK(cudaMemset(h->C3WORK, 0, n));
+  }
   DAWN_TRY(ws.alloc(3 * M0, &h->H_XT));
   DAWN_TRY(ws.alloc((size_t)(h->cfg.channels - 3) * P0, &h->H_FEA));
   DAWN_TRY(ws.alloc((size_t)F * h->cond_dim, &h->H_COND));
diff --git a/include/dawn_unet.h b/include/dawn_unet.h
--- a/include/dawn_unet.h
+++ b/include/dawn_unet.h
@@ -115,8 +115,14 @@
   const float* rot;
   const float* kq; const float* nkq; float* gates;
   const float* Y; int ldy; const double* gn_stats; const float* gn_w; const float* gn_b; const float* film; double gn_count;
+  void* c3_work; int c3_grid; int clips;
 } dawn_contraction_case;
 int dawn_test_contraction(const dawn_contraction_case* c, void* stream);
+int dawn_conv3_split_pays(int tiles, int grid, int nch);
+int64_t dawn_conv3_workspace_bytes(int grid);
+int64_t dawn_conv3_flag_bytes(int grid);
+int dawn_conv3_items(int tiles, int grid, int nch, int split, int cta, int* out, int cap);
+int dawn_conv3_producers(int tiles, int grid, int nch, int split, int cta, int j, int* out, int cap);
 
 enum {
   DAWN_FUSED_TEMPORAL = 0,
```

After: 23.44, median of 6. 1.01x the previous value.
